# GANtastic3/MaskCycleGAN-VC

Measured on AMD Instinct MI355X. Metric: train iters/s (full G+D step), 80x64 mel bs=1, higher is better.
Workload: dtype f32

## Files before the change

### include/mcvc.h

```cpp
#ifndef MCVC_H
#define MCVC_H

#ifdef __cplusplus
extern "C" {
#endif

#define MCVC_ABI_VERSION 3
#define MCVC_GEN_NPARAMS 110
#define MCVC_DISC_NPARAMS 20
#define MCVC_N_MEL 80

int mcvc_version(void);

int mcvc_set_deterministic(int on);
int mcvc_get_deterministic(void);
int mcvc_set_precise(int on);
int mcvc_get_precise(void);
int mcvc_set_trunk_persistent(int on);

int mcvc_twin_begin(void);
int mcvc_twin_switch(void);
int mcvc_twin_end(void);
int mcvc_twin_launches(void);

// ... 19 lines not shown
                     float* out, float* stash, float* scratch, long long scratch_floats, int B, int T, void* stream);
int mcvc_gen_backward(const float* const* params, const float* packed, float* const* grads, const float* mask,
                      const float* dout, float* dx, int accumulate_dx, const float* stash,
                      float* scratch, long long scratch_floats, int B, int T, void* stream, void* aux_stream);
int mcvc_gen_backward_overlap(const float* const* params, const float* packed, float* const* grads, const float* mask,
                              const float* dout, float* dx, int accumulate_dx, const float* stash,
                              float* scratch, long long scratch_floats, int B, int T, void* stream, void* aux_stream,
                              void* const* milestones);

int mcvc_gen_trunk_fault(float* scratch, int B, int T, int reset, void* stream);
int mcvc_debug_trunk_fault_inject(int on);

#define MCVC_BWD_NO_JOIN 1
#define MCVC_BWD_FINE_MILESTONES 2
#define MCVC_BWD_STORE_GRADS 4
int mcvc_grad_store_mask(int net, int T, unsigned char* covered);
int mcvc_gen_backward_flags(const float* const* params, const float* packed, float* const* grads, const float* mask,
                            const float* dout, float* dx, int accumulate_dx, const float* stash,
                            float* scratch, long long scratch_floats, int B, int T, void* stream, void* aux_stream,
                            void* const* milestones, int flags);
int mcvc_gen_backward_prefix(const float* const* params, const float* packed, float* const* grads, const float* mask,
                             const float* dout, float* dx, int accumulate_dx, const float* stash, int stash_B,
                             float* scratch, long long scratch_floats, int B, int T, void* stream, void* aux_stream,
                             void* const* milestones, int flags);
int mcvc_gen_backward_window(const float* const* params, const float* packed, float* const* grads, const float* mask,
                             const float* dout, float* dx, int accumulate_dx, const float* stash, int stash_B, int stash_b0,
                             float* scratch, long long scratch_floats, int B, int T, void* stream, void* aux_stream,
                             void* const* milestones, int flags);
int mcvc_set_trunk_passes_in_flight(int n);
int mcvc_gen_trunk_persistent(int B, int T);

long long mcvc_gen_bf16_packed_bytes(void);
long long mcvc_gen_bf16_workspace_bytes(int B, int T);
int mcvc_gen_bf16_pack(const float* const* params, void* packed, void* stream);
int mcvc_gen_infer_bf16(const float* const* params, const void* packed, const float* x, const float* mask, float* out, void* workspace,
                        long long workspace_bytes, int B, int T, void* stream);

long long mcvc_bf16_conv2d_pack_bytes(int Cout, int Cin, int KH, int KW);
int mcvc_bf16_conv2d(const void* x, const float* w, const float* bias, void* y, void* wpack, int N, int H, int W, int Cin, int Cout,
                     int KH, int KW, int stride, int pad_h, int pad_w, void* stream);
long long mcvc_bf16_conv1_glu_pack_bytes(void);
int mcvc_bf16_conv1_glu(const float* x, const float* mask, const float* w, const float* b, const float* wg, const float* bg, void* y, void* wpack,
                        int B, int T, void* stream);
long long mcvc_bf16_last_conv_pack_bytes(void);
int mcvc_bf16_last_conv(const void* x, const float* w, const float* b, float* out, void* wpack, int B, int T, void* stream);
long long mcvc_bf16_c2d1d_pack_bytes(void);
int mcvc_bf16_c2d1d_norm(const void* x, const float* w, const float* gamma, const float* beta, void* y, void* wpack, int B, int W, void* stream);
long long mcvc_bf16_trunk_layer_pack_bytes(int Cin, int C, int gated);
int mcvc_bf16_trunk_layer(const void* x, const float* w, const float* w_gate, const float* gamma, const float* beta, const float* gamma_gate,
                          const float* beta_gate, const void* residual, void* y, void* wpack, int B, int W, int Cin, int C, void* stream);
int mcvc_bf16_instnorm_act(const void* x, const float* gamma, const float* beta, const float* gamma_gate, const float* beta_gate,
                           const void* residual, void* y, float* scratch, int N, int H, int W, int Cx, int act, int pixel_shuffle, void* stream);

int mcvc_disc_forward(const float* const* params, const float* packed, const float* x, float* out,
                      float* stash, float* scratch, long long scratch_floats, int B, int T, void* stream);
int mcvc_disc_backward(const float* const* params, const float* packed, float* const* grads,
                       const float* dout, int dout_is_logit_grad, float* dx, int accumulate_dx,
                       const float* stash, float* scratch, long long scratch_floats, int B, int T, void* stream,
                       void* aux_stream);
int mcvc_disc_backward_flags(const float* const* params, const float* packed, float* const* grads,
                             const float* dout, int dout_is_logit_grad, float* dx, int accumulate_dx,
                             const float* stash, float* scratch, long long scratch_floats, int B, int T, void* stream,
                             void* aux_stream, int flags);

int mcvc_l1_loss(const float* a, const float* b, long long n, float weight, float* loss_slot, float* term_slot,
                 float* grad_a, int accumulate_grad, void* stream);
int mcvc_lsgan_loss(const float* d, long long n, float target, float weight, float* loss_slot, float* term_slot,
                    float* grad_logit, void* stream);

int mcvc_loss_combine(const float* pairs, int n, const int* loss_dst, const int* term_dst, float* slots, void* stream);

int mcvc_adam_step(float* p, const float* g, float* exp_avg, float* exp_avg_sq, long long n, float lr,
                   float beta1, float beta2, float eps, int step, float grad_scale, void* stream);
int mcvc_adam_step2(float* p, float* g, float* g2, int zero_grads, float* exp_avg, float* exp_avg_sq, long long n, float lr,
                    float beta1, float beta2, float eps, int step, float grad_scale, void* stream);
int mcvc_gen_update_ranges(const float* const* params, const long long* numel, float* packed, int max_batch, int T, int range_mask,
                           const float* flat, float* grad, float* grad2, float* exp_avg, float* exp_avg_sq, float lr, float beta1,
                           float beta2, float eps, int step, float grad_scale, int zero_grads, void* stream);
int mcvc_disc_update_batch(const float* const* params, const long long* numel, float* packed, int max_batch, int T,
                           const float* flat, float* grad, float* grad2, float* exp_avg, float* exp_avg_sq, float lr, float beta1,
                           float beta2, float eps, int step, float grad_scale, int zero_grads, void* stream);

int mcvc_pack_plan(int net, int max_batch, int T, int sets, int range_mask, int update, long long* rows, int cap, int* n_rows);
int mcvc_axpy(float* y, const float* x, float alpha, long long n, void* stream);

int mcvc_draw_batch(const float* bank_A, const int* offs_A, int n_A, long long frames_A, const float* bank_B, const int* offs_B, int n_B,
                    long long frames_B, int B, int T, int max_mask_len, unsigned long long seed, unsigned long long step,
                    float* real_A, float* mask_A, float* real_B, float* mask_B, int* draws, void* stream);

int mcvc_audio_frames(int n_samples);
long long mcvc_audio_basis_floats(void);
int mcvc_audio_basis_init(float* basis);
int mcvc_audio_plan(const int* sample_offs, int n_utts, int* frame_offs, int* tiles, int max_tiles, int* n_tiles);
int mcvc_audio_log_mel(const float* wave, long long n_samples, const int* tiles, int n_tiles, const float* basis, float* out,
                       long long total_frames, void* stream);

int mcvc_voc_out_samples(int T);
int mcvc_voc_launches(void);
long long mcvc_voc_packed_floats(void);
int mcvc_voc_pack(const float* const* host_table, float* packed_host);
long long mcvc_voc_workspace_floats(int B, int T);
int mcvc_voc_decode(const float* packed, const float* mel, float* out, float* workspace, long long workspace_floats, int B, int T, void* stream);
long long mcvc_voc_layer_packed_floats(int kind, int Cin, int Cout, int k, int r);
int mcvc_voc_layer_pack(int kind, const float* w0, const float* b0, const float* w1, const float* b1, float* packed_host, int Cin, int Cout, int k, int r);
int mcvc_voc_layer(int kind, const float* packed, const float* x0, const float* x1, float* y, int B, int Cin, int Cout, int L, int k, int dilation, int r,
                   int act_in, void* stream);

int mcvc_gl_out_samples(int T);
int mcvc_gl_launches(int n_iter);
long long mcvc_gl_tables_floats(void);
int mcvc_gl_tables_init(const float* host_pinv, float* host_out);
long long mcvc_gl_workspace_floats(int B, int T);
int mcvc_gl_decode(const float* in, int in_kind, const float* angles0, const float* tables, float* out, float* workspace,
                   long long workspace_floats, int B, int T, int n_iter, float momentum, void* stream);

int mcvc_melinv_max_iter(void);
long long mcvc_melinv_tables_floats(void);
int mcvc_melinv_tables_init(const float* host_basis, const float* host_pinv, double lambda, float* host_out);
int mcvc_melinv_solve(const float* logmel, const float* tables, float* mag_out, int B, int T, int n_iter, void* stream);

int mcvc_dtw_max_frames(void);
int mcvc_dtw_launches(int want_path);
int mcvc_cep_basis_init(int n_cep, float* basis_host);
int mcvc_cep_project(const float* mel, long long n_frames, const float* basis, int n_cep, float* out, void* stream);
int mcvc_dtw_plan(const int* x_offs, const int* y_offs, int n_pairs, int want_path, long long* table, long long* workspace_bytes, long long* path_rows);
int mcvc_dtw_run(const float* x, long long x_frames, const float* y, long long y_frames, int K, float scale, const int* x_offs, const int* y_offs,
                 const long long* table, int n_pairs, float* cost, int* length, int* path, void* workspace, long long workspace_bytes, void* stream);

int mcvc_f0_max_lag(void);
int mcvc_f0_launches(int want_cmnd);
int mcvc_f0_track(const float* wave, long long n_samples, const int* tiles, int n_tiles, int tau_min, int tau_max, float threshold, float* f0,
                  float* aperiodicity, float* cmnd, long long total_frames, void* stream);
int mcvc_f0_stats(const float* fx, long long x_frames, const float* fy, long long y_frames, const int* path, const long long* pairs, int n_pairs,
                  int* counts, float* sums, void* stream);

int mcvc_ms_max_fft(void);
int mcvc_ms_launches(void);
int mcvc_ms_table_init(int n_fft, float* table_host);
int mcvc_ms_power(const float* cep, long long n_frames, int K, const int* offs_dev, int n_utts, const int* offs_host, int n_fft, const float* table,
                  float* power, float* mean, float* var, void* stream);
int mcvc_ms_mean_log(const float* values, int n, long long R, float floor, float* out, void* stream);
int mcvc_ms_distance(const float* a, const float* b, int K, int n_bins, int n_used, float* per_dim, float* total, void* stream);

long long mcvc_conv2d_pack_floats(int Cout, int Cin, int KH, int KW);
int mcvc_conv2d_forward(const float* x, const float* w, const float* bias, float* y, float* wpack,
                        float* slabs, int max_slabs, int N, int Cin, int H, int W, int Cout, int KH, int KW,
                        int stride, int pad_h, int pad_w, int pixel_shuffle, void* stream);
int mcvc_conv2d_dgrad(const float* dy, const float* w, float* dx, float* wpack, float* slabs, int max_slabs,
                      int N, int Cin, int H, int W, int Cout, int KH, int KW, int stride, int pad_h, int pad_w,
                      void* stream);
long long mcvc_conv2d_wgrad_slab_floats(int N, int Cin, int H, int W, int Cout, int KH, int KW, int stride, int pad_h, int pad_w);
int mcvc_conv2d_wgrad(const float* x, const float* dy, float* dw, float* slabs, long long slab_floats, int N, int Cin, int H, int W,
                      int Cout, int KH, int KW, int stride, int pad_h, int pad_w, void* stream);
long long mcvc_layer_packed_floats(int Cin, int Cout, int branches, int KH, int KW, int stride, int pad_h, int pad_w);
long long mcvc_layer_scratch_floats(int N, int H, int W, int Cin, int Cout, int branches, int KH, int KW, int stride, int pad_h, int pad_w);
int mcvc_layer_pack(const float* w0, const float* b0, const float* w1, const float* b1, float* packed, int Cin, int Cout, int branches,
                    int KH, int KW, int stride, int pad_h, int pad_w, void* stream);
int mcvc_layer_forward(const float* x, const float* packed, const float* w0, const float* w1, float* y, float* scratch,
                       long long scratch_floats, int N, int H, int W, int Cin, int Cout, int branches, int KH, int KW, int stride,
                       int pad_h, int pad_w, int scheme, int pixel_shuffle, void* stream);
int mcvc_layer_dgrad(const float* dy, const float* packed, const float* w0, const float* w1, float* dx, float* scratch,
                     long long scratch_floats, int N, int H, int W, int Cin, int Cout, int branches, int KH, int KW, int stride,
                     int pad_h, int pad_w, int scheme, void* stream);
int mcvc_layer_wgrad(const float* x, const float* dy, float* dw0, float* dw1, float* scratch, long long scratch_floats, int N, int H,
                     int W, int Cin, int Cout, int branches, int KH, int KW, int stride, int pad_h, int pad_w, int scheme, void* stream);
int mcvc_layer_wgrad_flags(const float* x, const float* dy, float* dw0, float* dw1, float* scratch, long long scratch_floats, int N, int H,
// ... 39 lines not shown
```

### maskcyclegan-vc_amd/csrc/net.hip

```cpp
#include "mcvc_common.h"
#include "twin.h"
#include "pack.h"
#include "packforms.h"
#include "misc.h"
#include "trunk.h"
#include "wino.h"
#include "wino4.h"
#include "sgemm.h"
#include "sampler.h"
#include "audio.h"
#include "vocoder.h"
#include "griffinlim.h"
#include "melinv.h"
#include "dtw.h"
#include "ms.h"
#include "f0.h"
#include "../../include/mcvc.h"
#include <string.h>
#include <algorithm>
#include <array>
#include <tuple>
#include <map>
#include <mutex>
#include <vector>

static int g_deterministic = [] { const char* e = getenv("MCVC_DETERMINISTIC"); return (e && atoi(e) != 0) ? 1 : 0; }();
int mcvc_deterministic() { return g_deterministic; }

namespace {

constexpr float kInEps = 1e-5f;

struct View { float* p; long long sb, sc; int sh; };
struct CView { const float* p; long long sb, sc; int sh; };
static inline CView cv(const View& v) { return CView{v.p, v.sb, v.sc, v.sh}; }

constexpr int kMaxLayers = 20;
struct PackFresh { unsigned layer[kMaxLayers]; PackFresh() { for (unsigned& m : layer) m = kAllForms; } };

struct Exec {
    hipStream_t s;
    bool dry;
    int err;
    bool fine_ms = false;
    float* slabs;
    long long slab_cap;
    long long slab_need;
    int max_split;
    hipStream_t s2;
    float* wslabs;
    long long wslab_cap;
    long long wslab_need;
    float* wv; float* wm;
    long long wino_cap;
    float* wv2; float* wm2; float* wu;
    long long wu_cap;
    float* sg; long long sg_cap, sg_need;
    float* sgw; long long sgw_cap, sgw_need;
    const float* const* params;
    int br1_on_main = 0;
    int no_join = 0;
    int fuse_next = 0;
    const struct WinoFam* pend_fam = nullptr;
    WinoOutArgs pend;
    int y_xs_pw = 0; long long y_xs_plane = 0;
    int dx_pitch = 0;
    int wgrad_x_xs = 0;
    int store_grads = 0;
    int force_scheme = 0;
    PackFresh fresh;
    unsigned* sync;
    std::vector<std::pair<const void*, hipEvent_t>> readers;
    void fail(int e) { if (!err && e) err = e; }
};

static std::mutex g_pack_mu;
static std::map<const void*, PackFresh> g_pack_fresh;
static PackFresh get_fresh(const void* packed)
{
    std::lock_guard<std::mutex> lk(g_pack_mu);
    auto it = g_pack_fresh.find(packed);
    return it == g_pack_fresh.end() ? PackFresh() : it->second;
}

static hipEvent_t pool_event()
{
    static std::mutex mu;
    static std::vector<hipEvent_t> pool;
    static size_t next = 0;
    std::lock_guard<std::mutex> lk(mu);
    if (pool.empty()) {
        pool.resize(1024);
        for (hipEvent_t& e : pool) (void)hipEventCreateWithFlags(&e, hipEventDisableTiming);
    }
    next = (next + 1) % pool.size();
    return pool[next];
}

static bool is_fresh(const Exec& ex, const ConvSpec& c, PackForm f) { return (ex.fresh.layer[c.index] >> f & 1) != 0; }
static bool any_fresh(const Exec& ex, PackForm f) { for (unsigned m : ex.fresh.layer) if (m >> f & 1) return true; return false; }
static bool stale(Exec& ex, const ConvSpec& c, PackForm f)
{
    if (ex.dry || is_fresh(ex, c, f)) return false;
    ex.fail(MCVC_ERR_INVALID);
    return true;
}

static void wait_readers(Exec& ex, const void* buf)
{
    if (!ex.s2 || ex.dry) return;
    for (auto it = ex.readers.begin(); it != ex.readers.end();) {
        if (it->first == buf) { ex.fail(mcvc_stream_wait(ex.s, it->second)); it = ex.readers.erase(it); }
        else ++it;
    }
}

static void join_aux(Exec& ex)
{
    if (!ex.s2 || ex.dry) return;
    hipEvent_t e = pool_event();
    ex.fail(mcvc_event_record(e, ex.s2));
    ex.fail(mcvc_stream_wait(ex.s, e));
    ex.readers.clear();
}

static ConvSpec mk(int Cin, int Cout, int nbr, int KH, int KW, int stride, int ph, int pw, int w0, int b0, int w1, int b1, int bias_grad)
{
    ConvSpec c{};
    c.Cin = Cin; c.Cout = Cout; c.nbr = nbr; c.KH = KH; c.KW = KW; c.stride = stride; c.ph = ph; c.pw = pw;
    c.wi[0] = w0; c.bi[0] = b0; c.wi[1] = w1; c.bi[1] = b1; c.has_bias_grad = bias_grad;
    return c;
}

static inline int conv_out(int H, int K, int s, int p) { return (H + 2 * p - K) / s + 1; }

static void run_conv(Exec& ex, const ConvProblem& p, int NB, ConvIO io, long long y_total, const float* w, int w_rows, int w_cout,
                     const float* bias, int allow_split, int force_nsplit, int* nsplit_out)
{
    int ns = 1;
    if (force_nsplit > 0) ns = force_nsplit;
    else if (allow_split) ns = mcvc_conv_plan_nsplit(p, NB, 1);
    if (ns < 1) { ex.fail(MCVC_ERR_INVALID); ns = 1; }
    if (ex.max_split > 0 && ns > ex.max_split) ns = ex.max_split;
    if (io.accumulate && mcvc_deterministic()) ns = 1;
    if (!io.accumulate) {
        const long long need = (long long)(ns - 1) * y_total;
        if (need > ex.slab_need) ex.slab_need = need;
// ... 47 lines not shown
    return n < 32 ? 32 : n;
}
static int wino43_min_nb()
{
    static const int nb = mcvc_knob("MCVC_WINO43_NB", 4);
    return nb;
}
static bool wino4_applies(const Exec& ex, const ConvSpec& c, int NB, int H, int W, bool reads_set = true)
{
    if (ex.force_scheme == 1 || ex.force_scheme >= 3) return false;
    if (ex.force_scheme == 2) return c.wino && (H & 3) == 0 && (W & 3) == 0;
    return c.wino && wino4_min_nb() > 0 && NB >= wino4_min_nb() && (H & 3) == 0 && (W & 3) == 0 &&
           (reads_set ? is_fresh(ex, c, PF_W4F) : any_fresh(ex, PF_W4F));
}
static bool wino43_applies(const Exec& ex, const ConvSpec& c, int NB, int OH, int OW, bool reads_set = true)
{
    if (ex.force_scheme == 1 || ex.force_scheme >= 3) return false;
    if (ex.force_scheme == 2) return c.wino3 && (OH & 3) == 0 && (OW & 3) == 0;
    return c.wino3 && wino43_min_nb() > 0 && NB >= wino43_min_nb() && (OH & 3) == 0 && (OW & 3) == 0 &&
           (reads_set ? is_fresh(ex, c, PF_W43F) : any_fresh(ex, PF_W43F));
}
static int wino4_chunk(const Exec& ex, int NB, long long tiles_per_sample, int KM, int pts)
{
    const long long cap_tiles = (ex.wino_cap / ((long long)pts * KM)) & ~31LL;
    if (tiles_per_sample <= 0 || cap_tiles < tiles_per_sample) return 0;
    const long long nbmax = cap_tiles / tiles_per_sample;
    if (NB <= nbmax) return NB;
    const long long nch = (NB + nbmax - 1) / nbmax;
    return (int)((NB + nch - 1) / nch);
}

struct WinoFam {
    int pts;
    int nxi;
    int tile;
    int pad;
    int min_pitch;
    int norm_pts;
    int (*input)(const WinoXformArgs&, hipStream_t);
    int (*input_phase)(const WinoXformArgs&, int XH, int XW, hipStream_t);
    int (*output)(const WinoOutArgs&, hipStream_t);
    int (*input_t)(const WinoXformArgs&, hipStream_t);
    int (*input_phase_t)(const WinoXformArgs&, int XH, int XW, hipStream_t);
    int (*dy_t)(const WinoXformArgs&, hipStream_t);
    int (*dw)(const float* du, float* dw0, float* dw1, int Cout, int nbr, int Cin, int store, hipStream_t);
};
enum { kF23, kF25, kF43, kF45 };
static const WinoFam kWino[4] = {
    {16, 16, 2, 1, 32, 16, mcvc_wino3_input_launch, mcvc_wino3_input_phase_launch, mcvc_wino3_output_launch,
     nullptr, mcvc_wino3_input_phase_t_launch, mcvc_wino3_dy_t_launch, mcvc_wino3_dw_launch},
    {36, 0, 2, 2, 32, 36, mcvc_wino_input_launch, nullptr, mcvc_wino_output_launch,
     mcvc_wino_input_t_launch, nullptr, mcvc_wino_dy_t_launch,
     [](const float* du, float* dw0, float*, int Cout, int, int Cin, int store, hipStream_t s) { return mcvc_wino_dw_launch(du, dw0, Cout, Cin, store, s); }},
    {36, 36, 4, 1, 32, 43, mcvc_wino43_input_launch, mcvc_wino43_input_phase_launch, mcvc_wino43_output_launch,
     nullptr, mcvc_wino43_input_phase_t_launch, mcvc_wino43_dy_t_launch, mcvc_wino43_dw_launch},
    {64, 64, 4, 2, 64 , 64, mcvc_wino4_input_launch, nullptr, mcvc_wino4_output_launch,
     mcvc_wino4_input_t_launch, nullptr, mcvc_wino4_dy_t_launch,
     [](const float* du, float* dw0, float*, int Cout, int, int Cin, int store, hipStream_t s) { return mcvc_wino4_dw_launch(du, dw0, Cout, Cin, store, s); }},
};
static long long wino_tiles(const WinoFam& f, int H, int W) { return (long long)((H + f.tile - 1) / f.tile) * ((W + f.tile - 1) / f.tile); }

static int wino_nbc(const Exec& ex, const WinoFam& f, int NB, long long tiles, int KM, int min_tiles)
{
    if (f.tile == 4) {
        const int nbc = wino4_chunk(ex, NB, tiles, KM, f.pts);
        return (nbc && (nbc * tiles >= min_tiles || ex.force_scheme == 2)) ? nbc : 0;
    }
    const int nbc = wino_chunk(NB, tiles);
    const long long NTc = wino_chunk_tiles(NB, tiles);
    return (nbc && NTc >= min_tiles && f.pts * NTc * KM <= ex.wino_cap) ? nbc : 0;
}

struct WinoPass {
    const WinoFam* f;
    int K, M;
    int NB, nbc;
    int H, W;
    int XH, XW;
    const float* a; long long a_xi; int lda, a_rows;
    const float* bias;
    int shuffle, YH, YW, accumulate;
    bool may_defer;
};
static void wino_pass(Exec& ex, const WinoPass& p, CView x, View y)
{
    const WinoFam& f = *p.f;
    const int K = p.K, M = p.M, TH = (p.H + f.tile - 1) / f.tile, TW = (p.W + f.tile - 1) / f.tile;
    for (int b0 = 0; b0 < p.NB; b0 += p.nbc) {
        const int nb = p.NB - b0 < p.nbc ? p.NB - b0 : p.nbc;
        const long long NT = (long long)nb * TH * TW, NTp = std::max<long long>((NT + 31) & ~31LL, f.min_pitch);
        WinoXformArgs xi{};
        xi.x = x.p + (long long)b0 * x.sb; xi.x_sb = x.sb; xi.x_sc = x.sc; xi.x_sh = x.sh; xi.v = ex.wv;
        xi.N = nb; xi.C = K; xi.H = p.H; xi.W = p.W; xi.TH = TH; xi.TW = TW; xi.NT = (int)NT; xi.NTp = (int)NTp; xi.pad = f.pad;
        ex.fail(p.XH ? f.input_phase(xi, p.XH, p.XW, ex.s) : f.input(xi, ex.s));
        static const int own_gemm = mcvc_knob("MCVC_WINO_GEMM", 1);
        if (&f != &kWino[kF25] || (own_gemm && (M % 128) == 0 && (K % 16) == 0 && NTp >= 64)) {
            WinoGemmArgs ga{};
            ga.a = p.a; ga.a_xi = p.a_xi; ga.lda = p.lda;
            ga.b = ex.wv; ga.b_xi = (long long)K * NTp; ga.ldb = (int)NTp;
            ga.c = ex.wm; ga.c_xi = (long long)M * NTp; ga.ldc = (int)NTp;
            ga.M = M; ga.N = (int)NTp; ga.K = K; ga.nxi = f.nxi;
            ex.fail(mcvc_wino_gemm_launch(ga, ex.s));
        } else {
            ConvProblem cp{K, (int)(NTp / 32), 32, M, (int)(NTp / 32), 32, 1, 1, 1, 0, 0};
            ConvIO io{};
            io.x = ex.wv; io.x_sb = (long long)K * NTp; io.x_sc = NTp; io.x_sh = 32;
            io.y = ex.wm; io.y_sb = (long long)M * NTp; io.y_sc = NTp; io.y_sh = 32; io.y_sw = 1;
            io.nsplit = 1;
            io.w_nstride = p.a_xi;
            io.tile_cfg = wino_tile_cfg(M, NT);
            io.gemm_ok = 1;
            ex.fail(mcvc_conv_launch(cp, 36, io, p.a, p.a_rows, p.lda, nullptr, ex.s, nullptr));
        }
        WinoOutArgs oa{};
        oa.m = ex.wm; oa.bias = p.bias;
        oa.y = y.p + (long long)b0 * y.sb; oa.y_sb = y.sb; oa.y_sc = y.sc; oa.y_sh = y.sh;
        oa.N = nb; oa.Cout = M; oa.OH = p.H; oa.OW = p.W; oa.TH = TH; oa.TW = TW; oa.NT = (int)NT; oa.NTp = (int)NTp;
        oa.shuffle = p.shuffle; oa.YH = p.YH; oa.YW = p.YW; oa.accumulate = p.accumulate;
        if (p.may_defer && ex.fuse_next && p.nbc == p.NB) { ex.pend = oa; ex.pend_fam = &f; }
        else ex.fail(f.output(oa, ex.s));
    }
}

static void wino_wgrad_pass(Exec& ex, const WinoFam& f, const ConvSpec& c, float* const* grads, int NB, int nbc, int H, int W, CView x, CView dy,
                            int store, hipStream_t ws)
{
    const bool phase = c.stride == 2;
    const int IH = phase ? H / 2 : H, IW = phase ? W / 2 : W, N = phase ? 4 * c.Cin : c.Cin, M = c.cout_tot;
    const int TH = (IH + f.tile - 1) / f.tile, TW = (IW + f.tile - 1) / f.tile;
    for (int b0 = 0; b0 < NB; b0 += nbc) {
        const int nb = NB - b0 < nbc ? NB - b0 : nbc;
        const long long NT = (long long)nb * TH * TW, NTp = (NT + 31) & ~31LL;
        WinoXformArgs xi{};
        xi.x = x.p + (long long)b0 * x.sb; xi.x_sb = x.sb; xi.x_sc = x.sc; xi.x_sh = x.sh; xi.v = ex.wv2;
        xi.N = nb; xi.C = N; xi.H = IH; xi.W = IW; xi.TH = TH; xi.TW = TW; xi.NT = (int)NT; xi.NTp = (int)NTp; xi.pad = f.pad;
        ex.fail(phase ? f.input_phase_t(xi, H, W, ws) : f.input_t(xi, ws));
        WinoXformArgs di{};
        di.x = dy.p + (long long)b0 * dy.sb; di.x_sb = dy.sb; di.x_sc = dy.sc; di.x_sh = dy.sh; di.v = ex.wm2;
        di.N = nb; di.C = M; di.H = IH; di.W = IW; di.TH = TH; di.TW = TW; di.NT = (int)NT; di.NTp = (int)NTp; di.pad = 0;
        ex.fail(f.dy_t(di, ws));
        WinoGemmArgs ga{};
        ga.a = ex.wm2; ga.a_xi = NTp * M; ga.lda = M;
        ga.b = ex.wv2; ga.b_xi = NTp * N; ga.ldb = N;
        ga.c = ex.wu; ga.c_xi = (long long)M * N; ga.ldc = N;
        ga.M = M; ga.N = N; ga.K = (int)((NT + 15) & ~15LL); ga.nxi = f.nxi;
        ex.fail(mcvc_wino_gemm_launch(ga, ws));
        ex.fail(f.dw(ex.wu, grads[c.wi[0]], c.nbr == 2 ? grads[c.wi[1]] : nullptr, c.Cout, c.nbr, c.Cin, store && b0 == 0, ws));
    }
}

static bool conv_wino(Exec& ex, const ConvSpec& c, const float* packed, int dgrad, int NB, int H, int W, CView x, View y, int shuffle,
                      int accumulate)
{
    if (!c.wino || !wino_enabled() || !ex.wv) return false;
    const int K = dgrad ? c.cout_tot : c.Cin, M = dgrad ? c.Cin : c.cout_tot;
    const WinoFam* f = &kWino[kF45];
    int nbc = 0;
    if (wino4_applies(ex, c, NB, H, W) && (M % 128) == 0 && (K % 16) == 0) nbc = wino_nbc(ex, *f, NB, wino_tiles(*f, H, W), K > M ? K : M, wino4_min_tiles());
    if (!nbc) {
        if (stale(ex, c, wino_form(false, dgrad))) return true;
        f = &kWino[kF25];
        nbc = wino_nbc(ex, *f, NB, wino_tiles(*f, H, W), K > M ? K : M, 0);
    }
    if (!nbc) return false;
    if (ex.dry) return true;
    const bool four = f->tile == 4;
    WinoPass p{};
    p.f = f; p.K = K; p.M = M; p.NB = NB; p.nbc = nbc; p.H = H; p.W = W;
    const PackForm form = wino_form(four, dgrad);
    p.a = packed + c.off[form]; p.a_xi = form_xi(c, form); p.lda = kPackForms[form].ld(c); p.a_rows = dgrad ? c.dg_rows_co : c.cin_pad;
    p.bias = dgrad ? nullptr : packed + c.off[PF_BIAS];
    p.shuffle = shuffle; p.YH = 2 * H; p.YW = 2 * W; p.accumulate = accumulate;
    p.may_defer = !dgrad && shuffle;
    wino_pass(ex, p, x, y);
    return true;
}

static bool conv_wino3(Exec& ex, const ConvSpec& c, const float* packed, int dgrad, int NB, int H, int W, CView x, View y, int accumulate)
{
    if (!c.wino3 || !wino_enabled() || !ex.wv) return false;
    if (!dgrad && ((H & 1) != 0 || (W & 1) != 0 || (c.cout_tot % 128) != 0)) return false;
    static const int en[2] = {mcvc_knob("MCVC_WINO3_FWD", 1), mcvc_knob("MCVC_WINO3", 1)};
    if (!en[dgrad]) return false;
    const int OH = conv_out(H, c.KH, c.stride, c.ph), OW = conv_out(W, c.KW, c.stride, c.pw);
    const int K = dgrad ? c.cout_tot : 4 * c.Cin, M = dgrad ? 4 * c.Cin : c.cout_tot;
    const WinoFam* f = &kWino[kF43];
    int nbc = 0;
    if (wino43_applies(ex, c, NB, OH, OW) && 2 * OH == H && 2 * OW == W) nbc = wino_nbc(ex, *f, NB, wino_tiles(*f, OH, OW), K > M ? K : M, 64);
    if (!nbc) {
        f = &kWino[kF23];
        nbc = wino_nbc(ex, *f, NB, wino_tiles(*f, OH, OW), K > M ? K : M, 64);
    }
    if (!nbc) return false;
    if (ex.dry) return true;
    const bool four = f->tile == 4;
    WinoPass p{};
    p.f = f; p.K = K; p.M = M; p.NB = NB; p.nbc = nbc; p.H = OH; p.W = OW;
    const PackForm form = wino3_form(four, dgrad);
    p.a = packed + c.off[form]; p.a_xi = form_xi(c, form); p.lda = kPackForms[form].ld(c);
    if (dgrad) {
        p.shuffle = 1; p.YH = H; p.YW = W; p.accumulate = accumulate;
    } else {
        p.XH = H; p.XW = W;
        p.bias = packed + c.off[PF_BIAS];
        p.YH = OH; p.YW = OW;
        p.may_defer = true;
    }
    wino_pass(ex, p, x, y);
    return true;
}

struct SgKind { int kind, taps, OH, OW; };
static thread_local int t_no_sgemm = 0;
static thread_local int t_user_operands = 0;
static SgKind sgemm_kind(const ConvSpec& c, int NB, int H, int W)
{
    static const int min_cols = mcvc_knob("MCVC_SGEMM1D_COLS", 64);
    SgKind k{0, 0, 0, 0};
    if (t_no_sgemm || t_user_operands) return k;
    if (c.nbr > 2 || (c.cout_tot % 64) != 0 || (c.Cout % 32) != 0 || c.cin_pad != c.Cin) return k;
    if (c.KH == 1 && (c.KW == 1 || c.KW == 3) && c.stride == 1 && c.ph == 0 && c.pw == (c.KW - 1) / 2) {
        k.OH = H; k.OW = W; k.taps = c.KW;
        if (min_cols > 0 && (long long)NB * H * W >= min_cols && (c.Cin % 64) == 0 && (W & 3) == 0) k.kind = 2;
    }
    return k;
}
static int split_by_cost(long long tiles, int Kmin)
{
    static const int wgs = mcvc_knob("MCVC_SGEMM_WGS", 256);
    static const int maxsp = mcvc_knob("MCVC_SGEMM_MAXSPLIT", 8);
    int sp = 1;
    while (sp < maxsp && tiles * sp < wgs && (Kmin % (64 * sp)) == 0 && Kmin / (2 * sp) >= 64) sp *= 2;
    return sp;
}
static int sgemm_split(int M, long long N, int K)
{
    return split_by_cost((long long)(M / 64) * ((N + 63) / 64), K);
}

static bool igemm_enabled()
{
    static const int en = mcvc_knob("MCVC_IGEMM", 1);
    return en != 0;
}
static bool igemm_applies(const ConvSpec& c, int H, int W)
{
    return igemm_enabled() && c.igemm && (H & 1) == 0 && (W & 1) == 0 && ((W / 2) & 3) == 0 && H >= 2 && W >= 8;
}
static void xs_tap_offsets(int H, int W, long long boff[9])
{
    const int pw = mcvc_xs_pw(W);
    const long long plane = mcvc_xs_plane(H, W);
    for (int kh = 0; kh < 3; ++kh)
        for (int kw = 0; kw < 3; ++kw) {
            const int ph = (kh == 1) ? 0 : 1, di = (kh == 0) ? -1 : 0, pq = (kw == 1) ? 0 : 1, dj = (kw == 0) ? -1 : 0;
            boff[3 * kh + kw] = (long long)(2 * ph + pq) * plane + (long long)(1 + di) * pw + 4 + dj;
        }
}
static int igemm_split(long long tiles, int Kmin) { return split_by_cost(tiles, Kmin); }
static void conv_fwd_igemm(Exec& ex, const ConvSpec& c, const float* packed, int NB, int H, int W, const float* xs, View y, long long y_total,
                           int allow_split, int* nsplit)
{
    const int OH = H / 2, OW = W / 2, P = OH * OW, KT = 9 * c.Cin;
    const long long NT = (long long)NB * P;
    const int sp = (allow_split && nsplit) ? igemm_split((long long)(c.cout_tot / 64) * ((NT + 63) / 64), KT) : 1;
    const long long slab_need = (long long)(sp - 1) * y_total;
    if (slab_need > ex.slab_need) ex.slab_need = slab_need;
    if (nsplit) *nsplit = sp;
    if (ex.dry) return;
    if (slab_need > ex.slab_cap) { ex.fail(MCVC_ERR_WORKSPACE); return; }
    const int pw = mcvc_xs_pw(W);
    const long long plane = mcvc_xs_plane(H, W);
    IGemmArgs g{};
    g.ncls = 1;
    g.cls[0].a = packed + c.off[PF_IFWD]; g.cls[0].ntaps = 9; g.cls[0].coff = 0;
    xs_tap_offsets(H, W, g.cls[0].boff);
    for (int t = 0; t < 9; ++t) g.cls[0].aoff[t] = (long long)t * c.Cin * c.cout_pk;
    g.a_ks = c.cout_pk;
    g.b = xs; g.b_cs = 4 * plane; g.b_sn = (long long)c.Cin * 4 * plane; g.b_pitch = pw; g.Cb = c.Cin; g.OW = OW; g.P = P;
    g.c = y.p; g.ldc = y.sc; g.c_sn = y.sb; g.c_sh = y.sh; g.c_sw = 1;
    g.bias = packed + c.off[PF_BIAS];
    g.M = c.cout_tot; g.N = (int)NT; g.nsplit = sp; g.c_slab = ex.slabs; g.c_split = y_total;
    ex.fail(mcvc_igemm_launch(g, ex.s));
}
static void conv_dgrad_igemm(Exec& ex, const ConvSpec& c, const float* packed, int NB, int H, int W, const float* dyp, View dx, long long dx_total,
                             int accumulate, int allow_split, int* nsplit)
{
    const int OH = H / 2, OW = W / 2, P = OH * OW;
    const long long NT = (long long)NB * P;
    int sp = (allow_split && nsplit && !accumulate) ? igemm_split(4LL * (c.Cin / 64) * ((NT + 63) / 64), c.cout_tot) : 1;
    const long long slab_need = (long long)(sp - 1) * dx_total;
    if (slab_need > ex.slab_need) ex.slab_need = slab_need;
    if (nsplit) *nsplit = sp;
    if (ex.dry) return;
    if (slab_need > ex.slab_cap) { ex.fail(MCVC_ERR_WORKSPACE); return; }
    const int pitch = mcvc_dyp_pitch(OW);
    const long long plane = mcvc_dyp_plane(OH, OW);
    IGemmArgs g{};
    g.ncls = c.ncls;
    for (int k = 0; k < c.ncls; ++k) {
        const DgradClass& d = c.icls[k];
        IGemmClass& q = g.cls[k];
        q.a = packed + c.off[PF_IFWD]; q.ntaps = d.nth * d.ntw;
        q.coff = (long long)d.qh * dx.sh + d.qw;
        for (int u = 0; u < d.nth; ++u)
            for (int v = 0; v < d.ntw; ++v) {
                const int kh = d.khmax - 2 * u, kw = d.kwmax - 2 * v;
                q.boff[u * d.ntw + v] = (long long)((d.qh + 1 - kh) / 2) * pitch + (d.qw + 1 - kw) / 2;
                q.aoff[u * d.ntw + v] = (long long)(3 * kh + kw) * c.Cin * c.cout_pk;
            }
    }
    g.a_ks = c.cout_pk; g.arow = 1;
    g.b = dyp; g.b_cs = plane; g.b_sn = (long long)c.cout_tot * plane; g.b_pitch = pitch; g.Cb = c.cout_tot; g.OW = OW; g.P = P;
    g.c = dx.p; g.ldc = dx.sc; g.c_sn = dx.sb; g.c_sh = 2 * dx.sh; g.c_sw = 2; g.accumulate = accumulate;
    g.M = c.Cin; g.N = (int)NT; g.nsplit = sp; g.c_slab = ex.slabs; g.c_split = dx_total;
    ex.fail(mcvc_igemm_launch(g, ex.s));
}

static void conv_fwd(Exec& ex, const ConvSpec& c, const float* packed, int NB, int H, int W, CView x, View y, long long y_total,
                     int shuffle, int allow_split, int* nsplit)
{
    const SgKind sk = shuffle ? SgKind{0, 0, 0, 0} : sgemm_kind(c, NB, H, W);
    if (sk.kind) {
        const int P = sk.OH * sk.OW, KT = sk.taps * c.Cin;
        const long long NT = (long long)NB * P;
        const bool b_in_place = c.KW == 1;
        const int sp = (allow_split && nsplit) ? sgemm_split(c.cout_tot, NT, KT) : 1;
        const long long slab_need = (long long)(sp - 1) * y_total;
        if (ex.dry) { if (slab_need > ex.slab_need) ex.slab_need = slab_need; if (nsplit) *nsplit = sp; return; }
        if (stale(ex, c, PF_FWD)) return;
        if (!b_in_place && slab_need <= ex.slab_cap && y.sh == sk.OW && y.sc == P && (NB == 1 || y.sb == (long long)c.cout_tot * P)) {
            IGemmArgs g{};
            g.ncls = 1;
            IGemmClass& q = g.cls[0];
            q.a = packed + c.off[PF_FWD]; q.ntaps = c.KW; q.coff = 0;
            for (int kw = 0; kw < c.KW; ++kw) { q.boff[kw] = kw - c.pw; q.aoff[kw] = (long long)kw * c.cout_pk; q.zs[kw] = kw < c.pw ? 1 : (kw > c.pw ? 2 : 0); }
            g.a_ks = (long long)c.KW * c.cout_pk; g.zw = W;
            g.b = x.p; g.b_cs = x.sc; g.b_sn = x.sb; g.b_pitch = x.sh; g.Cb = c.Cin; g.OW = W; g.P = P;
            g.c = y.p; g.ldc = y.sc; g.c_sn = y.sb; g.c_sh = y.sh; g.c_sw = 1;
            g.bias = packed + c.off[PF_BIAS];
            g.M = c.cout_tot; g.N = (int)NT; g.nsplit = sp; g.c_slab = ex.slabs; g.c_split = y_total;
            ex.fail(mcvc_igemm_launch(g, ex.s));
            if (nsplit) *nsplit = sp;
            return;
        }
        if (b_in_place && x.sh == W && x.sc == P && slab_need <= ex.slab_cap && y.sh == sk.OW && y.sc == P &&
            (NB == 1 || y.sb == (long long)c.cout_tot * P)) {
            SGemmArgs g{};
            g.a = packed + c.off[PF_FWD]; g.lda = c.cout_pk;
            g.b = x.p; g.ldb = x.sc; g.bseg = P; g.b_sn = x.sb;
            g.c = y.p; g.ldc = y.sc; g.cseg = P; g.c_sn = y.sb;
            g.bias = packed + c.off[PF_BIAS];
            g.M = c.cout_tot; g.N = (int)NT; g.K = KT; g.nsplit = sp; g.c_slab = ex.slabs; g.c_split = y_total;
            ex.fail(mcvc_sgemm_launch(g, ex.s));
            if (nsplit) *nsplit = sp;
            return;
        }
    }
    if (conv_wino(ex, c, packed, 0, NB, H, W, x, y, shuffle, 0) || (!shuffle && conv_wino3(ex, c, packed, 0, NB, H, W, x, y, 0))) { if (nsplit) *nsplit = 1; return; }
    if (stale(ex, c, PF_FWD)) return;
    ConvProblem p{c.Cin, H, W, c.cout_tot, conv_out(H, c.KH, c.stride, c.ph), conv_out(W, c.KW, c.stride, c.pw),
                  c.KH, c.KW, c.stride, c.ph, c.pw};
    ConvIO io{};
    io.x = x.p; io.x_sb = x.sb; io.x_sc = x.sc; io.x_sh = x.sh;
    io.y = y.p; io.y_sb = y.sb; io.y_sc = y.sc; io.y_sh = y.sh; io.y_sw = 1;
    io.shuffle = shuffle;
    run_conv(ex, p, NB, io, y_total, packed + c.off[PF_FWD], c.w_rows, c.cout_pk, packed + c.off[PF_BIAS], allow_split, 0, nsplit);
}

static void conv_dgrad(Exec& ex, const ConvSpec& c, const float* packed, int NB, int H, int W, CView dy, View dx, long long dx_total,
                       int accumulate, int allow_split, int* nsplit)
{
    if (conv_wino(ex, c, packed, 1, NB, H, W, dy, dx, 0, accumulate)) { if (nsplit) *nsplit = 1; return; }
    const int OH = conv_out(H, c.KH, c.stride, c.ph), OW = conv_out(W, c.KW, c.stride, c.pw);
    const int st = c.stride;
    const SgKind sk = sgemm_kind(c, NB, H, W);
    if (sk.kind) {
        const int P = sk.OH * sk.OW;
        const long long NT = (long long)NB * P;
        int sp = (allow_split && nsplit) ? igemm_split((long long)(c.Cin / 64) * ((NT + 63) / 64), sk.taps * c.cout_tot) : 1;
        while (sp > 1 && ((long long)sk.taps * c.cout_tot) % (32LL * sp) != 0) sp /= 2;
        const bool slab_all = accumulate && sp > 1;
        const long long slab_need = (long long)(slab_all ? sp : sp - 1) * dx_total;
        if (slab_need > ex.slab_need) ex.slab_need = slab_need;
        if (nsplit) *nsplit = slab_all ? sp + 1 : sp;
        if (ex.dry) return;
        if (stale(ex, c, PF_FWD)) return;
        if (slab_need > ex.slab_cap) { ex.fail(MCVC_ERR_WORKSPACE); return; }
        IGemmArgs g{};
        g.ncls = 1;
        IGemmClass& q = g.cls[0];
        q.a = packed + c.off[PF_FWD]; q.ntaps = c.KW; q.coff = 0;
        for (int kw = 0; kw < c.KW; ++kw) {
            const int sh = c.pw - kw;
            q.boff[kw] = sh; q.aoff[kw] = (long long)kw * c.cout_pk; q.zs[kw] = sh < 0 ? 1 : (sh > 0 ? 2 : 0);
        }
        g.a_ks = (long long)c.KW * c.cout_pk; g.arow = 1; g.zw = W;
        g.b = dy.p; g.b_cs = dy.sc; g.b_sn = dy.sb; g.b_pitch = dy.sh; g.Cb = c.cout_tot; g.OW = W; g.P = P;
        g.ldc = dx.sc; g.c_sn = dx.sb; g.c_sh = dx.sh; g.c_sw = 1;
        g.M = c.Cin; g.N = (int)NT; g.nsplit = sp; g.c_split = dx_total;
        if (slab_all) { g.c = ex.slabs; g.c_slab = ex.slabs + dx_total; }
        else { g.c = dx.p; g.c_slab = ex.slabs; g.accumulate = accumulate; }
        ex.fail(mcvc_igemm_launch(g, ex.s));
        return;
    }
    if (conv_wino3(ex, c, packed, 1, NB, H, W, dy, dx, accumulate)) { if (nsplit) *nsplit = 1; return; }
    static const int ucls_nb = mcvc_knob("MCVC_DGRAD_CLASSES_NB", 8);
    const bool per_class = c.merged && c.off[PF_DCLS] >= 0 && NB >= ucls_nb;
    if (stale(ex, c, per_class ? PF_DCLS : PF_DGRAD)) return;
    if (c.merged && !per_class) {
        ConvProblem p{c.cout_tot, OH, OW, 4 * c.Cin, (H + 1) / 2, (W + 1) / 2, c.mg_kh, c.mg_kw, 1, c.mg_pad_h, c.mg_pad_w};
        ConvIO io{};
        io.x = dy.p; io.x_sb = dy.sb; io.x_sc = dy.sc; io.x_sh = dy.sh;
        io.y = dx.p; io.y_sb = dx.sb; io.y_sc = dx.sc; io.y_sh = dx.sh; io.y_sw = 1;
        io.accumulate = accumulate; io.shuffle = 1; io.YH = H; io.YW = W;
        run_conv(ex, p, NB, io, dx_total, packed + c.off[PF_DGRAD], c.dg_rows_co * c.mg_kh * c.mg_kw, c.mg_ld, nullptr, allow_split, 0, nsplit);
        return;
    }
    const DgradClass* klass = per_class ? c.ucls : c.cls;
    const long long kbase = c.off[per_class ? PF_DCLS : PF_DGRAD];
    ConvProblem ps[4];
    int force = 0;
    for (int k = 0; k < c.ncls; ++k) {
        const DgradClass& d = klass[k];
        ps[k] = ConvProblem{c.cout_tot, OH, OW, c.Cin, (H - d.qh + st - 1) / st, (W - d.qw + st - 1) / st,
                            d.nth, d.ntw, 1, d.pad_h, d.pad_w};
    }
    if (c.ncls > 1 && allow_split) {
        force = 1 << 30;
        for (int k = 0; k < c.ncls; ++k) { const int n = mcvc_conv_plan_nsplit(ps[k], NB, 1); if (n < force) force = n; }
        if (force < 1) force = 1;
        if (ex.max_split > 0 && force > ex.max_split) force = ex.max_split;
    }
    int ns_all = 1;
    for (int k = 0; k < c.ncls; ++k) {
        const DgradClass& d = klass[k];
        if (ps[k].OH <= 0 || ps[k].OW <= 0) continue;
        ConvIO io{};
        io.x = dy.p; io.x_sb = dy.sb; io.x_sc = dy.sc; io.x_sh = dy.sh;
        io.y = dx.p + (long long)d.qh * dx.sh + d.qw; io.y_sb = dx.sb; io.y_sc = dx.sc; io.y_sh = dx.sh * st; io.y_sw = st;
        io.accumulate = accumulate;
        int ns = 1;
        Exec sub = ex;
        if (!ex.dry) sub.slabs = ex.slabs + (long long)d.qh * dx.sh + d.qw;
        run_conv(sub, ps[k], NB, io, dx_total, packed + kbase + d.offset, c.dg_rows_co * d.nth * d.ntw, c.cin_pk, nullptr,
                 allow_split, force, &ns);
        ex.err = sub.err; ex.slab_need = sub.slab_need;
        if (ns > ns_all) ns_all = ns;
    }
    if (nsplit) *nsplit = ns_all;
// ... 323 lines not shown
    const float* x; const float* stats;
    const float* g0; const float* b0; const float* g1; const float* b1;
    float* out;
    float* dg0; float* db0; float* dg1; float* db1;
    int xB;
};

static bool trunk_dgrad(Exec& ex, const ConvSpec& c, const float* packed, const float* dy, float* dx, int accumulate, int B, int W4,
                        int* nsplit = nullptr, const TrunkPre* pre = nullptr)
{
    if (!trunk_enabled() || c.off[PF_TRUNK_T] < 0) return false;
    int ks = 1;
    if (!accumulate && mcvc_trunk_applies(c.cout_tot, c.KW, c.Cin, B, W4, TRUNK_PLAIN, 1)) ks = 1;
    else ks = trunk_pick_ksplit(c.cout_tot, c.KW, c.Cin, B, W4, 0);
    if (ks < 1) return false;
    if (!accumulate && ks > 1 && !nsplit) return false;
    const long long tot = (long long)c.Cin * B * W4;
    const bool slab_all = accumulate && ks > 1 && nsplit && mcvc_deterministic();
    if (ks > 1 && (!accumulate || nsplit)) {
        const long long need = (long long)(accumulate ? ks : ks - 1) * tot;
        if (need > ex.slab_need) ex.slab_need = need;
        if (!ex.dry && need > ex.slab_cap) { ex.fail(MCVC_ERR_WORKSPACE); return true; }
    }
    if (nsplit) *nsplit = slab_all ? ks + 1 : (accumulate ? 1 : ks);
    if (ex.dry) return true;
    TrunkArgs a{};
    a.a0 = packed + c.off[PF_TRUNK_T];
    a.x = dy; a.x_sc = (long long)B * W4; a.x_sb = W4;
    a.Cin = c.cout_tot; a.KW = c.KW; a.K = c.cout_tot * c.KW; a.M = c.Cin; a.Mtot = c.Cin; a.B = B; a.T4 = W4; a.N = B * W4;
    a.conv_out = dx; a.c_sc = (long long)B * W4; a.c_sb = W4; a.accumulate = accumulate; a.mode = TRUNK_PLAIN;
    a.slabs = ex.slabs; a.slab_stride = tot; a.slab_all = slab_all ? 1 : 0;
    if (pre) {
        a.pre = pre->kind; a.pre_C = (pre->kind == 2) ? c.cout_tot / 2 : c.cout_tot;
        a.pre_x = pre->x; a.pre_xB = pre->xB; a.pre_stats = pre->stats; a.pre_gamma0 = pre->g0; a.pre_beta0 = pre->b0; a.pre_gamma1 = pre->g1; a.pre_beta1 = pre->b1;
        a.pre_out = pre->out; a.pre_dgamma0 = pre->dg0; a.pre_dbeta0 = pre->db0; a.pre_dgamma1 = pre->dg1; a.pre_dbeta1 = pre->db1;
        wait_readers(ex, pre->out);
    }
    ex.fail(mcvc_trunk_launch(a, ks, ex.s));
    return true;
}

static bool trunk_fwd_ksplit(Exec& ex, const ConvSpec& c, const float* const* P, const float* x, float* conv_out, int B, int W4, int* nsplit)
{
    if (!trunk_enabled() || c.KH != 1 || c.nbr != 1) return false;
    const int ks = trunk_pick_ksplit(c.Cin, c.KW, c.Cout, B, W4, 1);
    if (ks < 1) return false;
    const long long tot = (long long)c.Cout * B * W4;
    const long long need = (long long)(ks - 1) * tot;
    if (need > ex.slab_need) ex.slab_need = need;
    if (!ex.dry && need > ex.slab_cap) { ex.fail(MCVC_ERR_WORKSPACE); return true; }
    *nsplit = ks;
    if (ex.dry) return true;
    TrunkArgs a{};
    a.a0 = P[c.wi[0]]; a.bias0 = P[c.bi[0]];
    a.x = x; a.x_sc = (long long)B * W4; a.x_sb = W4;
    a.Cin = c.Cin; a.KW = c.KW; a.K = c.Cin * c.KW; a.M = c.Cout; a.Mtot = c.Cout; a.B = B; a.T4 = W4; a.N = B * W4;
    a.conv_out = conv_out; a.c_sc = (long long)B * W4; a.c_sb = W4; a.accumulate = 0; a.mode = TRUNK_PLAIN;
    a.slabs = ex.slabs; a.slab_stride = tot;
    ex.fail(mcvc_trunk_launch(a, ks, ex.s));
    return true;
}

struct NormP { const float* g[2]; const float* b[2]; float* dg[2]; float* db[2]; };

static NormP normp(const float* const* params, float* const* grads, int g0, int b0, int g1 = -1, int b1 = -1)
{
    NormP n{};
    if (!params) return n;
    n.g[0] = params[g0]; n.b[0] = params[b0];
    if (g1 >= 0) { n.g[1] = params[g1]; n.b[1] = params[b1]; }
    if (grads) {
        n.dg[0] = grads[g0]; n.db[0] = grads[b0];
        if (g1 >= 0) { n.dg[1] = grads[g1]; n.db[1] = grads[b1]; }
    }
    return n;
}

static int fuse_wino_norm()
{
    static const int en = mcvc_knob("MCVC_FUSE_WINO_NORM", 1);
    return en;
}

static void norm_fwd(Exec& ex, float* x, long long x_sn, long long x_sc, long long x_total, int nslab, const NormP& np, float* stats,
                     float* y, long long y_sn, long long y_sc, int y_sh, const float* res, int N, int C, int H, int W, int act)
{
    if (ex.dry) { ex.y_xs_pw = 0; return; }
    NormArgs a{};
    a.x = x; a.x_slabs = ex.slabs; a.x_sn = x_sn; a.x_sc = x_sc; a.slab_stride = x_total; a.nslab = nslab;
    a.gamma[0] = np.g[0]; a.gamma[1] = np.g[1]; a.beta[0] = np.b[0]; a.beta[1] = np.b[1];
    a.stats = stats; a.y = y; a.res = res; a.y_sn = y_sn; a.y_sc = y_sc; a.y_sh = y_sh;
    a.N = N; a.C = C; a.H = H; a.W = W; a.act = act; a.eps = kInEps;
    if (ex.y_xs_pw) { a.y_xs = 1; a.xs_pw = ex.y_xs_pw; a.xs_plane = ex.y_xs_plane; ex.y_xs_pw = 0; }
    if (ex.pend_fam) {
        const WinoFam& f = *ex.pend_fam;
        ex.pend_fam = nullptr;
        if (mcvc_norm_fwd_wino_applies(a, ex.pend, f.norm_pts)) { ex.fail(mcvc_norm_fwd_wino_launch(a, ex.pend, f.norm_pts, ex.s)); return; }
        ex.fail(f.output(ex.pend, ex.s));
    }
    ex.fail(mcvc_norm_fwd_launch(a, ex.s));
}

static void norm_bwd(Exec& ex, const float* x, long long x_sn, long long x_sc, const NormP& np, const float* stats,
                     float* dy, long long y_sn, long long y_sc, int y_sh, long long dy_total, int nslab,
                     float* dx, long long dx_sn, long long dx_sc, int dx_sh, int unshuffle, int N, int C, int H, int W, int act)
{
    if (ex.dry) { ex.dx_pitch = 0; return; }
    wait_readers(ex, dx);
    NormBwdArgs a{};
    a.x = x; a.x_sn = x_sn; a.x_sc = x_sc;
    a.gamma[0] = np.g[0]; a.gamma[1] = np.g[1]; a.beta[0] = np.b[0]; a.beta[1] = np.b[1];
    a.stats = stats; a.dy = dy; a.dy_slabs = ex.slabs; a.y_sn = y_sn; a.y_sc = y_sc; a.y_sh = y_sh; a.slab_stride = dy_total; a.nslab = nslab;
    a.dx = dx; a.dx_sn = dx_sn; a.dx_sc = dx_sc; a.dx_sh = dx_sh; a.unshuffle = unshuffle;
    a.dgamma[0] = np.dg[0]; a.dgamma[1] = np.dg[1]; a.dbeta[0] = np.db[0]; a.dbeta[1] = np.db[1];
    a.N = N; a.C = C; a.H = H; a.W = W; a.act = act;
    a.dx_pitch = ex.dx_pitch; ex.dx_pitch = 0;
    ex.fail(mcvc_norm_bwd_launch(a, ex.s));
}

static void act_fwd(Exec& ex, float* x, long long x_total, int nslab, float* y, int N, int C, int P, int act)
{
    if (ex.dry) return;
    ActArgs a{}; a.x = x; a.x_slabs = ex.slabs; a.slab_stride = x_total; a.nslab = nslab; a.y = y; a.N = N; a.C = C; a.P = P; a.act = act;
    ex.fail(mcvc_act_fwd_launch(a, ex.s));
}

static void act_bwd(Exec& ex, const float* x, float* dy, long long dy_total, int nslab, float* dx, int N, int C, int P, int act)
{
    if (ex.dry) return;
    wait_readers(ex, dx);
    ActBwdArgs a{}; a.x = x; a.dy = dy; a.dy_slabs = ex.slabs; a.slab_stride = dy_total; a.nslab = nslab; a.dx = dx; a.N = N; a.C = C; a.P = P; a.act = act;
    ex.fail(mcvc_act_bwd_launch(a, ex.s));
}

struct GenNet {
    ConvSpec conv1, ds1, ds2, c2d1d, res_vg[6], res_out[6], c1d2d, up1, up2, last;
    long long packed_floats;
};

static void gen_layers(const GenNet& g, const ConvSpec** l)
{
    const ConvSpec* head[] = {&g.conv1, &g.ds1, &g.ds2, &g.c2d1d, &g.c1d2d, &g.up1, &g.up2, &g.last};
    for (int i = 0; i < 8; ++i) l[i] = head[i];
    for (int i = 0; i < 6; ++i) { l[8 + 2 * i] = &g.res_vg[i]; l[9 + 2 * i] = &g.res_out[i]; }
}
static GenNet build_gen()
{
    GenNet g{};
    long long cur = 0;
    g.conv1 = mk(2, 128, 2, 5, 15, 1, 2, 7, 0, 1, 2, 3, 1);
    g.ds1 = mk(128, 256, 2, 5, 5, 2, 2, 2, 4, 5, 8, 9, 0);
    g.ds2 = mk(256, 256, 2, 5, 5, 2, 2, 2, 12, 13, 16, 17, 0);
    g.c2d1d = mk(5120, 256, 1, 1, 1, 1, 0, 0, 20, 21, -1, -1, 0);
    for (int i = 0; i < 6; ++i) {
        const int b = 24 + 12 * i;
        g.res_vg[i] = mk(256, 512, 2, 1, 3, 1, 0, 1, b + 0, b + 1, b + 4, b + 5, 0);
        g.res_out[i] = mk(512, 256, 1, 1, 3, 1, 0, 1, b + 8, b + 9, -1, -1, 0);
    }
    g.c1d2d = mk(256, 5120, 1, 1, 1, 1, 0, 0, 96, 97, -1, -1, 0);
    g.up1 = mk(256, 1024, 1, 5, 5, 1, 2, 2, 104, 105, -1, -1, 1);
    g.up2 = mk(256, 512, 1, 5, 5, 1, 2, 2, 100, 101, -1, -1, 1);
    g.last = mk(128, 1, 1, 5, 15, 1, 2, 7, 108, 109, -1, -1, 1);
    const ConvSpec* l[kMaxLayers];
    gen_layers(g, l);
    for (int i = 0; i < kMaxLayers; ++i) { ConvSpec& c = const_cast<ConvSpec&>(*l[i]); c.index = i; spec_finalize(c, cur); }
    g.packed_floats = cur;
    return g;
}
static const GenNet& gen_net() { static const GenNet g = build_gen(); return g; }
static const ConvSpec* const* gen_specs()
{
    static const ConvSpec* l[kMaxLayers];
    static const bool once = (gen_layers(gen_net(), l), true);
    (void)once;
    return l;
}

struct GenDims {
    int B, T, W2, W4, Wu1, Wu2;
    long long big;
};
static GenDims gen_dims(int B, int T)
{
    GenDims d{};
    d.B = B; d.T = T;
    d.W2 = conv_out(T, 5, 2, 2);
    d.W4 = conv_out(d.W2, 5, 2, 2);
    d.Wu1 = 2 * d.W4; d.Wu2 = 4 * d.W4;
    const int wmax = d.T > d.Wu2 ? d.T : d.Wu2;
    d.big = (long long)B * 256 * 80 * wmax;
    return d;
}

struct GenStash {
    long long xin, c1, y1, c2, s2, y2, c3, s3, y3, c4, s4, y4;
    struct { long long ca, sa, ya, cb, sb, y; } r[6];
    long long c6, s6, y6, c7, s7, y7, c8, s8, y8, total;
};
static GenStash gen_stash(const GenDims& d)
{
    GenStash s{};
    long long cur = 0;
    auto take = [&](long long n) { const long long o = cur; cur += (n + 3) & ~3LL; return o; };
    const long long B = d.B;
    s.xin = take(B * 2 * 80 * d.T);
    s.c1 = take(B * 256 * 80 * d.T);   s.y1 = take(B * 128 * 80 * d.T);
    s.c2 = take(B * 512 * 40 * d.W2);  s.s2 = take(B * 512 * 2);  s.y2 = take(B * 256 * 40 * d.W2);
    s.c3 = take(B * 512 * 20 * d.W4);  s.s3 = take(B * 512 * 2);  s.y3 = take(B * 5120 * d.W4);
    s.c4 = take(B * 256 * d.W4);       s.s4 = take(B * 256 * 2);  s.y4 = take(B * 256 * d.W4);
    for (int i = 0; i < 6; ++i) {
        s.r[i].ca = take(B * 1024 * d.W4); s.r[i].sa = take(B * 1024 * 2); s.r[i].ya = take(B * 512 * d.W4);
        s.r[i].cb = take(B * 256 * d.W4);  s.r[i].sb = take(B * 256 * 2);  s.r[i].y = take(B * 256 * d.W4);
    }
    s.c6 = take(B * 5120 * d.W4);      s.s6 = take(B * 5120 * 2); s.y6 = take(B * 5120 * d.W4);
    s.c7 = take(B * 256 * 40 * d.Wu1); s.s7 = take(B * 256 * 2);  s.y7 = take(B * 256 * 40 * d.Wu1);
    s.c8 = take(B * 128 * 80 * d.Wu2); s.s8 = take(B * 128 * 2);  s.y8 = take(B * 128 * 80 * d.Wu2);
    s.total = cur;
    return s;
}

struct GenScratch { long long ga, gb, gb2, dh, dt1, dt1b, dt2, dt3, dt3b, dtx1, dtx3, wv, wm, wino_floats, wv2, wm2, wu, wu_floats, sync, slabs; };
static GenScratch gen_scratch(const GenDims& d)
{
    GenScratch s{};
    long long cur = 0;
    auto take = [&](long long n) { const long long o = cur; cur += (n + 3) & ~3LL; return o; };
    s.sync = take(2 * MCVC_TRUNK_SYNC_WORDS);
    s.ga = take(d.big); s.gb = take(d.big); s.gb2 = take(d.big);
    s.dh = take((long long)256 * d.B * d.W4); s.dt1 = take((long long)1024 * d.B * d.W4); s.dt1b = take((long long)1024 * d.B * d.W4);
    s.dt2 = take((long long)512 * d.B * d.W4); s.dt3 = take((long long)256 * d.B * d.W4); s.dt3b = take((long long)256 * d.B * d.W4);
    s.dtx1 = take(mcvc_wgrad_smallk_batch_applies(d.B, d.W4) ? 6LL * 1024 * d.B * d.W4 : 0);
    s.dtx3 = take(mcvc_wgrad_smallk_batch_applies(d.B, d.W4) ? 6LL * 256 * d.B * d.W4 : 0);
    {
        const long long nt1 = wino_chunk_tiles(d.B, 10LL * ((d.W4 + 1) / 2)), nt2 = wino_chunk_tiles(d.B, 20LL * ((d.Wu1 + 1) / 2));
        const long long a1 = 36LL * 1024 * nt1, a2 = 36LL * 512 * nt2;
        s.wino_floats = wino_enabled() ? (a1 > a2 ? a1 : a2) : 0;
        s.wv = take(s.wino_floats); s.wm = take(s.wino_floats);
        s.wv2 = take(s.wino_floats); s.wm2 = take(s.wino_floats);
        s.wu_floats = wino_enabled() ? 36LL * 1024 * 1024 : 0;
        s.wu = take(s.wu_floats);
    }
    s.slabs = cur;
    return s;
}

static void gen_forward_impl(Exec& ex, const float* const* P, const float* packed, const float* x, const float* mask, float* out,
                             float* st, const GenDims& d)
{
    ex.params = P;
    const GenNet& g = gen_net();
    const GenStash o = gen_stash(d);
    const int B = d.B, T = d.T, W2 = d.W2, W4 = d.W4, Wu1 = d.Wu1, Wu2 = d.Wu2;
    const long long BT4 = (long long)B * W4;
    int ns = 1;
    if (!ex.dry) ex.fail(mcvc_prep_input_launch(x, mask, st + o.xin, B, 80 * T, ex.s));
    conv_fwd(ex, g.conv1, packed, B, 80, T, CView{st + o.xin, 2LL * 80 * T, 80LL * T, T}, View{st + o.c1, 256LL * 80 * T, 80LL * T, T},
             (long long)B * 256 * 80 * T, 0, 1, &ns);
    act_fwd(ex, st + o.c1, (long long)B * 256 * 80 * T, ns, st + o.y1, B, 128, 80 * T, ACT_GLU);
    ex.fuse_next = fuse_wino_norm();
    conv_fwd(ex, g.ds1, packed, B, 80, T, CView{st + o.y1, 128LL * 80 * T, 80LL * T, T}, View{st + o.c2, 512LL * 40 * W2, 40LL * W2, W2},
             (long long)B * 512 * 40 * W2, 0, 1, &ns);
    ex.fuse_next = 0;
    norm_fwd(ex, st + o.c2, 512LL * 40 * W2, 40LL * W2, (long long)B * 512 * 40 * W2, ns, normp(P, nullptr, 6, 7, 10, 11), st + o.s2,
             st + o.y2, 256LL * 40 * W2, 40LL * W2, W2, nullptr, B, 256, 40, W2, ACT_GLU);
    ex.fuse_next = fuse_wino_norm();
    conv_fwd(ex, g.ds2, packed, B, 40, W2, CView{st + o.y2, 256LL * 40 * W2, 40LL * W2, W2}, View{st + o.c3, 512LL * 20 * W4, 20LL * W4, W4},
             (long long)B * 512 * 20 * W4, 0, 1, &ns);
    ex.fuse_next = 0;
    norm_fwd(ex, st + o.c3, 512LL * 20 * W4, 20LL * W4, (long long)B * 512 * 20 * W4, ns, normp(P, nullptr, 14, 15, 18, 19), st + o.s3,
             st + o.y3, W4, 20LL * BT4, (int)BT4, nullptr, B, 256, 20, W4, ACT_GLU);
    if (trunk_fwd_ksplit(ex, g.c2d1d, P, st + o.y3, st + o.c4, B, W4, &ns)) {}
    else conv_fwd(ex, g.c2d1d, packed, 1, B, W4, CView{st + o.y3, 0, BT4, W4}, View{st + o.c4, 0, BT4, W4}, 256 * BT4, 0, 1, &ns);
    norm_fwd(ex, st + o.c4, W4, BT4, 256 * BT4, ns, normp(P, nullptr, 22, 23), st + o.s4, st + o.y4, W4, BT4, W4, nullptr, B, 256, 1, W4, ACT_NONE);
    const float* h = st + o.y4;
    if (trunk_net_enabled() && trunk_enabled() && ex.sync && mcvc_trunk_net_applies(B, W4)) {
        if (!ex.dry) {
            TrunkFwdNetArgs na{};
            int l = 0;
            auto fill = [&](const ConvSpec& c, int g0, int be0, int g1, int be1, const float* x, float* cvo, float* stats, float* y,
                            long long y_sn, long long y_sc, const float* res, int rows) {
                TrunkLayerDesc& d = na.L[l++];
                d.a0 = P[c.wi[0]]; d.bias0 = P[c.bi[0]]; d.gamma0 = P[g0]; d.beta0 = P[be0];
                if (c.nbr == 2) { d.a1 = P[c.wi[1]]; d.bias1 = P[c.bi[1]]; d.gamma1 = P[g1]; d.beta1 = P[be1]; }
                d.x = x; d.conv_out = cvo; d.stats = stats; d.y = y; d.y_sn = y_sn; d.y_sc = y_sc; d.res = res;
                d.Cin = c.Cin; d.KW = c.KW; d.M = c.Cout; d.mode = (c.nbr == 2) ? TRUNK_IN_GLU : TRUNK_IN; d.rows = rows;
            };
            for (int i = 0; i < 6; ++i) {
                const int b = 24 + 12 * i;
                fill(g.res_vg[i], b + 2, b + 3, b + 6, b + 7, h, st + o.r[i].ca, st + o.r[i].sa, st + o.r[i].ya, W4, BT4, nullptr, 8);
                fill(g.res_out[i], b + 10, b + 11, -1, -1, st + o.r[i].ya, st + o.r[i].cb, st + o.r[i].sb, st + o.r[i].y, W4, BT4, h, 4);
                h = st + o.r[i].y;
            }
            na.nlayers = l; na.B = B; na.T4 = W4; na.eps = kInEps; na.sync = ex.sync;
            ex.fail(mcvc_trunk_fwd_net_launch(na, ex.s));
        } else {
            h = st + o.r[5].y;
        }
        if (!trunk_fwd(ex, g.c1d2d, P, 98, 99, -1, -1, h, st + o.c6, st + o.s6, st + o.y6, 5120LL * W4, W4, nullptr, B, W4)) ex.fail(MCVC_ERR_INVALID);
    } else {
    for (int i = 0; i < 6; ++i) {
        const int b = 24 + 12 * i;
        if (!trunk_fwd(ex, g.res_vg[i], P, b + 2, b + 3, b + 6, b + 7, h, st + o.r[i].ca, st + o.r[i].sa, st + o.r[i].ya, W4, BT4, nullptr, B, W4)) {
            conv_fwd(ex, g.res_vg[i], packed, 1, B, W4, CView{h, 0, BT4, W4}, View{st + o.r[i].ca, 0, BT4, W4}, 1024 * BT4, 0, 1, &ns);
            norm_fwd(ex, st + o.r[i].ca, W4, BT4, 1024 * BT4, ns, normp(P, nullptr, b + 2, b + 3, b + 6, b + 7), st + o.r[i].sa,
                     st + o.r[i].ya, W4, BT4, W4, nullptr, B, 512, 1, W4, ACT_GLU);
        }
        if (!trunk_fwd(ex, g.res_out[i], P, b + 10, b + 11, -1, -1, st + o.r[i].ya, st + o.r[i].cb, st + o.r[i].sb, st + o.r[i].y, W4, BT4, h, B, W4)) {
            conv_fwd(ex, g.res_out[i], packed, 1, B, W4, CView{st + o.r[i].ya, 0, BT4, W4}, View{st + o.r[i].cb, 0, BT4, W4}, 256 * BT4, 0, 1, &ns);
            norm_fwd(ex, st + o.r[i].cb, W4, BT4, 256 * BT4, ns, normp(P, nullptr, b + 10, b + 11), st + o.r[i].sb,
                     st + o.r[i].y, W4, BT4, W4, h, B, 256, 1, W4, ACT_NONE);
        }
        h = st + o.r[i].y;
    }
    if (!trunk_fwd(ex, g.c1d2d, P, 98, 99, -1, -1, h, st + o.c6, st + o.s6, st + o.y6, 5120LL * W4, W4, nullptr, B, W4)) {
        conv_fwd(ex, g.c1d2d, packed, 1, B, W4, CView{h, 0, BT4, W4}, View{st + o.c6, 0, BT4, W4}, 5120 * BT4, 0, 1, &ns);
        norm_fwd(ex, st + o.c6, W4, BT4, 5120 * BT4, ns, normp(P, nullptr, 98, 99), st + o.s6, st + o.y6, 5120LL * W4, W4, W4, nullptr,
                 B, 5120, 1, W4, ACT_NONE);
    }
    }
    ex.fuse_next = fuse_wino_norm();
    conv_fwd(ex, g.up1, packed, B, 20, W4, CView{st + o.y6, 256LL * 20 * W4, 20LL * W4, W4}, View{st + o.c7, 256LL * 40 * Wu1, 40LL * Wu1, Wu1},
             (long long)B * 256 * 40 * Wu1, 1, 1, &ns);
    ex.fuse_next = 0;
    norm_fwd(ex, st + o.c7, 256LL * 40 * Wu1, 40LL * Wu1, (long long)B * 256 * 40 * Wu1, ns, normp(P, nullptr, 106, 107), st + o.s7,
             st + o.y7, 256LL * 40 * Wu1, 40LL * Wu1, Wu1, nullptr, B, 256, 40, Wu1, ACT_SILU);
    ex.fuse_next = fuse_wino_norm();
    conv_fwd(ex, g.up2, packed, B, 40, Wu1, CView{st + o.y7, 256LL * 40 * Wu1, 40LL * Wu1, Wu1}, View{st + o.c8, 128LL * 80 * Wu2, 80LL * Wu2, Wu2},
             (long long)B * 128 * 80 * Wu2, 1, 1, &ns);
    ex.fuse_next = 0;
    norm_fwd(ex, st + o.c8, 128LL * 80 * Wu2, 80LL * Wu2, (long long)B * 128 * 80 * Wu2, ns, normp(P, nullptr, 102, 103), st + o.s8,
             st + o.y8, 128LL * 80 * Wu2, 80LL * Wu2, Wu2, nullptr, B, 128, 80, Wu2, ACT_SILU);
    conv_fwd(ex, g.last, packed, B, 80, Wu2, CView{st + o.y8, 128LL * 80 * Wu2, 80LL * Wu2, Wu2}, View{out, 80LL * Wu2, 80LL * Wu2, Wu2},
             (long long)B * 80 * Wu2, 0, 1, &ns);
    if (ns > 1) act_fwd(ex, out, (long long)B * 80 * Wu2, ns, nullptr, B, 1, 80 * Wu2, ACT_NONE);
}

static void record_milestone(Exec& ex, void* ev)
{
    if (!ev || ex.dry) return;
    hipStream_t on = ex.s;
    if (ex.s2) {
        hipEvent_t e = pool_event();
        ex.fail(mcvc_event_record(e, ex.s));
        ex.fail(mcvc_stream_wait(ex.s2, e));
        on = ex.s2;
    }
    ex.fail(mcvc_event_record((hipEvent_t)ev, on));
}

static void shift_stash(GenStash& s, const GenDims& d, int b0)
{
    if (b0 <= 0) return;
    const long long b = b0, T = d.T, W2 = d.W2, W4 = d.W4;
    s.xin += b * 2 * 80 * T; s.c1 += b * 256 * 80 * T; s.y1 += b * 128 * 80 * T;
    s.c2 += b * 512 * 40 * W2; s.s2 += b * 512 * 2; s.y2 += b * 256 * 40 * W2;
    s.c3 += b * 512 * 20 * W4; s.s3 += b * 512 * 2; s.y3 += b * W4;
    s.c4 += b * W4; s.s4 += b * 256 * 2; s.y4 += b * W4;
    for (int i = 0; i < 6; ++i) {
        s.r[i].ca += b * W4; s.r[i].sa += b * 1024 * 2; s.r[i].ya += b * W4;
        s.r[i].cb += b * W4; s.r[i].sb += b * 256 * 2; s.r[i].y += b * W4;
    }
    s.c6 += b * W4; s.s6 += b * 5120 * 2; s.y6 += b * 5120 * W4;
    s.c7 += b * 256 * 40 * d.Wu1; s.s7 += b * 256 * 2; s.y7 += b * 256 * 40 * d.Wu1;
    s.c8 += b * 128 * 80 * d.Wu2; s.s8 += b * 128 * 2; s.y8 += b * 128 * 80 * d.Wu2;
}

static void gen_backward_impl(Exec& ex, const float* const* P, const float* packed, float* const* G, const float* mask, const float* dout,
                              float* dx, int accumulate_dx, const float* stc, float* sc, const GenDims& d, void* const* milestones = nullptr,
                              int stash_B = 0, int stash_b0 = 0)
{
    ex.params = P;
    const GenNet& g = gen_net();
    if (stash_B < d.B) stash_B = d.B;
    GenStash o = gen_stash(gen_dims(stash_B, d.T));
    shift_stash(o, d, stash_b0);
    const GenScratch q = gen_scratch(d);
    float* st = const_cast<float*>(stc);
    const int B = d.B, T = d.T, W2 = d.W2, W4 = d.W4, Wu1 = d.Wu1, Wu2 = d.Wu2;
    const long long BT4 = (long long)B * W4;
    const long long SBT4 = (long long)stash_B * W4;
    const int pxB = stash_B > B ? stash_B : 0;
    if (stash_b0 > 0 && (((long long)stash_b0 * W4) & 3)) { ex.fail(MCVC_ERR_INVALID); return; }
    float* GA = sc + q.ga;
    float* GBs[2] = {sc + q.gb, sc + q.gb2};
    float* DT1s[2] = {sc + q.dt1, sc + q.dt1b};
    float* DT3s[2] = {sc + q.dt3, sc + q.dt3b};
    int gbi = 0;
    auto nextGB = [&]() { gbi ^= 1; return GBs[gbi]; };
    float* GB = GBs[0];
    float* DH = sc + q.dh; float* DT1 = DT1s[0]; float* DT2 = sc + q.dt2; float* DT3 = DT3s[0];
    int ns = 1;
    {
        CView dyv{dout, 80LL * Wu2, 80LL * Wu2, Wu2};
        CView xv{st + o.y8, 128LL * 80 * Wu2, 80LL * Wu2, Wu2};
        conv_wgrad(ex, g.last, G, B, 80, Wu2, xv, dyv);
        conv_bias_grad(ex, g.last, G, B, dyv, 80 * Wu2);
        conv_dgrad(ex, g.last, packed, B, 80, Wu2, dyv, View{GA, 128LL * 80 * Wu2, 80LL * Wu2, Wu2}, (long long)B * 128 * 80 * Wu2, 0, 1, &ns);
    }
    GB = nextGB();
    norm_bwd(ex, st + o.c8, 128LL * 80 * Wu2, 80LL * Wu2, normp(P, G, 102, 103), st + o.s8, GA, 128LL * 80 * Wu2, 80LL * Wu2, Wu2,
             (long long)B * 128 * 80 * Wu2, ns, GB, 512LL * 40 * Wu1, 40LL * Wu1, Wu1, 1, B, 128, 80, Wu2, ACT_SILU);
    {
        CView dyv{GB, 512LL * 40 * Wu1, 40LL * Wu1, Wu1};
        CView xv{st + o.y7, 256LL * 40 * Wu1, 40LL * Wu1, Wu1};
        conv_wgrad(ex, g.up2, G, B, 40, Wu1, xv, dyv);
        conv_bias_grad(ex, g.up2, G, B, dyv, 40 * Wu1);
        conv_dgrad(ex, g.up2, packed, B, 40, Wu1, dyv, View{GA, 256LL * 40 * Wu1, 40LL * Wu1, Wu1}, (long long)B * 256 * 40 * Wu1, 0, 1, &ns);
    }
    GB = nextGB();
    norm_bwd(ex, st + o.c7, 256LL * 40 * Wu1, 40LL * Wu1, normp(P, G, 106, 107), st + o.s7, GA, 256LL * 40 * Wu1, 40LL * Wu1, Wu1,
// ... 663 lines not shown
    if (!n_rows || (net != 0 && net != 1) || (update != 0 && update != 1) || max_batch < 1 || T < 1 || sets < 1 || sets > 3 || (update && sets != 3) ||
        cap < 0 || (cap > 0 && !rows)) return MCVC_ERR_INVALID;
    if (net == 0 ? !gen_range_mask_ok(range_mask) : range_mask != 7) return MCVC_ERR_INVALID;
    const ConvSpec* const* specs = net == 0 ? gen_specs() : disc_specs();
    const int nl = net == 0 ? kMaxLayers : 5, nparams = net == 0 ? MCVC_GEN_NPARAMS : MCVC_DISC_NPARAMS;
    long long cfg = 0;
    PackPlan k;
    if (net == 0) {
        const GenPackCfg q = gen_pack_cfg(max_batch, T);
        cfg = q.fused | q.wino_only << 1 | q.w4 << 2 | q.w43 << 3 | q.up1_w4 << 4 | q.up1_w2 << 5 | q.up2_w2 << 6;
        k = gen_pack_build(q, sets, range_mask, update);
    } else {
        cfg = disc_pack_kind(max_batch, T);
        k = disc_pack_build((int)cfg, update);
    }
    const PackTable t = build_table(k, specs);
    UpdPlan u;
    if (update) {
        long long numel[128] = {};
        net_numel(specs, nl, numel);
        std::vector<char> in_range(nparams, 1);
        if (net == 0) for (int p = 0; p < nparams; ++p) in_range[p] = gen_in_range(range_mask, p);
        if (int e = plan_upd(t, numel, nparams, in_range, covered_params(k, specs), u)) return e;
    }
    const std::vector<PackJob>& jobs = update ? u.jobs : t.jobs;
    PlanRows R{rows, cap};
    R.put({0, net, update, (long long)jobs.size(), (long long)u.owners.size(), (long long)t.dga.size(), update ? u.nblocks : t.nblocks,
           net == 0 ? gen_net().packed_floats : disc_net().packed_floats, dbits(t.bytes), dbits(t.wbytes), cfg, kPlanW});
    for (const PackJob& j : jobs) {
        int layer = -1, form = -1;
        for (int l = 0; l < nl && layer < 0; ++l)
            for (int f = 0; f < kNumForms; ++f) {
                const long long o = specs[l]->off[f];
                if (o >= 0 && kPackForms[f].kind == j.kind && j.dst >= o && j.dst < o + form_floats(*specs[l], (PackForm)f)) { layer = l; form = f; }
            }
        if (layer < 0) return MCVC_ERR_INVALID;
        const long long len = j.kind == PACK_COPY ? j.Cout : form_floats(*specs[layer], (PackForm)form);
        R.put({1, layer, form, j.kind, j.param, j.dst, len, j.block0, j.gx, j.Cout, j.Cin, j.K, j.ld, j.co_off, j.KW, j.taps, j.xi_stride, j.dg});
    }
    for (const UpdOwner& o : u.owners) R.put({2, o.param, o.block0, o.gx, o.Cout, o.Cin, o.taps, o.CB, o.IB, o.e0, o.ne, o.flat, o.vec4});
    std::sort(k.layers.begin(), k.layers.end());
    for (const auto& lf : k.layers) R.put({3, lf.first, sets, lf.second & side_forms(sets)});
    for (size_t i = 0; i < t.dga.size(); ++i) {
        const PackDgradArgs& a = t.dga[i];
        R.put({4, (long long)i, a.Cin, a.KH, a.KW, a.step, a.ld, a.co_off, a.merged, a.mg_kh, a.mg_kw, a.ncls, a.tapmajor, a.cout_rows});
        for (int c = 0; c < a.ncls; ++c) {
            const DgradClass& d = a.cls[c];
            R.put({5, (long long)i, c, d.nth, d.ntw, d.khmax, d.kwmax, d.pad_h, d.pad_w, d.qh, d.qw, d.su, d.sv, d.offset});
        }
    }
    *n_rows = R.n;
    return R.n > cap ? MCVC_ERR_WORKSPACE : 0;
}

int mcvc_grad_store_mask(int net, int T, unsigned char* covered)
{
    if ((net != 0 && net != 1) || T < 1 || !covered) return MCVC_ERR_INVALID;
    memset(covered, 0, 128);
    const ConvSpec* const* specs = net == 0 ? gen_specs() : disc_specs();
    const int nl = net == 0 ? kMaxLayers : 5;
    for (int l = 0; l < nl; ++l) {
        const ConvSpec& c = *specs[l];
        if (!grad_store_covered(c)) continue;
        for (int br = 0; br < c.nbr; ++br) covered[c.wi[br]] = 1;
    }
    return net == 0 ? MCVC_GEN_NPARAMS : MCVC_DISC_NPARAMS;
}

int mcvc_gen_forward(const float* const* params, const float* packed, const float* x, const float* mask, float* out, float* stash,
                     float* scratch, long long scratch_floats, int B, int T, void* stream)
{
    if (B < 1 || T < 1 || !params || !packed || !x || !out || !stash || !scratch) return MCVC_ERR_INVALID;
    const GenDims d = gen_dims(B, T);
    if (d.W4 < 2) return MCVC_ERR_INVALID;
    Exec ex = make_exec(stream, nullptr, scratch, scratch_floats, gen_scratch(d).slabs, gen_needs(B, T));
    if (ex.wslab_cap < 0) return MCVC_ERR_WORKSPACE;
    { const GenScratch q = gen_scratch(d); ex.wv = scratch + q.wv; ex.wm = scratch + q.wm; ex.wino_cap = q.wino_floats;
      ex.sync = reinterpret_cast<unsigned*>(scratch + q.sync); }
    ex.fresh = get_fresh(packed);
    gen_forward_impl(ex, params, packed, x, mask, out, stash, d);
    return ex.err;
}

int mcvc_gen_trunk_fault(float* scratch, int B, int T, int reset, void* stream)
{
    if (!scratch || B < 1 || T < 1) return -MCVC_ERR_INVALID;
    unsigned* w = reinterpret_cast<unsigned*>(scratch + gen_scratch(gen_dims(B, T)).sync) + MCVC_TRUNK_SYNC_WORDS - 1;
    unsigned v = 0;
    hipStream_t s = (hipStream_t)stream;
    if (hipMemcpyAsync(&v, w, sizeof(v), hipMemcpyDeviceToHost, s) != hipSuccess) return -MCVC_ERR_INVALID;
    if (reset && hipMemsetAsync(w, 0, sizeof(v), s) != hipSuccess) return -MCVC_ERR_INVALID;
    if (hipStreamSynchronize(s) != hipSuccess) return -MCVC_ERR_INVALID;
    return (int)(v & 0x7fffffffu);
}
int mcvc_debug_trunk_fault_inject(int on) { return mcvc_trunk_set_fault_inject(on); }
int mcvc_set_trunk_passes_in_flight(int n) { return mcvc_trunk_set_passes_in_flight(n); }

int mcvc_gen_backward_overlap(const float* const* params, const float* packed, float* const* grads, const float* mask, const float* dout,
                              float* dx, int accumulate_dx, const float* stash, float* scratch, long long scratch_floats, int B, int T,
                              void* stream, void* aux_stream, void* const* milestones)
{
    return mcvc_gen_backward_flags(params, packed, grads, mask, dout, dx, accumulate_dx, stash, scratch, scratch_floats, B, T, stream, aux_stream,
                                   milestones, 0);
}

int mcvc_gen_backward_flags(const float* const* params, const float* packed, float* const* grads, const float* mask, const float* dout,
                            float* dx, int accumulate_dx, const float* stash, float* scratch, long long scratch_floats, int B, int T,
                            void* stream, void* aux_stream, void* const* milestones, int flags)
{
    return mcvc_gen_backward_window(params, packed, grads, mask, dout, dx, accumulate_dx, stash, B, 0, scratch, scratch_floats, B, T, stream, aux_stream,
                                    milestones, flags);
}

int mcvc_gen_backward_prefix(const float* const* params, const float* packed, float* const* grads, const float* mask, const float* dout,
                             float* dx, int accumulate_dx, const float* stash, int stash_B, float* scratch, long long scratch_floats, int B, int T,
                             void* stream, void* aux_stream, void* const* milestones, int flags)
{
    return mcvc_gen_backward_window(params, packed, grads, mask, dout, dx, accumulate_dx, stash, stash_B, 0, scratch, scratch_floats, B, T, stream,
                                    aux_stream, milestones, flags);
}

int mcvc_gen_backward_window(const float* const* params, const float* packed, float* const* grads, const float* mask, const float* dout,
                             float* dx, int accumulate_dx, const float* stash, int stash_B, int stash_b0, float* scratch, long long scratch_floats,
                             int B, int T, void* stream, void* aux_stream, void* const* milestones, int flags)
{
    if (B < 1 || T < 1 || stash_b0 < 0 || stash_B < stash_b0 + B || !params || !packed || !dout || !stash || !scratch) return MCVC_ERR_INVALID;
    const GenDims d = gen_dims(B, T);
    if (d.W4 < 2) return MCVC_ERR_INVALID;
    Exec ex = make_exec(stream, aux_stream, scratch, scratch_floats, gen_scratch(d).slabs, gen_needs(B, T));
    if (ex.wslab_cap < 0) return MCVC_ERR_WORKSPACE;
    { const GenScratch q = gen_scratch(d); ex.wv = scratch + q.wv; ex.wm = scratch + q.wm; ex.wino_cap = q.wino_floats;
      ex.wv2 = scratch + q.wv2; ex.wm2 = scratch + q.wm2; ex.wu = scratch + q.wu; ex.wu_cap = q.wu_floats;
      ex.sync = reinterpret_cast<unsigned*>(scratch + q.sync); }
    ex.fresh = get_fresh(packed);
    for (int l = 0; l < kMaxLayers; ++l)
        if (!(ex.fresh.layer[l] & spec_forms(*gen_specs()[l]) & side_forms(PACK_SIDE_BWD))) return MCVC_ERR_INVALID;
    ex.no_join = (flags & 1) && aux_stream;
    ex.fine_ms = (flags & 2) != 0;
    ex.store_grads = (flags & MCVC_BWD_STORE_GRADS) ? 1 : 0;
    gen_backward_impl(ex, params, packed, grads, mask, dout, dx, accumulate_dx, stash, scratch, d, milestones, stash_B, stash_b0);
    return ex.err;
}

int mcvc_gen_backward(const float* const* params, const float* packed, float* const* grads, const float* mask, const float* dout,
                      float* dx, int accumulate_dx, const float* stash, float* scratch, long long scratch_floats, int B, int T, void* stream,
                      void* aux_stream)
{
    return mcvc_gen_backward_overlap(params, packed, grads, mask, dout, dx, accumulate_dx, stash, scratch, scratch_floats, B, T, stream,
                                     aux_stream, nullptr);
}

int mcvc_disc_forward(const float* const* params, const float* packed, const float* x, float* out, float* stash, float* scratch,
                      long long scratch_floats, int B, int T, void* stream)
{
    if (B < 1 || T < 1 || !params || !packed || !x || !out || !stash || !scratch) return MCVC_ERR_INVALID;
    const DiscDims d = disc_dims(B, T);
    Exec ex = make_exec(stream, nullptr, scratch, scratch_floats, disc_scratch(d).slabs, disc_needs(B, T));
    if (ex.wslab_cap < 0) return MCVC_ERR_WORKSPACE;
    ex.fresh = get_fresh(packed);
    ex.fail(mcvc_copy_launch(x, stash + disc_stash(d).total, B * 80 * T, ex.s));
    disc_forward_impl(ex, params, packed, x, out, stash, d);
    return ex.err;
}

int mcvc_disc_backward(const float* const* params, const float* packed, float* const* grads, const float* dout, int dout_is_logit_grad,
                       float* dx, int accumulate_dx, const float* stash, float* scratch, long long scratch_floats, int B, int T, void* stream,
// ... 632 lines not shown
```

### maskcyclegan-vc_amd/csrc/norm_kernels.hip

```cpp
#include "mcvc_common.h"
#include "trace.h"
#include "launch.h"
#include "wino.h"

namespace {

__device__ __forceinline__ float sigmoidf_(float v) { return 1.0f / (1.0f + expf(-v)); }

template <int G>
__device__ __forceinline__ float gsum(float v, float* red)
{
    if constexpr (G <= 64) {
#pragma unroll
        for (int o = G / 2; o > 0; o >>= 1) v += __shfl_xor(v, o, 64);
        return v;
    } else {
#pragma unroll
        for (int o = 32; o > 0; o >>= 1) v += __shfl_xor(v, o, 64);
        __syncthreads();
        if ((threadIdx.x & 63) == 0) red[threadIdx.x >> 6] = v;
        __syncthreads();
        return (red[0] + red[1]) + (red[2] + red[3]);
    }
}

template <int G>
__device__ __forceinline__ void xs_zero_borders(float* y0, int H, int pw, long long plane, int l)
{
    const int per = pw + 4 * (H >> 1);
    for (int i = l; i < 4 * per; i += G) {
        const int pq = i / per, j = i - pq * per;
        float* p = y0 + pq * plane;
        if (j < pw) p[j] = 0.f;
        else { const int r = (j - pw) >> 2, cc = (j - pw) & 3; p[(long long)(r + 1) * pw + cc] = 0.f; }
    }
}
__device__ __forceinline__ long long xs_off(int h, int w, int pw, long long plane)
{
    return (long long)((h & 1) * 2 + (w & 1)) * plane + (long long)((h >> 1) + 1) * pw + (w >> 1) + 4;
}
template <int G>
__device__ __forceinline__ void dyp_zero_borders(float* d0, int H, int W, int pitch, int l)
{
    const int pc = pitch - W, per = H * pc + pitch;
    for (int i = l; i < per; i += G) {
        if (i < H * pc) { const int r = i / pc, cc = i - r * pc; d0[(long long)r * pitch + W + cc] = 0.f; }
        else d0[(long long)H * pitch + (i - H * pc)] = 0.f;
    }
}

template <int G>
__global__ void __launch_bounds__(256) norm_fwd_kernel(const Twin<NormArgs> tw)
{
    const NormArgs a = tw.v[blockIdx.z];
    __shared__ float red[4];
    constexpr int GPB = 256 / G;
    const int g = threadIdx.x / G, l = threadIdx.x % G;
    const long long plane_id = (long long)blockIdx.x * GPB + g;
    if (plane_id >= (long long)a.N * a.C) return;
    const int n = (int)(plane_id / a.C), c = (int)(plane_id - (long long)n * a.C);
    const int P = a.H * a.W;
    const float invP = 1.0f / (float)P;
    const int nbr = (a.act == ACT_GLU) ? 2 : 1;
    const int Cx = a.C * nbr;
    float mean[2] = {0.f, 0.f}, rstd[2] = {0.f, 0.f};
    float* xp[2];
    for (int br = 0; br < nbr; ++br) {
        const int cx = c + br * a.C;
        const long long poff = (long long)n * a.x_sn + (long long)cx * a.x_sc;
        float* x = a.x + poff;
        xp[br] = x;
        float s = 0.f;
        for (int i = l; i < P; i += G) {
            float v = x[i];
            if (a.nslab > 1) {
                for (int sl = 1; sl < a.nslab; ++sl) v += a.x_slabs[(long long)(sl - 1) * a.slab_stride + poff + i];
                x[i] = v;
            }
            s += v;
        }
        s = gsum<G>(s, red);
        const float m = s * invP;
        float q = 0.f;
        for (int i = l; i < P; i += G) { const float d = x[i] - m; q += d * d; }
        q = gsum<G>(q, red);
        const float r = 1.0f / sqrtf(q * invP + a.eps);
// ... 434 lines not shown
        float4 v[2];
        v[1] = make_float4(0.f, 0.f, 0.f, 0.f);
#pragma unroll
        for (int br = 0; br < 2; ++br) {
            if (br < nbr) {
                const long long xo = ((long long)(n * nbr * a.C + c + br * a.C)) * a.P + 4 * i4;
                float4 t = ld4(a.x + xo);
                if (a.nslab > 1) {
                    t = slab_sum4(t, a.x_slabs, a.slab_stride, xo, a.nslab);
                    st4(a.x + xo, t);
                }
                v[br] = t;
            }
        }
        float4 y;
        if (a.act == ACT_GLU) y = make_float4(v[0].x * sigmoidf_(v[1].x), v[0].y * sigmoidf_(v[1].y), v[0].z * sigmoidf_(v[1].z), v[0].w * sigmoidf_(v[1].w));
        else if (a.act == ACT_SILU) y = make_float4(v[0].x * sigmoidf_(v[0].x), v[0].y * sigmoidf_(v[0].y), v[0].z * sigmoidf_(v[0].z), v[0].w * sigmoidf_(v[0].w));
        else if (a.act == ACT_SIGMOID) y = make_float4(sigmoidf_(v[0].x), sigmoidf_(v[0].y), sigmoidf_(v[0].z), sigmoidf_(v[0].w));
        else y = v[0];
        if (a.y) st4(a.y + 4LL * q, y);
    }
}

__global__ void __launch_bounds__(256) act_bwd_vec_kernel(const Twin<ActBwdArgs> tw)
{
    const ActBwdArgs a = tw.v[blockIdx.z];
    const unsigned p4 = (unsigned)a.P >> 2;
    const unsigned total4 = (unsigned)a.N * (unsigned)a.C * p4;
    const int nbr = (a.act == ACT_GLU) ? 2 : 1;
    for (unsigned q = blockIdx.x * 256u + threadIdx.x; q < total4; q += gridDim.x * 256u) {
        const unsigned nc = q / p4, i4 = q - nc * p4;
        const unsigned n = nc / (unsigned)a.C, c = nc - n * (unsigned)a.C;
        float4 d = ld4(a.dy + 4LL * q);
        if (a.nslab > 1) {
            d = slab_sum4(d, a.dy_slabs, a.slab_stride, 4LL * q, a.nslab);
            st4(a.dy + 4LL * q, d);
        }
        const long long xo0 = ((long long)(n * nbr * a.C + c)) * a.P + 4 * i4;
        const float4 x0 = ld4(a.x + xo0);
        const float dv[4] = {d.x, d.y, d.z, d.w}, xv[4] = {x0.x, x0.y, x0.z, x0.w};
        float o0[4], o1[4];
        if (a.act == ACT_GLU) {
            const long long xo1 = xo0 + (long long)a.C * a.P;
            const float4 x1 = ld4(a.x + xo1);
            const float gv[4] = {x1.x, x1.y, x1.z, x1.w};
#pragma unroll
            for (int e = 0; e < 4; ++e) { const float sg = sigmoidf_(gv[e]); o0[e] = dv[e] * sg; o1[e] = dv[e] * xv[e] * sg * (1.0f - sg); }
            st4(a.dx + xo0, make_float4(o0[0], o0[1], o0[2], o0[3]));
            st4(a.dx + xo1, make_float4(o1[0], o1[1], o1[2], o1[3]));
        } else {
#pragma unroll
            for (int e = 0; e < 4; ++e) {
                if (a.act == ACT_SILU) { const float sg = sigmoidf_(xv[e]); o0[e] = dv[e] * (sg * (1.0f + xv[e] * (1.0f - sg))); }
                else if (a.act == ACT_SIGMOID) { const float sg = sigmoidf_(xv[e]); o0[e] = dv[e] * sg * (1.0f - sg); }
                else o0[e] = dv[e];
            }
            st4(a.dx + xo0, make_float4(o0[0], o0[1], o0[2], o0[3]));
        }
    }
}

template <int PTS> struct WinoOutT;
template <> struct WinoOutT<16> { static constexpr int R = 4, S = 2; static constexpr bool SHUF = false;
    static __device__ __forceinline__ void at(const float* m, float* o) { o[0] = m[0] + m[1] + m[2]; o[1] = m[1] - m[2] - m[3]; } };
template <> struct WinoOutT<36> { static constexpr int R = 6, S = 2; static constexpr bool SHUF = true;
    static __device__ __forceinline__ void at(const float* m, float* o) { o[0] = m[0] + m[1] + m[2] + m[3] + m[4]; o[1] = m[1] - m[2] + 2.f * (m[3] - m[4]) + m[5]; } };
template <> struct WinoOutT<43> { static constexpr int R = 6, S = 4; static constexpr bool SHUF = false;
    static __device__ __forceinline__ void at(const float* m, float* o)
    {
        const float s12 = m[1] + m[2], d12 = m[1] - m[2], s34 = m[3] + m[4], d34 = m[3] - m[4];
        o[0] = m[0] + s12 + s34; o[1] = d12 + 2.f * d34; o[2] = s12 + 4.f * s34; o[3] = d12 + 8.f * d34 + m[5];
    } };
template <> struct WinoOutT<64> { static constexpr int R = 8, S = 4; static constexpr bool SHUF = true;
    static __device__ __forceinline__ void at(const float* m, float* o)
    {
        const float s12 = m[1] + m[2], d12 = m[1] - m[2], s34 = m[3] + m[4], d34 = m[3] - m[4], s56 = m[5] + m[6], d56 = m[5] - m[6];
        o[0] = m[0] + s12 + s34 + s56;
        o[1] = d12 + 2.f * d34 + 0.5f * d56;
        o[2] = s12 + 4.f * s34 + 0.25f * s56;
        o[3] = d12 + 8.f * d34 + 0.125f * d56 + m[7];
    } };

struct NormFwdWinoKArgs { NormArgs a; WinoOutArgs w; };
template <int G, int TT, int PTS>
__global__ void __launch_bounds__(256) norm_fwd_wino_kernel(const Twin<NormFwdWinoKArgs> tw)
{
    const NormFwdWinoKArgs ka_ = tw.v[blockIdx.z];
    const NormArgs& a = ka_.a;
    const WinoOutArgs& w = ka_.w;
    __shared__ float red[4];
    using WT = WinoOutT<PTS>;
    constexpr bool SHUF = WT::SHUF;
    constexpr int R = WT::R, S = WT::S, E = S * S;
    constexpr int GPB = 256 / G;
    const int g = threadIdx.x / G, l = threadIdx.x % G;
    const long long plane_id = (long long)blockIdx.x * GPB + g;
    if (plane_id >= (long long)a.N * a.C) return;
    const int n = (int)(plane_id / a.C), c = (int)(plane_id - (long long)n * a.C);
    const int tiles = w.TH * w.TW;
    const int items = SHUF ? 4 * tiles : tiles;
    const int nbr = (!SHUF && a.act == ACT_GLU) ? 2 : 1;
    const int Cx = a.C * nbr;
    const long long xs = (long long)w.Cout * w.NTp;
    const float invP = 1.0f / (float)(a.H * a.W);
    float xv[2][TT][E];
    int pos[TT];
#pragma unroll
    for (int k = 0; k < TT; ++k) {
        const int item = l + k * G;
        const int sub = SHUF ? item / tiles : 0;
        const int t = item - sub * tiles;
        const int ty = t / w.TW, tx = t - ty * w.TW;
        pos[k] = item < items ? (SHUF ? (2 * S * ty + (sub >> 1)) * a.W + 2 * S * tx + (sub & 1) : S * ty * a.W + S * tx) : -1;
#pragma unroll
        for (int br = 0; br < 2; ++br) {
            if (br < nbr) {
                const int co = SHUF ? 4 * c + sub : c + br * a.C;
                float o[E];
#pragma unroll
                for (int e = 0; e < E; ++e) o[e] = 0.f;
                if (item < items) {
                    const float* src = w.m + (long long)co * w.NTp + (long long)n * tiles + t;
                    float u[S][R];
#pragma unroll
                    for (int b = 0; b < R; ++b) {
                        float m[R], q[S];
#pragma unroll
                        for (int aa = 0; aa < R; ++aa) m[aa] = src[(long long)(aa * R + b) * xs];
                        WT::at(m, q);
#pragma unroll
                        for (int i = 0; i < S; ++i) u[i][b] = q[i];
                    }
                    const float bias = w.bias ? w.bias[co] : 0.f;
#pragma unroll
                    for (int i = 0; i < S; ++i) {
                        float q[S];
                        WT::at(u[i], q);
#pragma unroll
                        for (int j = 0; j < S; ++j) o[i * S + j] = q[j] + bias;
                    }
                }
#pragma unroll
                for (int e = 0; e < E; ++e) xv[br][k][e] = o[e];
            }
        }
    }
    const float g0 = a.gamma[0][c], b0 = a.beta[0][c];
    float g1 = 0.f, b1 = 0.f;
    if (nbr == 2) { g1 = a.gamma[1][c]; b1 = a.beta[1][c]; }
    const int dh = (SHUF ? 2 : 1) * a.W, dw = SHUF ? 2 : 1;
    float mean[2] = {0.f, 0.f}, rstd[2] = {0.f, 0.f};
#pragma unroll
    for (int br = 0; br < 2; ++br) {
        if (br < nbr) {
            float s = 0.f;
#pragma unroll
            for (int k = 0; k < TT; ++k) {
                float sk = 0.f;
#pragma unroll
                for (int e = 0; e < E; e += 4) sk += (xv[br][k][e] + xv[br][k][e + 1]) + (xv[br][k][e + 2] + xv[br][k][e + 3]);
                s += sk;
            }
            s = gsum<G>(s, red);
            const float m = s * invP;
            float q = 0.f;
#pragma unroll
            for (int k = 0; k < TT; ++k) {
                if (pos[k] >= 0) {
#pragma unroll
                    for (int e = 0; e < E; ++e) { const float d = xv[br][k][e] - m; q += d * d; }
                }
            }
            q = gsum<G>(q, red);
            const float r = 1.0f / sqrtf(q * invP + a.eps);
            mean[br] = m; rstd[br] = r;
            if (l == 0) {
                float* st = a.stats + ((long long)n * Cx + c + br * a.C) * 2;
                st[0] = m; st[1] = r;
            }
            float* xp = a.x + (long long)n * a.x_sn + (long long)(c + br * a.C) * a.x_sc;
#pragma unroll
            for (int k = 0; k < TT; ++k) {
                if (pos[k] >= 0) {
#pragma unroll
                    for (int e = 0; e < E; ++e) xp[pos[k] + (e / S) * dh + (e % S) * dw] = xv[br][k][e];
                }
            }
        }
    }
    float* yp = a.y + (long long)n * a.y_sn + (long long)c * a.y_sc;
#pragma unroll
    for (int k = 0; k < TT; ++k) {
        if (pos[k] >= 0) {
            const int h0 = pos[k] / a.W, w0 = pos[k] - h0 * a.W;
#pragma unroll
            for (int e = 0; e < E; ++e) {
                const float z0 = (xv[0][k][e] - mean[0]) * rstd[0] * g0 + b0;
                float y;
                if (a.act == ACT_GLU) y = z0 * sigmoidf_((xv[1][k][e] - mean[1]) * rstd[1] * g1 + b1);
                else if (a.act == ACT_SILU) y = z0 * sigmoidf_(z0);
                else y = z0;
                yp[(long long)(h0 + (e / S) * (SHUF ? 2 : 1)) * a.y_sh + w0 + (e % S) * dw] = y;
            }
        }
    }
}

static int pick_group(int P) { return P <= 32 ? 16 : (P <= 640 ? 64 : 256); }

}

static int wino_norm_items(const NormArgs& a, const WinoOutArgs& w, int pts)
{
    if (a.nslab != 1 || a.res != nullptr || w.accumulate || w.N != a.N || (w.OH & 1) || (w.OW & 1) || w.NT != w.N * w.TH * w.TW) return 0;
    if ((pts == 43 || pts == 64) && ((w.OH & 3) || (w.OW & 3))) return 0;
    if (pts == 16 || pts == 43) {
        if (w.shuffle || a.H != w.OH || a.W != w.OW || w.Cout != a.C * (a.act == ACT_GLU ? 2 : 1) || a.x_sc != (long long)a.H * a.W) return 0;
        return w.TH * w.TW;
    }
    if (pts == 36 || pts == 64) {
        if (!w.shuffle || a.act == ACT_GLU || a.H != 2 * w.OH || a.W != 2 * w.OW || w.Cout != 4 * a.C || a.x_sc != (long long)a.H * a.W) return 0;
        return 4 * w.TH * w.TW;
    }
    return 0;
}
static int wino_norm_max_items(int pts) { return (pts == 43 || pts == 64) ? 320 : 1280; }

bool mcvc_norm_fwd_wino_applies(const NormArgs& a, const WinoOutArgs& w, int pts)
{
    const int items = wino_norm_items(a, w, pts);
    return items > 0 && items <= wino_norm_max_items(pts);
}

int mcvc_norm_fwd_wino_launch(const NormArgs& a, const WinoOutArgs& w, int pts, hipStream_t s)
{
    const int items = wino_norm_items(a, w, pts);
    if (items <= 0 || items > wino_norm_max_items(pts)) return MCVC_ERR_INVALID;
    const long long planes = (long long)a.N * a.C;
    const int nbr = ((pts == 16 || pts == 43) && a.act == ACT_GLU) ? 2 : 1;
    const double el = (double)planes * a.H * a.W * nbr;
    const double m_per_out = pts == 16 ? 4.0 : (pts == 36 ? 9.0 : (pts == 43 ? 2.25 : 4.0));
    TraceScope ts(K_NORM_FWD, s, 0.0, 4.0 * (el * m_per_out + el + (double)planes * a.H * a.W));
#define MCVC_FWD_WINO(GG, TT) { \
        if (pts == 16) mcvc_launch((norm_fwd_wino_kernel<GG, TT, 16>), dim3((unsigned)cdiv_ll(planes, 256 / GG)), dim3(256), 0, s, NormFwdWinoKArgs{a, w}); \
        else if (pts == 36) mcvc_launch((norm_fwd_wino_kernel<GG, TT, 36>), dim3((unsigned)cdiv_ll(planes, 256 / GG)), dim3(256), 0, s, NormFwdWinoKArgs{a, w}); \
        else if (pts == 43) mcvc_launch((norm_fwd_wino_kernel<GG, TT, 43>), dim3((unsigned)cdiv_ll(planes, 256 / GG)), dim3(256), 0, s, NormFwdWinoKArgs{a, w}); \
        else mcvc_launch((norm_fwd_wino_kernel<GG, TT, 64>), dim3((unsigned)cdiv_ll(planes, 256 / GG)), dim3(256), 0, s, NormFwdWinoKArgs{a, w}); \
        return (int)hipGetLastError(); }
    if (pts == 43 || pts == 64) {
        if (items <= 64) MCVC_FWD_WINO(64, 1)
        if (items <= 128) MCVC_FWD_WINO(64, 2)
        if (items <= 256 && planes < 2048) MCVC_FWD_WINO(256, 1)
        if (items <= 512) MCVC_FWD_WINO(256, 2)
        MCVC_FWD_WINO(64, 5)
    }
    if (items <= 128) MCVC_FWD_WINO(64, 2)
    if (items <= 512 && planes < 2048) MCVC_FWD_WINO(256, 2)
    if (items <= 320) MCVC_FWD_WINO(64, 5)
    MCVC_FWD_WINO(256, 5)
#undef MCVC_FWD_WINO
}

int mcvc_norm_fwd_launch(const NormArgs& a, hipStream_t s)
{
    const int P = a.H * a.W;
    const long long planes = (long long)a.N * a.C;
    const int G = pick_group(P);
    const unsigned blocks = (unsigned)cdiv_ll(planes, 256 / G);
    const double el = (double)planes * P * (a.act == ACT_GLU ? 2 : 1);
    TraceScope ts(K_NORM_FWD, s, 0.0, 4.0 * (el * (a.nslab + 1) + (double)planes * P));
#define MCVC_FWD_REG(GG, EE) { mcvc_launch((norm_fwd_reg_kernel<GG, EE>), dim3((unsigned)cdiv_ll(planes, 256 / GG)), dim3(256), 0, s, a); return (int)hipGetLastError(); }
    if (P <= 16) MCVC_FWD_REG(16, 1)
    if (P <= 64) MCVC_FWD_REG(16, 4)
    if (P <= 128) MCVC_FWD_REG(64, 2)
    if (P <= 320) MCVC_FWD_REG(64, 5)
    if (P <= 1280) MCVC_FWD_REG(256, 5)
    if (P <= 5120) MCVC_FWD_REG(256, 20)
#undef MCVC_FWD_REG
    if (G == 16) mcvc_launch(norm_fwd_kernel<16>, dim3(blocks), dim3(256), 0, s, a);
    else if (G == 64) mcvc_launch(norm_fwd_kernel<64>, dim3(blocks), dim3(256), 0, s, a);
    else mcvc_launch(norm_fwd_kernel<256>, dim3(blocks), dim3(256), 0, s, a);
    return (int)hipGetLastError();
}

int mcvc_norm_bwd_launch(const NormBwdArgs& a, hipStream_t s)
{
    const int P = a.H * a.W;
    const int G = pick_group(P);
    const unsigned blocks = (unsigned)cdiv_i(a.C, 256 / G);
    const double el = (double)a.N * a.C * P;
    TraceScope ts(K_NORM_BWD, s, 0.0, 4.0 * el * ((a.act == ACT_GLU ? 4 : 2) + a.nslab));
    auto chunks = [&](int cblocks) {
        int nc = 1;
        if (!mcvc_deterministic())
            while (2 * nc <= a.N && nc < 32 && cblocks * nc < 768) nc *= 2;
        return nc;
    };
#define MCVC_BWD_REG(GG, EE) { const int cb = cdiv_i(a.C, 256 / GG); mcvc_launch((norm_bwd_reg_kernel<GG, EE>), dim3((unsigned)cb, (unsigned)chunks(cb)), dim3(256), 0, s, a); return (int)hipGetLastError(); }
    if (P <= 16) MCVC_BWD_REG(16, 1)
    if (P <= 64) MCVC_BWD_REG(16, 4)
    if (P <= 128) MCVC_BWD_REG(64, 2)
    if (P <= 320) MCVC_BWD_REG(64, 5)
    if (P <= 1280) MCVC_BWD_REG(256, 5)
    if (P <= 5120) MCVC_BWD_REG(256, 20)
#undef MCVC_BWD_REG
    if (G == 16) mcvc_launch(norm_bwd_kernel<16>, dim3(blocks), dim3(256), 0, s, a);
    else if (G == 64) mcvc_launch(norm_bwd_kernel<64>, dim3(blocks), dim3(256), 0, s, a);
    else mcvc_launch(norm_bwd_kernel<256>, dim3(blocks), dim3(256), 0, s, a);
    return (int)hipGetLastError();
}

static unsigned ew_blocks(long long total)
{
    long long b = cdiv_ll(total, 256);
    if (b > 4096) b = 4096;
    if (b < 1) b = 1;
    return (unsigned)b;
}

int mcvc_act_fwd_launch(const ActArgs& a, hipStream_t s)
{
    TraceScope ts(K_ACT_FWD, s, 0.0, 4.0 * (double)a.N * a.C * a.P * ((a.act == ACT_GLU ? 2 : 1) * a.nslab + 1));
    const long long total = (long long)a.N * a.C * a.P;
    const bool al = ((((uintptr_t)a.x | (uintptr_t)a.x_slabs | (uintptr_t)a.y) & 15) == 0) && (a.slab_stride & 3) == 0;
    if ((a.P & 3) == 0 && al && total < (1LL << 33)) mcvc_launch(act_fwd_vec_kernel, dim3(ew_blocks(total >> 2)), dim3(256), 0, s, a);
    else mcvc_launch(act_fwd_kernel, dim3(ew_blocks(total)), dim3(256), 0, s, a);
    return (int)hipGetLastError();
}

int mcvc_act_bwd_launch(const ActBwdArgs& a, hipStream_t s)
{
    TraceScope ts(K_ACT_BWD, s, 0.0, 4.0 * (double)a.N * a.C * a.P * ((a.act == ACT_GLU ? 4 : 2) + a.nslab));
    const long long total = (long long)a.N * a.C * a.P;
    const bool al = ((((uintptr_t)a.x | (uintptr_t)a.dy | (uintptr_t)a.dy_slabs | (uintptr_t)a.dx) & 15) == 0) && (a.slab_stride & 3) == 0;
    if ((a.P & 3) == 0 && al && total < (1LL << 33)) mcvc_launch(act_bwd_vec_kernel, dim3(ew_blocks(total >> 2)), dim3(256), 0, s, a);
    else mcvc_launch(act_bwd_kernel, dim3(ew_blocks(total)), dim3(256), 0, s, a);
    return (int)hipGetLastError();
}
```

### maskcyclegan-vc_amd/csrc/wino.h

```cpp
#pragma once
#include <hip/hip_runtime.h>

struct WinoXformArgs {
    const float* x; long long x_sb, x_sc; int x_sh;
    float* v;
    int N, C, H, W;
    int TH, TW, NT;
    int NTp;
    int pad;
};

struct WinoOutArgs {
    const float* m;
    const float* bias;
    float* y; long long y_sb, y_sc; int y_sh;
    int N, Cout, OH, OW, TH, TW, NT, NTp;
    int shuffle, YH, YW;
    int accumulate;
};

int mcvc_wino_input_launch(const WinoXformArgs& a, hipStream_t s);
struct NormArgs;
bool mcvc_norm_fwd_wino_applies(const NormArgs& a, const WinoOutArgs& w, int pts);
int mcvc_norm_fwd_wino_launch(const NormArgs& a, const WinoOutArgs& w, int pts, hipStream_t s);
int mcvc_wino3_input_launch(const WinoXformArgs& a, hipStream_t s);
int mcvc_wino3_output_launch(const WinoOutArgs& a, hipStream_t s);
int mcvc_wino3_input_phase_launch(const WinoXformArgs& a, int XH, int XW, hipStream_t s);
int mcvc_wino3_input_phase_t_launch(const WinoXformArgs& a, int XH, int XW, hipStream_t s);
int mcvc_wino3_dy_t_launch(const WinoXformArgs& a, hipStream_t s);
int mcvc_wino3_dw_launch(const float* du, float* dw0, float* dw1, int Cout, int nbr, int Cin, int store, hipStream_t s);
int mcvc_wino_input_t_launch(const WinoXformArgs& a, hipStream_t s);
int mcvc_wino_dy_t_launch(const WinoXformArgs& a, hipStream_t s);
int mcvc_wino_dw_launch(const float* du, float* dw, int Cout, int Cin, int store, hipStream_t s);
int mcvc_wino_output_launch(const WinoOutArgs& a, hipStream_t s);
static __device__ __forceinline__ void wino_weight_core(const float* g, float* dst, int co, int ci, int ld, long long xi_stride, int co_off, int dgrad)
{
    float gg[5][5];
#pragma unroll
    for (int k = 0; k < 5; ++k)
#pragma unroll
        for (int l = 0; l < 5; ++l) gg[k][l] = dgrad ? g[(4 - k) * 5 + (4 - l)] : g[k * 5 + l];
    auto grow = [](const float v[5], float o[6]) {
        const float s_even = v[0] + v[2] + v[4], s_odd = v[1] + v[3];
        o[0] = 0.25f * v[0];
        o[1] = -(s_even + s_odd) * (1.0f / 6.0f);
        o[2] = -(s_even - s_odd) * (1.0f / 6.0f);
        const float e2 = v[0] * (1.0f / 24.0f) + v[2] * (1.0f / 6.0f) + v[4] * (2.0f / 3.0f);
        const float o2 = v[1] * (1.0f / 12.0f) + v[3] * (1.0f / 3.0f);
        o[3] = e2 + o2;
        o[4] = e2 - o2;
        o[5] = v[4];
    };
    float t[5][6];
#pragma unroll
    for (int k = 0; k < 5; ++k) grow(gg[k], t[k]);
    const long long row = dgrad ? (co_off + co) : ci;
    const long long col = dgrad ? ci : (co_off + co);
    float* d0 = dst + row * ld + col;
#pragma unroll
    for (int b = 0; b < 6; ++b) {
        float colv[5], o[6];
#pragma unroll
        for (int k = 0; k < 5; ++k) colv[k] = t[k][b];
        grow(colv, o);
#pragma unroll
        for (int aa = 0; aa < 6; ++aa) d0[(long long)(aa * 6 + b) * xi_stride] = o[aa];
    }
}
static __device__ __forceinline__ void wino_weight_tile(const float* w, float* dst, int Cout, int Cin, int ld, long long xi_stride, int co_off, int dgrad, int bx, int by)
{
    const int a_idx = bx * 256 + threadIdx.x;
    const int b_idx = by;
    const int co = dgrad ? b_idx : a_idx, ci = dgrad ? a_idx : b_idx;
    if (co >= Cout || ci >= Cin) return;
    wino_weight_core(w + ((long long)co * Cin + ci) * 25, dst, co, ci, ld, xi_stride, co_off, dgrad);
}


struct WinoGemmArgs {
    const float* a; long long a_xi; int lda;
    const float* b; long long b_xi; int ldb;
    float* c; long long c_xi; int ldc;
    int M, N, K;
    int nxi;
    int nt, mt;
    int mgroup;
};
int mcvc_wino_gemm_launch(const WinoGemmArgs& a, hipStream_t s);

template <int P>
static __device__ __forceinline__ void wino_g3(float v0, float v1, float v2, float* o)
{
    if constexpr (P == 4) { o[0] = v0; o[1] = 0.5f * (v0 + v1 + v2); o[2] = 0.5f * (v0 - v1 + v2); o[3] = v2; }
    else {
        const float e = v0 + v2, e2 = v0 * (1.0f / 24.0f) + v2 * (1.0f / 6.0f);
        o[0] = 0.25f * v0; o[1] = -(e + v1) * (1.0f / 6.0f); o[2] = -(e - v1) * (1.0f / 6.0f);
        o[3] = e2 + v1 * (1.0f / 12.0f); o[4] = e2 - v1 * (1.0f / 12.0f); o[5] = v2;
    }
}

template <int P>
static __device__ __forceinline__ void wino3_weight_core_p(const float* g, float* dst, int co, int ci, int ld, long long xi_stride, int co_off)
{
    float gg[5][5];
#pragma unroll
    for (int k = 0; k < 25; ++k) gg[k / 5][k % 5] = g[k];
#pragma unroll
// ... 82 lines not shown
```

### maskcyclegan-vc_amd/csrc/wino4.h

```cpp
#pragma once
#include <hip/hip_runtime.h>
#include "wino.h"

__device__ constexpr float kW4AT[4][8] = {
    {1.f, 1.f, 1.f, 1.f, 1.f, 1.f, 1.f, 0.f},
    {0.f, 1.f, -1.f, 2.f, -2.f, 0.5f, -0.5f, 0.f},
    {0.f, 1.f, 1.f, 4.f, 4.f, 0.25f, 0.25f, 0.f},
    {0.f, 1.f, -1.f, 8.f, -8.f, 0.125f, -0.125f, 1.f}};
__device__ constexpr float kW4G[8][5] = {
    {-1.f, 0.f, 0.f, 0.f, 0.f},
    {-2.f / 9.f, -2.f / 9.f, -2.f / 9.f, -2.f / 9.f, -2.f / 9.f},
    {-2.f / 9.f, 2.f / 9.f, -2.f / 9.f, 2.f / 9.f, -2.f / 9.f},
    {1.f / 90.f, 1.f / 45.f, 2.f / 45.f, 4.f / 45.f, 8.f / 45.f},
    {1.f / 90.f, -1.f / 45.f, 2.f / 45.f, -4.f / 45.f, 8.f / 45.f},
    {32.f / 45.f, 16.f / 45.f, 8.f / 45.f, 4.f / 45.f, 2.f / 45.f},
    {32.f / 45.f, -16.f / 45.f, 8.f / 45.f, -4.f / 45.f, 2.f / 45.f},
    {0.f, 0.f, 0.f, 0.f, 1.f}};
__device__ constexpr float kW4BT[8][8] = {
    {-1.f, 0.f, 5.25f, 0.f, -5.25f, 0.f, 1.f, 0.f},
    {0.f, 1.f, 1.f, -4.25f, -4.25f, 1.f, 1.f, 0.f},
    {0.f, -1.f, 1.f, 4.25f, -4.25f, -1.f, 1.f, 0.f},
    {0.f, 0.5f, 0.25f, -2.5f, -1.25f, 2.f, 1.f, 0.f},
    {0.f, -0.5f, 0.25f, 2.5f, -1.25f, -2.f, 1.f, 0.f},
    {0.f, 2.f, 4.f, -2.5f, -5.f, 0.5f, 1.f, 0.f},
    {0.f, -2.f, 4.f, 2.5f, -5.f, -0.5f, 1.f, 0.f},
    {0.f, -1.f, 0.f, 5.25f, 0.f, -5.25f, 0.f, 1.f}};

int mcvc_wino4_input_launch(const WinoXformArgs& a, hipStream_t s);
int mcvc_wino4_output_launch(const WinoOutArgs& a, hipStream_t s);
int mcvc_wino4_input_t_launch(const WinoXformArgs& a, hipStream_t s);
int mcvc_wino4_dy_t_launch(const WinoXformArgs& a, hipStream_t s);
int mcvc_wino4_dw_launch(const float* du, float* dw, int Cout, int Cin, int store, hipStream_t s);

static __device__ __forceinline__ void wino4_weight_core(const float* g, float* dst, int co, int ci, int ld, long long xi_stride, int co_off, int dgrad)
{
    float t[5][8];
#pragma unroll
    for (int k = 0; k < 5; ++k) {
        float gr[5];
#pragma unroll
        for (int l = 0; l < 5; ++l) gr[l] = dgrad ? g[(4 - k) * 5 + (4 - l)] : g[k * 5 + l];
#pragma unroll
        for (int b = 0; b < 8; ++b) {
            float acc = 0.f;
#pragma unroll
            for (int l = 0; l < 5; ++l) acc += gr[l] * kW4G[b][l];
            t[k][b] = acc;
        }
    }
    const long long row = dgrad ? (co_off + co) : ci;
    const long long col = dgrad ? ci : (co_off + co);
    float* d0 = dst + row * ld + col;
#pragma unroll
    for (int aa = 0; aa < 8; ++aa)
#pragma unroll
        for (int b = 0; b < 8; ++b) {
            float acc = 0.f;
#pragma unroll
            for (int k = 0; k < 5; ++k) acc += kW4G[aa][k] * t[k][b];
            d0[(long long)(aa * 8 + b) * xi_stride] = acc;
        }
}
static __device__ __forceinline__ void wino4_weight_tile(const float* w, float* dst, int Cout, int Cin, int ld, long long xi_stride, int co_off, int dgrad, int bx, int by)
{
    const int a_idx = bx * 256 + threadIdx.x, b_idx = by;
    const int co = dgrad ? b_idx : a_idx, ci = dgrad ? a_idx : b_idx;
    if (co >= Cout || ci >= Cin) return;
    wino4_weight_core(w + ((long long)co * Cin + ci) * 25, dst, co, ci, ld, xi_stride, co_off, dgrad);
}
```

### maskcyclegan-vc_amd/csrc/wino4_kernels.hip

```cpp
#include "mcvc_common.h"
#include "trace.h"
#include "launch.h"
#include "wino4.h"

namespace {

__device__ __forceinline__ void w4_bt(const float d[8], float o[8])
{
    const float e1 = d[2] - 4.25f * d[4] + d[6], o1 = d[1] - 4.25f * d[3] + d[5];
    const float e2 = 0.25f * d[2] - 1.25f * d[4] + d[6], o2 = 0.5f * d[1] - 2.5f * d[3] + 2.f * d[5];
    const float e3 = 4.f * d[2] - 5.f * d[4] + d[6], o3 = 2.f * d[1] - 2.5f * d[3] + 0.5f * d[5];
    o[0] = (d[6] - d[0]) + 5.25f * (d[2] - d[4]);
    o[1] = e1 + o1; o[2] = e1 - o1;
    o[3] = e2 + o2; o[4] = e2 - o2;
    o[5] = e3 + o3; o[6] = e3 - o3;
    o[7] = (d[7] - d[1]) + 5.25f * (d[3] - d[5]);
}
__device__ __forceinline__ void w4_at(const float m[8], float o[4])
{
    const float s12 = m[1] + m[2], d12 = m[1] - m[2], s34 = m[3] + m[4], d34 = m[3] - m[4], s56 = m[5] + m[6], d56 = m[5] - m[6];
    o[0] = m[0] + s12 + s34 + s56;
    o[1] = d12 + 2.f * d34 + 0.5f * d56;
    o[2] = s12 + 4.f * s34 + 0.25f * s56;
    o[3] = d12 + 8.f * d34 + 0.125f * d56 + m[7];
}
__device__ __forceinline__ void w4_a(const float d[4], float o[8])
{
    const float e = d[0] + d[2], f = d[1] + d[3];
    const float e4 = d[0] + 4.f * d[2], f4 = 2.f * d[1] + 8.f * d[3];
    const float eh = d[0] + 0.25f * d[2], fh = 0.5f * d[1] + 0.125f * d[3];
    o[0] = d[0]; o[1] = e + f; o[2] = e - f; o[3] = e4 + f4; o[4] = e4 - f4; o[5] = eh + fh; o[6] = eh - fh; o[7] = d[3];
}

__device__ __forceinline__ void w4_input(const float* src, int x_sh, int ih0, int iw0, int H, int W, float* o)
{
    float t[8][8];
    const float* rp = src + (long long)ih0 * x_sh + iw0;
    if (ih0 >= 0 && ih0 + 7 < H && iw0 >= 0 && iw0 + 7 < W) {
#pragma unroll
        for (int i = 0; i < 8; ++i) {
            float d[8];
#pragma unroll
            for (int j = 0; j < 8; ++j) d[j] = rp[j];
            rp += x_sh;
            w4_bt(d, t[i]);
        }
    } else {
#pragma unroll
        for (int i = 0; i < 8; ++i) {
            float d[8];
            const int ih = ih0 + i;
            const bool rok = (ih >= 0) && (ih < H);
#pragma unroll
            for (int j = 0; j < 8; ++j) {
                const int iw = iw0 + j;
                d[j] = (rok && iw >= 0 && iw < W) ? rp[j] : 0.f;
            }
            rp += x_sh;
            w4_bt(d, t[i]);
        }
    }
#pragma unroll
    for (int b = 0; b < 8; ++b) {
        float col[8], q[8];
#pragma unroll
        for (int i = 0; i < 8; ++i) col[i] = t[i][b];
        w4_bt(col, q);
#pragma unroll
        for (int aa = 0; aa < 8; ++aa) o[aa * 8 + b] = q[aa];
    }
}

__device__ __forceinline__ void w4_dy(const float* src, int x_sh, int oh0, int ow0, int H, int W, float* o)
{
    float t[8][4];
    float dy[4][4];
#pragma unroll
    for (int i = 0; i < 4; ++i)
#pragma unroll
        for (int j = 0; j < 4; ++j) dy[i][j] = (oh0 + i < H && ow0 + j < W) ? src[(long long)(oh0 + i) * x_sh + ow0 + j] : 0.f;
#pragma unroll
    for (int j = 0; j < 4; ++j) {
        const float col[4] = {dy[0][j], dy[1][j], dy[2][j], dy[3][j]};
        float q[8];
        w4_a(col, q);
#pragma unroll
        for (int aa = 0; aa < 8; ++aa) t[aa][j] = q[aa];
    }
#pragma unroll
    for (int aa = 0; aa < 8; ++aa) w4_a(t[aa], o + aa * 8);
}

__global__ void __launch_bounds__(256) wino4_input_kernel(const Twin<WinoXformArgs> tw)
{
    const WinoXformArgs a = tw.v[blockIdx.z];
    const int tile = blockIdx.x * 256 + threadIdx.x;
    const int c = blockIdx.y;
    if (tile >= a.NT) return;
    const int per = a.TH * a.TW;
    const int n = tile / per, r = tile - n * per;
    const int ty = r / a.TW, tx = r - ty * a.TW;
    float o[64];
    w4_input(a.x + (long long)n * a.x_sb + (long long)c * a.x_sc, a.x_sh, 4 * ty - a.pad, 4 * tx - a.pad, a.H, a.W, o);
    float* dst = a.v + (long long)c * a.NTp + tile;
    const long long xs = (long long)a.C * a.NTp;
#pragma unroll
    for (int q = 0; q < 64; ++q) dst[(long long)q * xs] = o[q];
}

__global__ void __launch_bounds__(256) wino4_output_kernel(const Twin<WinoOutArgs> tw)
{
    const WinoOutArgs a = tw.v[blockIdx.z];
    const int tile = blockIdx.x * 256 + threadIdx.x;
    const int co = blockIdx.y;
    if (tile >= a.NT) return;
    const int per = a.TH * a.TW;
    const int n = tile / per, r = tile - n * per;
    const int ty = r / a.TW, tx = r - ty * a.TW;
    const float* src = a.m + (long long)co * a.NTp + tile;
    const long long xs = (long long)a.Cout * a.NTp;
    float u[4][8];
#pragma unroll
    for (int b = 0; b < 8; ++b) {
        float col[8];
#pragma unroll
        for (int aa = 0; aa < 8; ++aa) col[aa] = src[(long long)(aa * 8 + b) * xs];
        float q[4];
        w4_at(col, q);
#pragma unroll
        for (int i = 0; i < 4; ++i) u[i][b] = q[i];
    }
    const float bias = a.bias ? a.bias[co] : 0.f;
    float* yn = a.y + (long long)n * a.y_sb;
#pragma unroll
    for (int i = 0; i < 4; ++i) {
        float row[4];
        w4_at(u[i], row);
#pragma unroll
        for (int j = 0; j < 4; ++j) {
            const float acc = row[j] + bias;
            const int oh = 4 * ty + i, ow = 4 * tx + j;
            if (oh >= a.OH || ow >= a.OW) continue;
            long long off;
            if (a.shuffle) {
                const int yh = 2 * oh + ((co >> 1) & 1), yw = 2 * ow + (co & 1);
                if (yh >= a.YH || yw >= a.YW) continue;
                off = (long long)(co >> 2) * a.y_sc + (long long)yh * a.y_sh + yw;
            } else {
                off = (long long)co * a.y_sc + (long long)oh * a.y_sh + ow;
            }
            if (a.accumulate) yn[off] += acc; else yn[off] = acc;
        }
    }
// ... 129 lines not shown
```

### maskcyclegan-vc_amd/csrc/wino_kernels.hip

```cpp
#include "mcvc_common.h"
#include "trace.h"
#include "launch.h"
#include "wino.h"

namespace {

__device__ __forceinline__ void bt6(const float d[6], float o[6])
{
    o[0] = 4.f * d[0] - 5.f * d[2] + d[4];
    o[1] = -4.f * (d[1] + d[2]) + d[3] + d[4];
    o[2] = 4.f * (d[1] - d[2]) - d[3] + d[4];
    o[3] = -2.f * d[1] - d[2] + 2.f * d[3] + d[4];
    o[4] = 2.f * d[1] - d[2] - 2.f * d[3] + d[4];
    o[5] = 4.f * d[1] - 5.f * d[3] + d[5];
}

__global__ void __launch_bounds__(256) wino_input_kernel(const Twin<WinoXformArgs> tw)
{
    const WinoXformArgs a = tw.v[blockIdx.z];
    const int tile = blockIdx.x * 256 + threadIdx.x;
    const int c = blockIdx.y;
    if (tile >= a.NT) return;
    const int per = a.TH * a.TW;
    const int n = tile / per, r = tile - n * per;
    const int ty = r / a.TW, tx = r - ty * a.TW;
    const int ih0 = 2 * ty - a.pad, iw0 = 2 * tx - a.pad;
    const float* src = a.x + (long long)n * a.x_sb + (long long)c * a.x_sc;
    float t[6][6];
#pragma unroll
    for (int i = 0; i < 6; ++i) {
        float d[6];
        const int ih = ih0 + i;
        const bool rok = (ih >= 0) && (ih < a.H);
#pragma unroll
        for (int j = 0; j < 6; ++j) {
            const int iw = iw0 + j;
            d[j] = (rok && iw >= 0 && iw < a.W) ? src[(long long)ih * a.x_sh + iw] : 0.f;
        }
        bt6(d, t[i]);
    }
    float* dst = a.v + (long long)c * a.NTp + tile;
    const long long xs = (long long)a.C * a.NTp;
#pragma unroll
    for (int b = 0; b < 6; ++b) {
        float col[6], o[6];
#pragma unroll
        for (int i = 0; i < 6; ++i) col[i] = t[i][b];
        bt6(col, o);
#pragma unroll
        for (int aa = 0; aa < 6; ++aa) dst[(long long)(aa * 6 + b) * xs] = o[aa];
    }
}

__device__ __forceinline__ void bt4(const float d[4], float o[4])
{
    o[0] = d[0] - d[2]; o[1] = d[1] + d[2]; o[2] = d[2] - d[1]; o[3] = d[1] - d[3];
}

__global__ void __launch_bounds__(256) wino3_input_kernel(const Twin<WinoXformArgs> tw)
{
    const WinoXformArgs a = tw.v[blockIdx.z];
    const int tile = blockIdx.x * 256 + threadIdx.x;
    const int c = blockIdx.y;
    if (tile >= a.NT) return;
    const int per = a.TH * a.TW;
    const int n = tile / per, r = tile - n * per;
    const int ty = r / a.TW, tx = r - ty * a.TW;
    const int ih0 = 2 * ty - a.pad, iw0 = 2 * tx - a.pad;
    const float* src = a.x + (long long)n * a.x_sb + (long long)c * a.x_sc;
    float t[4][4];
#pragma unroll
    for (int i = 0; i < 4; ++i) {
        float d[4];
        const int ih = ih0 + i;
        const bool rok = (ih >= 0) && (ih < a.H);
#pragma unroll
        for (int j = 0; j < 4; ++j) {
            const int iw = iw0 + j;
            d[j] = (rok && iw >= 0 && iw < a.W) ? src[(long long)ih * a.x_sh + iw] : 0.f;
        }
        bt4(d, t[i]);
    }
    float* dst = a.v + (long long)c * a.NTp + tile;
    const long long xs = (long long)a.C * a.NTp;
#pragma unroll
    for (int b = 0; b < 4; ++b) {
        float col[4], o[4];
#pragma unroll
        for (int i = 0; i < 4; ++i) col[i] = t[i][b];
        bt4(col, o);
#pragma unroll
        for (int aa = 0; aa < 4; ++aa) dst[(long long)(aa * 4 + b) * xs] = o[aa];
    }
}

struct Wino3InputPhaseKArgs { WinoXformArgs a; int XH; int XW; };
__global__ void __launch_bounds__(256) wino3_input_phase_kernel(const Twin<Wino3InputPhaseKArgs> tw)
{
    const Wino3InputPhaseKArgs ka_ = tw.v[blockIdx.z];
    const WinoXformArgs& a = ka_.a;
    int XH = ka_.XH;
    int XW = ka_.XW;
    const int tile = blockIdx.x * 256 + threadIdx.x;
    const int k = blockIdx.y;
    if (tile >= a.NT) return;
    const int ci = k >> 2, p = (k >> 1) & 1, q = k & 1;
    const int per = a.TH * a.TW;
    const int n = tile / per, r = tile - n * per;
    const int ty = r / a.TW, tx = r - ty * a.TW;
    const int i0 = 2 * ty - 1, j0 = 2 * tx - 1;
    const float* src = a.x + (long long)n * a.x_sb + (long long)ci * a.x_sc;
    float t[4][4];
#pragma unroll
    for (int i = 0; i < 4; ++i) {
        float d[4];
        const int ih = 2 * (i0 + i) + p;
        const bool rok = (i0 + i >= 0) && (ih < XH);
#pragma unroll
        for (int j = 0; j < 4; ++j) {
            const int iw = 2 * (j0 + j) + q;
            d[j] = (rok && j0 + j >= 0 && iw < XW) ? src[(long long)ih * a.x_sh + iw] : 0.f;
        }
        bt4(d, t[i]);
    }
    float* dst = a.v + (long long)k * a.NTp + tile;
    const long long xs = (long long)a.C * a.NTp;
#pragma unroll
    for (int b = 0; b < 4; ++b) {
        float col[4], o[4];
#pragma unroll
        for (int i = 0; i < 4; ++i) col[i] = t[i][b];
        bt4(col, o);
#pragma unroll
        for (int aa = 0; aa < 4; ++aa) dst[(long long)(aa * 4 + b) * xs] = o[aa];
    }
}


__device__ __forceinline__ void a42(float d0, float d1, float o[4]) { o[0] = d0; o[1] = d0 + d1; o[2] = d0 - d1; o[3] = -d1; }


struct Wino3DwKArgs { const float* du; float* dw0; float* dw1; int Cout; int nbr; int Cin; };
template <bool STORE>
__global__ void __launch_bounds__(256) wino3_dw_kernel(const Twin<Wino3DwKArgs> tw)
{
    const Wino3DwKArgs ka_ = tw.v[blockIdx.z];
    const float* __restrict__ du = ka_.du;
    float* __restrict__ dw0 = ka_.dw0;
    float* __restrict__ dw1 = ka_.dw1;
    int Cout = ka_.Cout;
    int nbr = ka_.nbr;
    int Cin = ka_.Cin;
    const int k = blockIdx.x * 256 + threadIdx.x, co = blockIdx.y;
    const int K = 4 * Cin;
    if (k >= K) return;
    const long long xs = (long long)Cout * nbr * K;
    const float* src = du + (long long)co * K + k;
    auto gt3 = [](const float v[4], float o[3]) {
        o[0] = v[0] + 0.5f * (v[1] + v[2]); o[1] = 0.5f * (v[1] - v[2]); o[2] = 0.5f * (v[1] + v[2]) + v[3];
    };
    float t[3][4];
#pragma unroll
    for (int b = 0; b < 4; ++b) {
        float col[4], o[3];
#pragma unroll
        for (int aa = 0; aa < 4; ++aa) col[aa] = src[(long long)(aa * 4 + b) * xs];
        gt3(col, o);
#pragma unroll
        for (int u = 0; u < 3; ++u) t[u][b] = o[u];
    }
    const int ci = k >> 2, p = (k >> 1) & 1, q = k & 1;
    float* dw = (co < Cout) ? dw0 : dw1;
    const int col = (co < Cout) ? co : co - Cout;
    if (!dw) return;
    float* dst = dw + ((long long)col * Cin + ci) * 25;
    float r[3][3], old[3][3];
#pragma unroll
    for (int u = 0; u < 3; ++u) gt3(t[u], r[u]);
#pragma unroll
    for (int u = 0; u < 3; ++u)
#pragma unroll
        for (int v = 0; v < 3; ++v) {
            const int kh = 2 * u + p, kw = 2 * v + q;
            old[u][v] = (!STORE && kh <= 4 && kw <= 4) ? dst[kh * 5 + kw] : 0.f;
        }
#pragma unroll
    for (int u = 0; u < 3; ++u)
#pragma unroll
        for (int v = 0; v < 3; ++v) {
            const int kh = 2 * u + p, kw = 2 * v + q;
            if (kh <= 4 && kw <= 4) dst[kh * 5 + kw] = STORE ? r[u][v] : old[u][v] + r[u][v];
        }
}

__global__ void __launch_bounds__(256) wino3_output_kernel(const Twin<WinoOutArgs> tw)
{
    const WinoOutArgs a = tw.v[blockIdx.z];
    const int tile = blockIdx.x * 256 + threadIdx.x;
    const int co = blockIdx.y;
    if (tile >= a.NT) return;
    const int per = a.TH * a.TW;
    const int n = tile / per, r = tile - n * per;
    const int ty = r / a.TW, tx = r - ty * a.TW;
    const float* src = a.m + (long long)co * a.NTp + tile;
    const long long xs = (long long)a.Cout * a.NTp;
    float u[2][4];
#pragma unroll
    for (int b = 0; b < 4; ++b) {
        float m[4];
#pragma unroll
        for (int aa = 0; aa < 4; ++aa) m[aa] = src[(long long)(aa * 4 + b) * xs];
        u[0][b] = m[0] + m[1] + m[2];
        u[1][b] = m[1] - m[2] - m[3];
    }
    const float bias = a.bias ? a.bias[co] : 0.f;
    float* yn = a.y + (long long)n * a.y_sb;
#pragma unroll
    for (int i = 0; i < 2; ++i) {
// ... 670 lines not shown
```

### maskcyclegan-vc_amd/mask_cyclegan_vc/_hip.py

```python
from __future__ import annotations

import ctypes
import os
from ctypes import c_double, c_float, c_int, c_longlong, c_void_p

import torch

_HERE = os.path.dirname(os.path.abspath(__file__))
LIB_PATH = os.environ.get("MCVC_LIB") or os.path.join(os.path.dirname(_HERE), "lib", "libmcvc_hip.so")

ABI_VERSION = 3
GEN_NPARAMS = 110
DISC_NPARAMS = 20
N_MEL = 80

_lib = None

_PP = ctypes.POINTER(c_void_p)

_SIGS = {
    "mcvc_version": (c_int, []),
    "mcvc_set_deterministic": (c_int, [c_int]),
    "mcvc_get_deterministic": (c_int, []),
    "mcvc_set_precise": (c_int, [c_int]),
    "mcvc_get_precise": (c_int, []),
    "mcvc_set_trunk_persistent": (c_int, [c_int]),
    "mcvc_twin_begin": (c_int, []),
    "mcvc_twin_switch": (c_int, []),
    "mcvc_twin_end": (c_int, []),
    "mcvc_twin_launches": (c_int, []),
    "mcvc_gen_packed_floats": (c_longlong, []),
    "mcvc_disc_packed_floats": (c_longlong, []),
    "mcvc_gen_stash_floats": (c_longlong, [c_int, c_int]),
    "mcvc_gen_scratch_floats": (c_longlong, [c_int, c_int]),
    "mcvc_disc_stash_floats": (c_longlong, [c_int, c_int]),
    "mcvc_disc_scratch_floats": (c_longlong, [c_int, c_int]),
    "mcvc_gen_out_frames": (c_int, [c_int]),
    "mcvc_disc_out_frames": (c_int, [c_int]),
    "mcvc_gen_pack": (c_int, [_PP, c_void_p, c_void_p]),
    "mcvc_gen_trunk_fused": (c_int, [c_int, c_int]),
    "mcvc_gen_pack_small_batch": (c_int, [_PP, c_void_p, c_int, c_int, c_void_p]),
    "mcvc_gen_pack_sets": (c_int, [_PP, c_void_p, c_int, c_int, c_int, c_void_p]),
    "mcvc_gen_pack_ranges": (c_int, [_PP, c_void_p, c_int, c_int, c_int, c_int, c_void_p]),
    "mcvc_disc_pack": (c_int, [_PP, c_void_p, c_void_p]),
    "mcvc_disc_pack_small": (c_int, [_PP, c_void_p, c_int, c_void_p]),
    "mcvc_disc_pack_batch": (c_int, [_PP, c_void_p, c_int, c_int, c_void_p]),
    "mcvc_gen_forward": (c_int, [_PP, c_void_p, c_void_p, c_void_p, c_void_p, c_void_p, c_void_p, c_longlong, c_int, c_int, c_void_p]),
    "mcvc_gen_backward": (c_int, [_PP, c_void_p, _PP, c_void_p, c_void_p, c_void_p, c_int, c_void_p, c_void_p, c_longlong, c_int, c_int, c_void_p, c_void_p]),
    "mcvc_gen_backward_overlap": (c_int, [_PP, c_void_p, _PP, c_void_p, c_void_p, c_void_p, c_int, c_void_p, c_void_p, c_longlong, c_int, c_int,
                                          c_void_p, c_void_p, _PP]),
    "mcvc_gen_backward_flags": (c_int, [_PP, c_void_p, _PP, c_void_p, c_void_p, c_void_p, c_int, c_void_p, c_void_p, c_longlong, c_int, c_int,
                                        c_void_p, c_void_p, _PP, c_int]),
    "mcvc_gen_backward_prefix": (c_int, [_PP, c_void_p, _PP, c_void_p, c_void_p, c_void_p, c_int, c_void_p, c_int, c_void_p, c_longlong, c_int, c_int,
                                         c_void_p, c_void_p, _PP, c_int]),
    "mcvc_gen_backward_window": (c_int, [_PP, c_void_p, _PP, c_void_p, c_void_p, c_void_p, c_int, c_void_p, c_int, c_int, c_void_p, c_longlong, c_int, c_int,
                                         c_void_p, c_void_p, _PP, c_int]),
    "mcvc_set_trunk_passes_in_flight": (c_int, [c_int]),
    "mcvc_gen_trunk_persistent": (c_int, [c_int, c_int]),
    "mcvc_gen_trunk_fault": (c_int, [c_void_p, c_int, c_int, c_int, c_void_p]),
    "mcvc_debug_trunk_fault_inject": (c_int, [c_int]),
    "mcvc_gen_bf16_packed_bytes": (c_longlong, []),
    "mcvc_gen_bf16_workspace_bytes": (c_longlong, [c_int, c_int]),
    "mcvc_gen_bf16_pack": (c_int, [_PP, c_void_p, c_void_p]),
    "mcvc_gen_infer_bf16": (c_int, [_PP, c_void_p, c_void_p, c_void_p, c_void_p, c_void_p, c_longlong, c_int, c_int, c_void_p]),
    "mcvc_bf16_conv2d_pack_bytes": (c_longlong, [c_int, c_int, c_int, c_int]),
    "mcvc_bf16_conv2d": (c_int, [c_void_p] * 5 + [c_int] * 10 + [c_void_p]),
    "mcvc_bf16_instnorm_act": (c_int, [c_void_p] * 8 + [c_int] * 6 + [c_void_p]),
    "mcvc_bf16_c2d1d_pack_bytes": (c_longlong, []),
    "mcvc_bf16_c2d1d_norm": (c_int, [c_void_p] * 6 + [c_int] * 2 + [c_void_p]),
    "mcvc_bf16_trunk_layer_pack_bytes": (c_longlong, [c_int] * 3),
    "mcvc_bf16_trunk_layer": (c_int, [c_void_p] * 10 + [c_int] * 4 + [c_void_p]),
    "mcvc_bf16_last_conv_pack_bytes": (c_longlong, []),
    "mcvc_bf16_last_conv": (c_int, [c_void_p] * 5 + [c_int] * 2 + [c_void_p]),
    "mcvc_bf16_conv1_glu_pack_bytes": (c_longlong, []),
    "mcvc_bf16_conv1_glu": (c_int, [c_void_p] * 8 + [c_int] * 2 + [c_void_p]),
    "mcvc_disc_forward": (c_int, [_PP, c_void_p, c_void_p, c_void_p, c_void_p, c_void_p, c_longlong, c_int, c_int, c_void_p]),
    "mcvc_disc_backward": (c_int, [_PP, c_void_p, _PP, c_void_p, c_int, c_void_p, c_int, c_void_p, c_void_p, c_longlong, c_int, c_int, c_void_p, c_void_p]),
    "mcvc_disc_backward_flags": (c_int, [_PP, c_void_p, _PP, c_void_p, c_int, c_void_p, c_int, c_void_p, c_void_p, c_longlong, c_int, c_int, c_void_p, c_void_p,
                                         c_int]),
    "mcvc_grad_store_mask": (c_int, [c_int, c_int, c_void_p]),
    "mcvc_l1_loss": (c_int, [c_void_p, c_void_p, c_longlong, c_float, c_void_p, c_void_p, c_void_p, c_int, c_void_p]),
    "mcvc_lsgan_loss": (c_int, [c_void_p, c_longlong, c_float, c_float, c_void_p, c_void_p, c_void_p, c_void_p]),
    "mcvc_loss_combine": (c_int, [c_void_p, c_int, c_void_p, c_void_p, c_void_p, c_void_p]),
    "mcvc_adam_step": (c_int, [c_void_p, c_void_p, c_void_p, c_void_p, c_longlong, c_float, c_float, c_float, c_float, c_int, c_float, c_void_p]),
    "mcvc_adam_step2": (c_int, [c_void_p, c_void_p, c_void_p, c_int, c_void_p, c_void_p, c_longlong, c_float, c_float, c_float, c_float, c_int, c_float, c_void_p]),
    "mcvc_gen_update_ranges": (c_int, [_PP, c_void_p, c_void_p, c_int, c_int, c_int, c_void_p, c_void_p, c_void_p, c_void_p, c_void_p,
                                       c_float, c_float, c_float, c_float, c_int, c_float, c_int, c_void_p]),
    "mcvc_disc_update_batch": (c_int, [_PP, c_void_p, c_void_p, c_int, c_int, c_void_p, c_void_p, c_void_p, c_void_p, c_void_p,
                                       c_float, c_float, c_float, c_float, c_int, c_float, c_int, c_void_p]),
    "mcvc_pack_plan": (c_int, [c_int, c_int, c_int, c_int, c_int, c_int, c_void_p, c_int, c_void_p]),
    "mcvc_draw_batch": (c_int, [c_void_p, c_void_p, c_int, c_longlong, c_void_p, c_void_p, c_int, c_longlong, c_int, c_int, c_int,
                                ctypes.c_ulonglong, ctypes.c_ulonglong, c_void_p, c_void_p, c_void_p, c_void_p, c_void_p, c_void_p]),
    "mcvc_audio_frames": (c_int, [c_int]),
    "mcvc_audio_basis_floats": (c_longlong, []),
    "mcvc_audio_basis_init": (c_int, [c_void_p]),
    "mcvc_audio_plan": (c_int, [c_void_p, c_int, c_void_p, c_void_p, c_int, ctypes.POINTER(c_int)]),
    "mcvc_audio_log_mel": (c_int, [c_void_p, c_longlong, c_void_p, c_int, c_void_p, c_void_p, c_longlong, c_void_p]),
    "mcvc_voc_out_samples": (c_int, [c_int]),
    "mcvc_voc_launches": (c_int, []),
    "mcvc_voc_packed_floats": (c_longlong, []),
    "mcvc_voc_pack": (c_int, [_PP, c_void_p]),
    "mcvc_voc_workspace_floats": (c_longlong, [c_int, c_int]),
    "mcvc_voc_decode": (c_int, [c_void_p, c_void_p, c_void_p, c_void_p, c_longlong, c_int, c_int, c_void_p]),
    "mcvc_voc_layer_packed_floats": (c_longlong, [c_int] * 5),
    "mcvc_voc_layer_pack": (c_int, [c_int] + [c_void_p] * 5 + [c_int] * 4),
    "mcvc_voc_layer": (c_int, [c_int] + [c_void_p] * 4 + [c_int] * 8 + [c_void_p]),
    "mcvc_gl_out_samples": (c_int, [c_int]),
    "mcvc_gl_launches": (c_int, [c_int]),
    "mcvc_gl_tables_floats": (c_longlong, []),
    "mcvc_gl_tables_init": (c_int, [c_void_p, c_void_p]),
    "mcvc_gl_workspace_floats": (c_longlong, [c_int, c_int]),
    "mcvc_gl_decode": (c_int, [c_void_p, c_int, c_void_p, c_void_p, c_void_p, c_void_p, c_longlong, c_int, c_int, c_int, c_float, c_void_p]),
    "mcvc_melinv_max_iter": (c_int, []),
    "mcvc_melinv_tables_floats": (c_longlong, []),
    "mcvc_melinv_tables_init": (c_int, [c_void_p, c_void_p, c_double, c_void_p]),
    "mcvc_melinv_solve": (c_int, [c_void_p, c_void_p, c_void_p, c_int, c_int, c_int, c_void_p]),
    "mcvc_dtw_max_frames": (c_int, []),
    "mcvc_dtw_launches": (c_int, [c_int]),
    "mcvc_cep_basis_init": (c_int, [c_int, c_void_p]),
    "mcvc_cep_project": (c_int, [c_void_p, c_longlong, c_void_p, c_int, c_void_p, c_void_p]),
    "mcvc_dtw_plan": (c_int, [c_void_p, c_void_p, c_int, c_int, c_void_p, ctypes.POINTER(c_longlong), ctypes.POINTER(c_longlong)]),
    "mcvc_dtw_run": (c_int, [c_void_p, c_longlong, c_void_p, c_longlong, c_int, c_float, c_void_p, c_void_p, c_void_p, c_int, c_void_p, c_void_p,
                             c_void_p, c_void_p, c_longlong, c_void_p]),
    "mcvc_f0_max_lag": (c_int, []),
    "mcvc_f0_launches": (c_int, [c_int]),
    "mcvc_f0_track": (c_int, [c_void_p, c_longlong, c_void_p, c_int, c_int, c_int, c_float, c_void_p, c_void_p, c_void_p, c_longlong, c_void_p]),
    "mcvc_f0_stats": (c_int, [c_void_p, c_longlong, c_void_p, c_longlong, c_void_p, c_void_p, c_int, c_void_p, c_void_p, c_void_p]),
    "mcvc_ms_max_fft": (c_int, []),
    "mcvc_ms_launches": (c_int, []),
    "mcvc_ms_table_init": (c_int, [c_int, c_void_p]),
    "mcvc_ms_power": (c_int, [c_void_p, c_longlong, c_int, c_void_p, c_int, c_void_p, c_int, c_void_p, c_void_p, c_void_p, c_void_p, c_void_p]),
    "mcvc_ms_mean_log": (c_int, [c_void_p, c_int, c_longlong, c_float, c_void_p, c_void_p]),
    "mcvc_ms_distance": (c_int, [c_void_p, c_void_p, c_int, c_int, c_int, c_void_p, c_void_p, c_void_p]),
    "mcvc_axpy": (c_int, [c_void_p, c_void_p, c_float, c_longlong, c_void_p]),
    "mcvc_conv2d_pack_floats": (c_longlong, [c_int, c_int, c_int, c_int]),
    "mcvc_conv2d_forward": (c_int, [c_void_p] * 6 + [c_int] * 12 + [c_void_p]),
    "mcvc_conv2d_dgrad": (c_int, [c_void_p] * 5 + [c_int] * 11 + [c_void_p]),
    "mcvc_conv2d_wgrad_slab_floats": (c_longlong, [c_int] * 10),
    "mcvc_conv2d_wgrad": (c_int, [c_void_p] * 4 + [c_longlong] + [c_int] * 10 + [c_void_p]),
    "mcvc_layer_packed_floats": (c_longlong, [c_int] * 8),
    "mcvc_layer_scratch_floats": (c_longlong, [c_int] * 11),
    "mcvc_layer_pack": (c_int, [c_void_p] * 5 + [c_int] * 8 + [c_void_p]),
    "mcvc_layer_forward": (c_int, [c_void_p] * 6 + [c_longlong] + [c_int] * 13 + [c_void_p]),
    "mcvc_layer_dgrad": (c_int, [c_void_p] * 6 + [c_longlong] + [c_int] * 12 + [c_void_p]),
    "mcvc_layer_wgrad": (c_int, [c_void_p] * 5 + [c_longlong] + [c_int] * 12 + [c_void_p]),
    "mcvc_layer_wgrad_flags": (c_int, [c_void_p] * 5 + [c_longlong] + [c_int] * 13 + [c_void_p]),
    "mcvc_trunk_layer_backward": (c_int, [c_void_p] * 19 + [c_int] * 5 + [c_void_p]),
    "mcvc_instnorm_act_forward": (c_int, [c_void_p] * 8 + [c_int] * 5 + [c_void_p]),
    "mcvc_instnorm_act_backward": (c_int, [c_void_p] * 12 + [c_int] * 5 + [c_void_p]),
    "mcvc_trunk_layer_forward": (c_int, [c_void_p] * 13 + [c_int] * 5 + [c_void_p]),
    "mcvc_batched_gemm": (c_int, [c_void_p] * 3 + [c_int] * 7 + [c_longlong] * 3 + [c_void_p]),
    "mcvc_bias_grad": (c_int, [c_void_p, c_void_p, c_int, c_int, c_int, c_void_p]),
    "mcvc_act_forward": (c_int, [c_void_p, c_void_p, c_int, c_int, c_int, c_int, c_void_p]),
    "mcvc_act_backward": (c_int, [c_void_p, c_void_p, c_void_p, c_int, c_int, c_int, c_int, c_void_p]),
    "mcvc_fif_input": (c_int, [c_void_p, c_void_p, c_void_p, c_int, c_int, c_void_p]),
    "mcvc_fif_input_grad": (c_int, [c_void_p, c_void_p, c_void_p, c_int, c_int, c_int, c_void_p]),
    "mcvc_trace_enable": (c_int, [c_int]),
    "mcvc_trace_kinds": (c_int, []),
    "mcvc_trace_kind_name": (ctypes.c_char_p, [c_int]),
    "mcvc_trace_collect": (c_int, [ctypes.POINTER(ctypes.c_double)]),
    "mcvc_trace_collect_raw": (c_int, [ctypes.POINTER(ctypes.c_double), c_int]),
}

EXPORTED_SYMBOLS = tuple(_SIGS)


def lib():
    global _lib
    if _lib is None:
        if not os.path.exists(LIB_PATH):
            raise RuntimeError(
                "libmcvc_hip.so not found at %s -- build it with `python -c 'import __graft_entry__ as g; g.build()'` "
                "(hipcc --offload-arch=gfx950). There is no CPU fallback." % LIB_PATH)
# ... 86 lines not shown
```

Baseline: 181.7.

## Fuse next conv's Winograd input transform into norm/activation forward epilogue

Norm and activation forward kernels can now write the Winograd input transform (V) for the following convolution directly, and that conv's pass skips its separate input-transform launch when the cached arguments match. This removes one kernel launch and one read of the activation tensor per fused boundary in the generator forward. By default only one boundary class (bit F1) is enabled. It adds matching state to the executor, and a stale or mismatched V would give wrong results.

```diff
diff --git a/include/mcvc.h b/include/mcvc.h
--- a/include/mcvc.h
+++ b/include/mcvc.h
@@ -125,6 +125,9 @@
                            float beta2, float eps, int step, float grad_scale, int zero_grads, void* stream);
 
 int mcvc_pack_plan(int net, int max_batch, int T, int sets, int range_mask, int update, long long* rows, int cap, int* n_rows);
+#define MCVC_XFORM_BOUNDARIES 6
+int mcvc_set_fuse_wino_xform(int v);
+int mcvc_gen_xform_fusion_plan(int B, int T, int* fused, int* planned);
 int mcvc_axpy(float* y, const float* x, float alpha, long long n, void* stream);
 
 int mcvc_draw_batch(const float* bank_A, const int* offs_A, int n_A, long long frames_A, const float* bank_B, const int* offs_B, int n_B,
diff --git a/maskcyclegan-vc_amd/csrc/net.hip b/maskcyclegan-vc_amd/csrc/net.hip
--- a/maskcyclegan-vc_amd/csrc/net.hip
+++ b/maskcyclegan-vc_amd/csrc/net.hip
@@ -35,6 +35,8 @@
 struct CView { const float* p; long long sb, sc; int sh; };
 static inline CView cv(const View& v) { return CView{v.p, v.sb, v.sc, v.sh}; }
 
+struct NextConv { const ConvSpec* c; const float* packed; int NB, H, W; CView x; int shuffle; int bit; };
+
 constexpr int kMaxLayers = 20;
 struct PackFresh { unsigned layer[kMaxLayers]; PackFresh() { for (unsigned& m : layer) m = kAllForms; } };
 
@@ -63,6 +65,8 @@
     int fuse_next = 0;
     const struct WinoFam* pend_fam = nullptr;
     WinoOutArgs pend;
+    const NextConv* next_conv = nullptr;
+    struct { int valid; const struct WinoFam* f; WinoXformArgs xi; int XH, XW; } v_ready{};
     int y_xs_pw = 0; long long y_xs_plane = 0;
     int dx_pitch = 0;
     int wgrad_x_xs = 0;
@@ -276,6 +280,35 @@
     int shuffle, YH, YW, accumulate;
     bool may_defer;
 };
+static WinoXformArgs wino_xi(const Exec& ex, const WinoPass& p, CView x, int b0, int nb)
+{
+    const WinoFam& f = *p.f;
+    const int TH = (p.H + f.tile - 1) / f.tile, TW = (p.W + f.tile - 1) / f.tile;
+    const long long NT = (long long)nb * TH * TW, NTp = std::max<long long>((NT + 31) & ~31LL, f.min_pitch);
+    WinoXformArgs xi{};
+    xi.x = x.p + (long long)b0 * x.sb; xi.x_sb = x.sb; xi.x_sc = x.sc; xi.x_sh = x.sh; xi.v = ex.wv;
+    xi.N = nb; xi.C = p.K; xi.H = p.H; xi.W = p.W; xi.TH = TH; xi.TW = TW; xi.NT = (int)NT; xi.NTp = (int)NTp; xi.pad = f.pad;
+    return xi;
+}
+static bool same_xi(const WinoXformArgs& a, const WinoXformArgs& b)
+{
+    return a.x == b.x && a.x_sb == b.x_sb && a.x_sc == b.x_sc && a.x_sh == b.x_sh && a.v == b.v && a.N == b.N && a.C == b.C && a.H == b.H && a.W == b.W &&
+           a.TH == b.TH && a.TW == b.TW && a.NT == b.NT && a.NTp == b.NTp && a.pad == b.pad;
+}
+static bool wino_defers(const Exec& ex, const WinoPass& p) { return p.may_defer && ex.fuse_next && p.nbc == p.NB; }
+static WinoOutArgs wino_oa(const Exec& ex, const WinoPass& p, View y, int b0, int nb)
+{
+    const WinoFam& f = *p.f;
+    const int TH = (p.H + f.tile - 1) / f.tile, TW = (p.W + f.tile - 1) / f.tile;
+    const long long NT = (long long)nb * TH * TW, NTp = std::max<long long>((NT + 31) & ~31LL, f.min_pitch);
+    WinoOutArgs oa{};
+    oa.m = ex.wm; oa.bias = p.bias;
+    oa.y = y.p + (long long)b0 * y.sb; oa.y_sb = y.sb; oa.y_sc = y.sc; oa.y_sh = y.sh;
+    oa.N = nb; oa.Cout = p.M; oa.OH = p.H; oa.OW = p.W; oa.TH = TH; oa.TW = TW; oa.NT = (int)NT; oa.NTp = (int)NTp;
+    oa.shuffle = p.shuffle; oa.YH = p.YH; oa.YW = p.YW; oa.accumulate = p.accumulate;
+    return oa;
+}
+
 static void wino_pass(Exec& ex, const WinoPass& p, CView x, View y)
 {
     const WinoFam& f = *p.f;
@@ -283,10 +316,11 @@
     for (int b0 = 0; b0 < p.NB; b0 += p.nbc) {
         const int nb = p.NB - b0 < p.nbc ? p.NB - b0 : p.nbc;
         const long long NT = (long long)nb * TH * TW, NTp = std::max<long long>((NT + 31) & ~31LL, f.min_pitch);
-        WinoXformArgs xi{};
-        xi.x = x.p + (long long)b0 * x.sb; xi.x_sb = x.sb; xi.x_sc = x.sc; xi.x_sh = x.sh; xi.v = ex.wv;
-        xi.N = nb; xi.C = K; xi.H = p.H; xi.W = p.W; xi.TH = TH; xi.TW = TW; xi.NT = (int)NT; xi.NTp = (int)NTp; xi.pad = f.pad;
-        ex.fail(p.XH ? f.input_phase(xi, p.XH, p.XW, ex.s) : f.input(xi, ex.s));
+        const WinoXformArgs xi = wino_xi(ex, p, x, b0, nb);
+        const bool have_v = ex.v_ready.valid && ex.v_ready.f == &f && ex.v_ready.XH == p.XH && ex.v_ready.XW == p.XW && p.nbc == p.NB &&
+                            same_xi(ex.v_ready.xi, xi);
+        ex.v_ready.valid = 0;
+        if (!have_v) ex.fail(p.XH ? f.input_phase(xi, p.XH, p.XW, ex.s) : f.input(xi, ex.s));
         static const int own_gemm = mcvc_knob("MCVC_WINO_GEMM", 1);
         if (&f != &kWino[kF25] || (own_gemm && (M % 128) == 0 && (K % 16) == 0 && NTp >= 64)) {
             WinoGemmArgs ga{};
@@ -306,12 +340,8 @@
             io.gemm_ok = 1;
             ex.fail(mcvc_conv_launch(cp, 36, io, p.a, p.a_rows, p.lda, nullptr, ex.s, nullptr));
         }
-        WinoOutArgs oa{};
-        oa.m = ex.wm; oa.bias = p.bias;
-        oa.y = y.p + (long long)b0 * y.sb; oa.y_sb = y.sb; oa.y_sc = y.sc; oa.y_sh = y.sh;
-        oa.N = nb; oa.Cout = M; oa.OH = p.H; oa.OW = p.W; oa.TH = TH; oa.TW = TW; oa.NT = (int)NT; oa.NTp = (int)NTp;
-        oa.shuffle = p.shuffle; oa.YH = p.YH; oa.YW = p.YW; oa.accumulate = p.accumulate;
-        if (p.may_defer && ex.fuse_next && p.nbc == p.NB) { ex.pend = oa; ex.pend_fam = &f; }
+        const WinoOutArgs oa = wino_oa(ex, p, y, b0, nb);
+        if (wino_defers(ex, p)) { ex.pend = oa; ex.pend_fam = &f; }
         else ex.fail(f.output(oa, ex.s));
     }
 }
@@ -343,39 +373,47 @@
     }
 }
 
-static bool conv_wino(Exec& ex, const ConvSpec& c, const float* packed, int dgrad, int NB, int H, int W, CView x, View y, int shuffle,
-                      int accumulate)
-{
-    if (!c.wino || !wino_enabled() || !ex.wv) return false;
+enum { kPlanNo, kPlanDone, kPlanPass };
+static int plan_wino(Exec& ex, const ConvSpec& c, const float* packed, int dgrad, int NB, int H, int W, int shuffle, int accumulate, bool probe,
+                     WinoPass& p)
+{
+    if (!c.wino || !wino_enabled() || !ex.wv) return kPlanNo;
     const int K = dgrad ? c.cout_tot : c.Cin, M = dgrad ? c.Cin : c.cout_tot;
     const WinoFam* f = &kWino[kF45];
     int nbc = 0;
     if (wino4_applies(ex, c, NB, H, W) && (M % 128) == 0 && (K % 16) == 0) nbc = wino_nbc(ex, *f, NB, wino_tiles(*f, H, W), K > M ? K : M, wino4_min_tiles());
     if (!nbc) {
-        if (stale(ex, c, wino_form(false, dgrad))) return true;
+        if (probe ? !is_fresh(ex, c, wino_form(false, dgrad)) : stale(ex, c, wino_form(false, dgrad))) return probe ? kPlanNo : kPlanDone;
         f = &kWino[kF25];
         nbc = wino_nbc(ex, *f, NB, wino_tiles(*f, H, W), K > M ? K : M, 0);
     }
-    if (!nbc) return false;
-    if (ex.dry) return true;
+    if (!nbc) return kPlanNo;
+    if (ex.dry) return kPlanDone;
     const bool four = f->tile == 4;
-    WinoPass p{};
+    p = WinoPass{};
     p.f = f; p.K = K; p.M = M; p.NB = NB; p.nbc = nbc; p.H = H; p.W = W;
     const PackForm form = wino_form(four, dgrad);
     p.a = packed + c.off[form]; p.a_xi = form_xi(c, form); p.lda = kPackForms[form].ld(c); p.a_rows = dgrad ? c.dg_rows_co : c.cin_pad;
     p.bias = dgrad ? nullptr : packed + c.off[PF_BIAS];
     p.shuffle = shuffle; p.YH = 2 * H; p.YW = 2 * W; p.accumulate = accumulate;
     p.may_defer = !dgrad && shuffle;
-    wino_pass(ex, p, x, y);
-    return true;
-}
-
-static bool conv_wino3(Exec& ex, const ConvSpec& c, const float* packed, int dgrad, int NB, int H, int W, CView x, View y, int accumulate)
-{
-    if (!c.wino3 || !wino_enabled() || !ex.wv) return false;
-    if (!dgrad && ((H & 1) != 0 || (W & 1) != 0 || (c.cout_tot % 128) != 0)) return false;
+    return kPlanPass;
+}
+static bool conv_wino(Exec& ex, const ConvSpec& c, const float* packed, int dgrad, int NB, int H, int W, CView x, View y, int shuffle,
+                      int accumulate)
+{
+    WinoPass p{};
+    const int r = plan_wino(ex, c, packed, dgrad, NB, H, W, shuffle, accumulate, false, p);
+    if (r == kPlanPass) wino_pass(ex, p, x, y);
+    return r != kPlanNo;
+}
+
+static int plan_wino3(Exec& ex, const ConvSpec& c, const float* packed, int dgrad, int NB, int H, int W, int accumulate, WinoPass& p)
+{
+    if (!c.wino3 || !wino_enabled() || !ex.wv) return kPlanNo;
+    if (!dgrad && ((H & 1) != 0 || (W & 1) != 0 || (c.cout_tot % 128) != 0)) return kPlanNo;
     static const int en[2] = {mcvc_knob("MCVC_WINO3_FWD", 1), mcvc_knob("MCVC_WINO3", 1)};
-    if (!en[dgrad]) return false;
+    if (!en[dgrad]) return kPlanNo;
     const int OH = conv_out(H, c.KH, c.stride, c.ph), OW = conv_out(W, c.KW, c.stride, c.pw);
     const int K = dgrad ? c.cout_tot : 4 * c.Cin, M = dgrad ? 4 * c.Cin : c.cout_tot;
     const WinoFam* f = &kWino[kF43];
@@ -385,10 +423,10 @@
         f = &kWino[kF23];
         nbc = wino_nbc(ex, *f, NB, wino_tiles(*f, OH, OW), K > M ? K : M, 64);
     }
-    if (!nbc) return false;
-    if (ex.dry) return true;
+    if (!nbc) return kPlanNo;
+    if (ex.dry) return kPlanDone;
     const bool four = f->tile == 4;
-    WinoPass p{};
+    p = WinoPass{};
     p.f = f; p.K = K; p.M = M; p.NB = NB; p.nbc = nbc; p.H = OH; p.W = OW;
     const PackForm form = wino3_form(four, dgrad);
     p.a = packed + c.off[form]; p.a_xi = form_xi(c, form); p.lda = kPackForms[form].ld(c);
@@ -400,8 +438,20 @@
         p.YH = OH; p.YW = OW;
         p.may_defer = true;
     }
-    wino_pass(ex, p, x, y);
-    return true;
+    return kPlanPass;
+}
+static bool conv_wino3(Exec& ex, const ConvSpec& c, const float* packed, int dgrad, int NB, int H, int W, CView x, View y, int accumulate)
+{
+    WinoPass p{};
+    const int r = plan_wino3(ex, c, packed, dgrad, NB, H, W, accumulate, p);
+    if (r == kPlanPass) wino_pass(ex, p, x, y);
+    return r != kPlanNo;
+}
+static int plan_conv_fwd_wino(Exec& ex, const ConvSpec& c, const float* packed, int NB, int H, int W, int shuffle, bool probe, WinoPass& p)
+{
+    int r = plan_wino(ex, c, packed, 0, NB, H, W, shuffle, 0, probe, p);
+    if (r == kPlanNo && !shuffle) r = plan_wino3(ex, c, packed, 0, NB, H, W, 0, p);
+    return r;
 }
 
 struct SgKind { int kind, taps, OH, OW; };
@@ -511,8 +561,8 @@
     ex.fail(mcvc_igemm_launch(g, ex.s));
 }
 
-static void conv_fwd(Exec& ex, const ConvSpec& c, const float* packed, int NB, int H, int W, CView x, View y, long long y_total,
-                     int shuffle, int allow_split, int* nsplit)
+static void conv_fwd_run(Exec& ex, const ConvSpec& c, const float* packed, int NB, int H, int W, CView x, View y, long long y_total,
+                         int shuffle, int allow_split, int* nsplit)
 {
     const SgKind sk = shuffle ? SgKind{0, 0, 0, 0} : sgemm_kind(c, NB, H, W);
     if (sk.kind) {
@@ -551,7 +601,12 @@
             return;
         }
     }
-    if (conv_wino(ex, c, packed, 0, NB, H, W, x, y, shuffle, 0) || (!shuffle && conv_wino3(ex, c, packed, 0, NB, H, W, x, y, 0))) { if (nsplit) *nsplit = 1; return; }
+    {
+        WinoPass wp{};
+        const int r = plan_conv_fwd_wino(ex, c, packed, NB, H, W, shuffle, false, wp);
+        if (r == kPlanPass) wino_pass(ex, wp, x, y);
+        if (r != kPlanNo) { if (nsplit) *nsplit = 1; return; }
+    }
     if (stale(ex, c, PF_FWD)) return;
     ConvProblem p{c.Cin, H, W, c.cout_tot, conv_out(H, c.KH, c.stride, c.ph), conv_out(W, c.KW, c.stride, c.pw),
                   c.KH, c.KW, c.stride, c.ph, c.pw};
@@ -560,6 +615,13 @@
     io.y = y.p; io.y_sb = y.sb; io.y_sc = y.sc; io.y_sh = y.sh; io.y_sw = 1;
     io.shuffle = shuffle;
     run_conv(ex, p, NB, io, y_total, packed + c.off[PF_FWD], c.w_rows, c.cout_pk, packed + c.off[PF_BIAS], allow_split, 0, nsplit);
+}
+
+static void conv_fwd(Exec& ex, const ConvSpec& c, const float* packed, int NB, int H, int W, CView x, View y, long long y_total,
+                     int shuffle, int allow_split, int* nsplit)
+{
+    conv_fwd_run(ex, c, packed, NB, H, W, x, y, y_total, shuffle, allow_split, nsplit);
+    ex.v_ready.valid = 0;
 }
 
 static void conv_dgrad(Exec& ex, const ConvSpec& c, const float* packed, int NB, int H, int W, CView dy, View dx, long long dx_total,
@@ -1049,20 +1111,63 @@
     return en;
 }
 
-static void norm_fwd(Exec& ex, float* x, long long x_sn, long long x_sc, long long x_total, int nslab, const NormP& np, float* stats,
-                     float* y, long long y_sn, long long y_sc, int y_sh, const float* res, int N, int C, int H, int W, int act)
-{
-    if (ex.dry) { ex.y_xs_pw = 0; return; }
+enum { kXfF1 = 1, kXfF2 = 2, kXfF3 = 3 };
+constexpr int kXfDefaultMask = 1 << kXfF1;
+static int g_fuse_wino_xform = mcvc_knob("MCVC_FUSE_WINO_XFORM", 1);
+static bool fuse_wino_xform(int bit) { return ((g_fuse_wino_xform == 1 ? kXfDefaultMask : g_fuse_wino_xform & ~1) >> bit & 1) != 0; }
+
+static bool next_conv_emit(Exec& ex, const NextConv* h, WinoEmitArgs& e, const WinoFam** fam)
+{
+    if (!h || ex.dry || !fuse_wino_xform(h->bit)) return false;
+    if (!h->shuffle && sgemm_kind(*h->c, h->NB, h->H, h->W).kind) return false;
+    WinoPass p{};
+    if (plan_conv_fwd_wino(ex, *h->c, h->packed, h->NB, h->H, h->W, h->shuffle, true, p) != kPlanPass || p.nbc != p.NB) return false;
+    e = WinoEmitArgs{};
+    e.fam = (p.f == &kWino[kF23] && p.XH) ? 16 : ((p.f == &kWino[kF45] && !p.XH) ? 64 : 0);
+    if (!e.fam) return false;
+    e.xi = wino_xi(ex, p, h->x, 0, p.NB); e.XH = p.XH; e.XW = p.XW;
+    *fam = p.f;
+    return true;
+}
+static void set_v_ready(Exec& ex, const WinoEmitArgs& e, const WinoFam* fam)
+{
+    ex.v_ready.valid = 1; ex.v_ready.f = fam; ex.v_ready.xi = e.xi; ex.v_ready.XH = e.XH; ex.v_ready.XW = e.XW;
+}
+
+static NormArgs norm_fwd_args(const Exec& ex, float* x, long long x_sn, long long x_sc, long long x_total, int nslab, const NormP& np, float* stats,
+                              float* y, long long y_sn, long long y_sc, int y_sh, const float* res, int N, int C, int H, int W, int act)
+{
     NormArgs a{};
     a.x = x; a.x_slabs = ex.slabs; a.x_sn = x_sn; a.x_sc = x_sc; a.slab_stride = x_total; a.nslab = nslab;
     a.gamma[0] = np.g[0]; a.gamma[1] = np.g[1]; a.beta[0] = np.b[0]; a.beta[1] = np.b[1];
     a.stats = stats; a.y = y; a.res = res; a.y_sn = y_sn; a.y_sc = y_sc; a.y_sh = y_sh;
     a.N = N; a.C = C; a.H = H; a.W = W; a.act = act; a.eps = kInEps;
+    return a;
+}
+static bool norm_fwd_emits(Exec& ex, const NormArgs& a, const WinoOutArgs& pend, const WinoFam& f, const NextConv* h, WinoEmitArgs& e, const WinoFam** fam)
+{
+    return mcvc_norm_fwd_wino_applies(a, pend, f.norm_pts) && next_conv_emit(ex, h, e, fam) && mcvc_norm_fwd_wino_emit_applies(a, pend, f.norm_pts, e);
+}
+
+static void norm_fwd(Exec& ex, float* x, long long x_sn, long long x_sc, long long x_total, int nslab, const NormP& np, float* stats,
+                     float* y, long long y_sn, long long y_sc, int y_sh, const float* res, int N, int C, int H, int W, int act)
+{
+    const NextConv* const next = ex.next_conv;
+    ex.next_conv = nullptr;
+    if (ex.dry) { ex.y_xs_pw = 0; return; }
+    NormArgs a = norm_fwd_args(ex, x, x_sn, x_sc, x_total, nslab, np, stats, y, y_sn, y_sc, y_sh, res, N, C, H, W, act);
     if (ex.y_xs_pw) { a.y_xs = 1; a.xs_pw = ex.y_xs_pw; a.xs_plane = ex.y_xs_plane; ex.y_xs_pw = 0; }
     if (ex.pend_fam) {
         const WinoFam& f = *ex.pend_fam;
         ex.pend_fam = nullptr;
-        if (mcvc_norm_fwd_wino_applies(a, ex.pend, f.norm_pts)) { ex.fail(mcvc_norm_fwd_wino_launch(a, ex.pend, f.norm_pts, ex.s)); return; }
+        if (mcvc_norm_fwd_wino_applies(a, ex.pend, f.norm_pts)) {
+            WinoEmitArgs e{};
+            const WinoFam* efam = nullptr;
+            const bool emit = norm_fwd_emits(ex, a, ex.pend, f, next, e, &efam);
+            ex.fail(mcvc_norm_fwd_wino_launch(a, ex.pend, f.norm_pts, ex.s, emit ? &e : nullptr));
+            if (emit) set_v_ready(ex, e, efam);
+            return;
+        }
         ex.fail(f.output(ex.pend, ex.s));
     }
     ex.fail(mcvc_norm_fwd_launch(a, ex.s));
@@ -1085,10 +1190,25 @@
     ex.fail(mcvc_norm_bwd_launch(a, ex.s));
 }
 
+static ActArgs act_fwd_args(const Exec& ex, float* x, long long x_total, int nslab, float* y, int N, int C, int P, int act)
+{
+    ActArgs a{}; a.x = x; a.x_slabs = ex.slabs; a.slab_stride = x_total; a.nslab = nslab; a.y = y; a.N = N; a.C = C; a.P = P; a.act = act;
+    return a;
+}
+static bool act_fwd_emits(Exec& ex, const ActArgs& a, const NextConv* h, WinoEmitArgs& e, const WinoFam** fam)
+{
+    return next_conv_emit(ex, h, e, fam) && mcvc_act_fwd_emit_applies(a, e);
+}
 static void act_fwd(Exec& ex, float* x, long long x_total, int nslab, float* y, int N, int C, int P, int act)
 {
+    const NextConv* const next = ex.next_conv;
+    ex.next_conv = nullptr;
     if (ex.dry) return;
-    ActArgs a{}; a.x = x; a.x_slabs = ex.slabs; a.slab_stride = x_total; a.nslab = nslab; a.y = y; a.N = N; a.C = C; a.P = P; a.act = act;
+    const ActArgs a = act_fwd_args(ex, x, x_total, nslab, y, N, C, P, act);
+    WinoEmitArgs e{};
+    const WinoFam* efam = nullptr;
+    const bool emit = act_fwd_emits(ex, a, next, e, &efam);
+    if (emit) { ex.fail(mcvc_act_fwd_emit_launch(a, e, ex.s)); set_v_ready(ex, e, efam); return; }
     ex.fail(mcvc_act_fwd_launch(a, ex.s));
 }
 
@@ -1211,6 +1331,13 @@
     return s;
 }
 
+struct GenFwdViews { CView y1, y2, y7; };
+static GenFwdViews gen_fwd_views(const float* st, const GenStash& o, const GenDims& d)
+{
+    return GenFwdViews{CView{st + o.y1, 128LL * 80 * d.T, 80LL * d.T, d.T}, CView{st + o.y2, 256LL * 40 * d.W2, 40LL * d.W2, d.W2},
+                       CView{st + o.y7, 256LL * 40 * d.Wu1, 40LL * d.Wu1, d.Wu1}};
+}
+
 static void gen_forward_impl(Exec& ex, const float* const* P, const float* packed, const float* x, const float* mask, float* out,
                              float* st, const GenDims& d)
 {
@@ -1223,15 +1350,19 @@
     if (!ex.dry) ex.fail(mcvc_prep_input_launch(x, mask, st + o.xin, B, 80 * T, ex.s));
     conv_fwd(ex, g.conv1, packed, B, 80, T, CView{st + o.xin, 2LL * 80 * T, 80LL * T, T}, View{st + o.c1, 256LL * 80 * T, 80LL * T, T},
              (long long)B * 256 * 80 * T, 0, 1, &ns);
+    const GenFwdViews gv = gen_fwd_views(st, o, d);
+    const NextConv nc1{&g.ds1, packed, B, 80, T, gv.y1, 0, kXfF1}, nc2{&g.ds2, packed, B, 40, W2, gv.y2, 0, kXfF2}, nc3{&g.up2, packed, B, 40, Wu1, gv.y7, 1, kXfF3};
+    ex.next_conv = &nc1;
     act_fwd(ex, st + o.c1, (long long)B * 256 * 80 * T, ns, st + o.y1, B, 128, 80 * T, ACT_GLU);
     ex.fuse_next = fuse_wino_norm();
-    conv_fwd(ex, g.ds1, packed, B, 80, T, CView{st + o.y1, 128LL * 80 * T, 80LL * T, T}, View{st + o.c2, 512LL * 40 * W2, 40LL * W2, W2},
+    conv_fwd(ex, g.ds1, packed, B, 80, T, gv.y1, View{st + o.c2, 512LL * 40 * W2, 40LL * W2, W2},
              (long long)B * 512 * 40 * W2, 0, 1, &ns);
     ex.fuse_next = 0;
+    ex.next_conv = &nc2;
     norm_fwd(ex, st + o.c2, 512LL * 40 * W2, 40LL * W2, (long long)B * 512 * 40 * W2, ns, normp(P, nullptr, 6, 7, 10, 11), st + o.s2,
              st + o.y2, 256LL * 40 * W2, 40LL * W2, W2, nullptr, B, 256, 40, W2, ACT_GLU);
     ex.fuse_next = fuse_wino_norm();
-    conv_fwd(ex, g.ds2, packed, B, 40, W2, CView{st + o.y2, 256LL * 40 * W2, 40LL * W2, W2}, View{st + o.c3, 512LL * 20 * W4, 20LL * W4, W4},
+    conv_fwd(ex, g.ds2, packed, B, 40, W2, gv.y2, View{st + o.c3, 512LL * 20 * W4, 20LL * W4, W4},
              (long long)B * 512 * 20 * W4, 0, 1, &ns);
     ex.fuse_next = 0;
     norm_fwd(ex, st + o.c3, 512LL * 20 * W4, 20LL * W4, (long long)B * 512 * 20 * W4, ns, normp(P, nullptr, 14, 15, 18, 19), st + o.s3,
@@ -1289,10 +1420,11 @@
     conv_fwd(ex, g.up1, packed, B, 20, W4, CView{st + o.y6, 256LL * 20 * W4, 20LL * W4, W4}, View{st + o.c7, 256LL * 40 * Wu1, 40LL * Wu1, Wu1},
              (long long)B * 256 * 40 * Wu1, 1, 1, &ns);
     ex.fuse_next = 0;
+    ex.next_conv = &nc3;
     norm_fwd(ex, st + o.c7, 256LL * 40 * Wu1, 40LL * Wu1, (long long)B * 256 * 40 * Wu1, ns, normp(P, nullptr, 106, 107), st + o.s7,
              st + o.y7, 256LL * 40 * Wu1, 40LL * Wu1, Wu1, nullptr, B, 256, 40, Wu1, ACT_SILU);
     ex.fuse_next = fuse_wino_norm();
-    conv_fwd(ex, g.up2, packed, B, 40, Wu1, CView{st + o.y7, 256LL * 40 * Wu1, 40LL * Wu1, Wu1}, View{st + o.c8, 128LL * 80 * Wu2, 80LL * Wu2, Wu2},
+    conv_fwd(ex, g.up2, packed, B, 40, Wu1, gv.y7, View{st + o.c8, 128LL * 80 * Wu2, 80LL * Wu2, Wu2},
              (long long)B * 128 * 80 * Wu2, 1, 1, &ns);
     ex.fuse_next = 0;
     norm_fwd(ex, st + o.c8, 128LL * 80 * Wu2, 80LL * Wu2, (long long)B * 128 * 80 * Wu2, ns, normp(P, nullptr, 102, 103), st + o.s8,
@@ -2122,6 +2254,57 @@
     return ex.err;
 }
 
+int mcvc_set_fuse_wino_xform(int v)
+{
+    const int old = g_fuse_wino_xform;
+    if (v >= 0) g_fuse_wino_xform = v;
+    return old;
+}
+
+int mcvc_gen_xform_fusion_plan(int B, int T, int* fused, int* planned)
+{
+    if (B < 1 || T < 1 || !fused || !planned) return MCVC_ERR_INVALID;
+    const GenDims d = gen_dims(B, T);
+    if (d.W4 < 2) return MCVC_ERR_INVALID;
+    for (int i = 0; i < MCVC_XFORM_BOUNDARIES; ++i) fused[i] = planned[i] = 0;
+    const GenNet& g = gen_net();
+    const GenStash o = gen_stash(d);
+    const int W2 = d.W2, Wu1 = d.Wu1;
+    float* const st = reinterpret_cast<float*>(1 << 20);
+    const float* const packed = reinterpret_cast<const float*>(1 << 12);
+    Exec ex{};
+    ex.wv = ex.wm = reinterpret_cast<float*>(16);
+    ex.wino_cap = gen_scratch(d).wino_floats;
+    const GenFwdViews gv = gen_fwd_views(st, o, d);
+    const NextConv nc[3] = {{&g.ds1, packed, B, 80, T, gv.y1, 0, kXfF1}, {&g.ds2, packed, B, 40, W2, gv.y2, 0, kXfF2}, {&g.up2, packed, B, 40, Wu1, gv.y7, 1, kXfF3}};
+    for (int i = 0; i < 3; ++i) {
+        WinoPass p{};
+        if (plan_conv_fwd_wino(ex, *nc[i].c, packed, nc[i].NB, nc[i].H, nc[i].W, nc[i].shuffle, true, p) == kPlanPass) planned[i] = p.f->norm_pts;
+    }
+    WinoEmitArgs e{};
+    const WinoFam* ef = nullptr;
+    {
+        int ns = 1;
+        Exec dry{}; dry.dry = true;
+        conv_fwd(dry, g.conv1, nullptr, B, 80, T, CView{nullptr, 2LL * 80 * T, 80LL * T, T}, View{nullptr, 256LL * 80 * T, 80LL * T, T}, (long long)B * 256 * 80 * T, 0, 1, &ns);
+        if (act_fwd_emits(ex, act_fwd_args(ex, st + o.c1, (long long)B * 256 * 80 * T, ns, st + o.y1, B, 128, 80 * T, ACT_GLU), &nc[0], e, &ef)) fused[0] = ef->norm_pts;
+    }
+    struct { const ConvSpec* c; int H, W, shuffle; View cv; NormArgs a; } prod[2] = {
+        {&g.ds1, 80, T, 0, View{st + o.c2, 512LL * 40 * W2, 40LL * W2, W2},
+         norm_fwd_args(ex, st + o.c2, 512LL * 40 * W2, 40LL * W2, (long long)B * 512 * 40 * W2, 1, NormP{}, st + o.s2, st + o.y2, 256LL * 40 * W2, 40LL * W2, W2,
+                       nullptr, B, 256, 40, W2, ACT_GLU)},
+        {&g.up1, 20, d.W4, 1, View{st + o.c7, 256LL * 40 * Wu1, 40LL * Wu1, Wu1},
+         norm_fwd_args(ex, st + o.c7, 256LL * 40 * Wu1, 40LL * Wu1, (long long)B * 256 * 40 * Wu1, 1, NormP{}, st + o.s7, st + o.y7, 256LL * 40 * Wu1, 40LL * Wu1, Wu1,
+                       nullptr, B, 256, 40, Wu1, ACT_SILU)}};
+    ex.fuse_next = fuse_wino_norm();
+    for (int i = 0; i < 2; ++i) {
+        WinoPass p{};
+        if (plan_conv_fwd_wino(ex, *prod[i].c, packed, B, prod[i].H, prod[i].W, prod[i].shuffle, true, p) != kPlanPass || !wino_defers(ex, p)) continue;
+        if (norm_fwd_emits(ex, prod[i].a, wino_oa(ex, p, prod[i].cv, 0, B), *p.f, &nc[1 + i], e, &ef)) fused[1 + i] = ef->norm_pts;
+    }
+    return 0;
+}
+
 int mcvc_gen_trunk_fault(float* scratch, int B, int T, int reset, void* stream)
 {
     if (!scratch || B < 1 || T < 1) return -MCVC_ERR_INVALID;
diff --git a/maskcyclegan-vc_amd/csrc/norm_kernels.hip b/maskcyclegan-vc_amd/csrc/norm_kernels.hip
--- a/maskcyclegan-vc_amd/csrc/norm_kernels.hip
+++ b/maskcyclegan-vc_amd/csrc/norm_kernels.hip
@@ -2,6 +2,7 @@
 #include "trace.h"
 #include "launch.h"
 #include "wino.h"
+#include "wino4.h"
 
 namespace {
 
@@ -602,10 +603,14 @@
     } };
 
 struct NormFwdWinoKArgs { NormArgs a; WinoOutArgs w; };
-template <int G, int TT, int PTS>
-__global__ void __launch_bounds__(256) norm_fwd_wino_kernel(const Twin<NormFwdWinoKArgs> tw)
-{
-    const NormFwdWinoKArgs ka_ = tw.v[blockIdx.z];
+struct NormFwdWinoEmitKArgs { NormArgs a; WinoOutArgs w; WinoXformArgs e; int XH, XW; };
+template <int EMIT> struct NormFwdWinoKA { using type = NormFwdWinoEmitKArgs; };
+template <> struct NormFwdWinoKA<0> { using type = NormFwdWinoKArgs; };
+template <int G, int TT, int PTS, int EMIT>
+__global__ void __launch_bounds__(256) norm_fwd_wino_kernel(const Twin<typename NormFwdWinoKA<EMIT>::type> tw)
+{
+    const typename NormFwdWinoKA<EMIT>::type ka_ = tw.v[blockIdx.z];
+    extern __shared__ __attribute__((aligned(16))) float ybuf[];
     const NormArgs& a = ka_.a;
     const WinoOutArgs& w = ka_.w;
     __shared__ float red[4];
@@ -709,6 +714,7 @@
         }
     }
     float* yp = a.y + (long long)n * a.y_sn + (long long)c * a.y_sc;
+    float* yb = ybuf + (EMIT != 0 ? g * (a.H * a.W) : 0);
 #pragma unroll
     for (int k = 0; k < TT; ++k) {
         if (pos[k] >= 0) {
@@ -721,8 +727,79 @@
                 else if (a.act == ACT_SILU) y = z0 * sigmoidf_(z0);
                 else y = z0;
                 yp[(long long)(h0 + (e / S) * (SHUF ? 2 : 1)) * a.y_sh + w0 + (e % S) * dw] = y;
-            }
-        }
+                if constexpr (EMIT != 0) yb[(h0 + (e / S) * (SHUF ? 2 : 1)) * a.W + w0 + (e % S) * dw] = y;
+            }
+        }
+    }
+    if constexpr (EMIT != 0) {
+        __syncthreads();
+        const WinoXformArgs& ea = ka_.e;
+        const int per = ea.TH * ea.TW;
+        const long long exs = (long long)ea.C * ea.NTp;
+        if constexpr (EMIT == 16) {
+            for (int item = l; item < 4 * per; item += G) {
+                const int ph = item / per, t = item - ph * per;
+                const int ty = t / ea.TW, tx = t - ty * ea.TW;
+                float o[16];
+                wino3_phase_window(yb, a.W, ka_.XH, ka_.XW, ph >> 1, ph & 1, ty, tx, o);
+                float* dst = ea.v + (long long)(4 * c + ph) * ea.NTp + (long long)n * per + t;
+#pragma unroll
+                for (int pt = 0; pt < 16; ++pt) dst[(long long)pt * exs] = o[pt];
+            }
+        } else {
+            for (int t = l; t < per; t += G) {
+                const int ty = t / ea.TW, tx = t - ty * ea.TW;
+                float o[64];
+                w4_input(yb, a.W, 4 * ty - ea.pad, 4 * tx - ea.pad, ea.H, ea.W, o);
+                float* dst = ea.v + (long long)c * ea.NTp + (long long)n * per + t;
+#pragma unroll
+                for (int pt = 0; pt < 64; ++pt) dst[(long long)pt * exs] = o[pt];
+            }
+        }
+    }
+}
+
+struct ActFwdEmitKArgs { ActArgs a; WinoXformArgs e; int XH, XW, TB; };
+__global__ void __launch_bounds__(256) act_fwd_emit_kernel(const Twin<ActFwdEmitKArgs> tw)
+{
+    const ActFwdEmitKArgs ka_ = tw.v[blockIdx.z];
+    const ActArgs& a = ka_.a;
+    const WinoXformArgs& ea = ka_.e;
+    extern __shared__ __attribute__((aligned(16))) float ybuf[];
+    const int XH = ka_.XH, XW = ka_.XW;
+    const int plane_id = blockIdx.y;
+    const int n = plane_id / a.C, c = plane_id - n * a.C;
+    const int ty0 = blockIdx.x * ka_.TB, ty1 = min(ea.TH, ty0 + ka_.TB);
+    const int r0 = 4 * ty0 - 2;
+    const int rlo = max(r0, 0), rhi = min(XH, 4 * ty1 + 2);
+    const int own_lo = 4 * ty0, own_hi = min(XH, 4 * ty1);
+    const unsigned w4 = (unsigned)XW >> 2;
+    const float* xv = a.x + ((long long)n * 2 * a.C + c) * a.P;
+    const float* xg = xv + (long long)a.C * a.P;
+    float* yp = a.y + ((long long)n * a.C + c) * a.P;
+    for (unsigned q = threadIdx.x; q < (unsigned)(rhi - rlo) * w4; q += 256u) {
+        const unsigned rr = q / w4, i4 = q - rr * w4;
+        const int r = rlo + (int)rr;
+        const long long xo = (long long)r * XW + 4 * i4;
+        float4 v[2];
+        v[0] = ld4(xv + xo);
+        v[1] = ld4(xg + xo);
+        const float4 y = make_float4(v[0].x * sigmoidf_(v[1].x), v[0].y * sigmoidf_(v[1].y), v[0].z * sigmoidf_(v[1].z), v[0].w * sigmoidf_(v[1].w));
+        if (r >= own_lo && r < own_hi) st4(yp + xo, y);
+        st4(ybuf + (r - r0) * XW + 4 * i4, y);
+    }
+    __syncthreads();
+    const int per = ea.TH * ea.TW, band = (ty1 - ty0) * ea.TW;
+    const long long exs = (long long)ea.C * ea.NTp;
+    const float* src = ybuf - r0 * XW;
+    for (int item = threadIdx.x; item < 4 * band; item += 256) {
+        const int ph = item / band, t = item - ph * band;
+        const int ty = ty0 + t / ea.TW, tx = t % ea.TW;
+        float o[16];
+        wino3_phase_window(src, XW, XH, XW, ph >> 1, ph & 1, ty, tx, o);
+        float* dst = ea.v + (long long)(4 * c + ph) * ea.NTp + (long long)n * per + ty * ea.TW + tx;
+#pragma unroll
+        for (int pt = 0; pt < 16; ++pt) dst[(long long)pt * exs] = o[pt];
     }
 }
 
@@ -752,33 +829,99 @@
     return items > 0 && items <= wino_norm_max_items(pts);
 }
 
-int mcvc_norm_fwd_wino_launch(const NormArgs& a, const WinoOutArgs& w, int pts, hipStream_t s)
+static void wino_norm_cfg(int pts, int items, long long planes, int* G, int* TT)
+{
+    if (pts == 43 || pts == 64) {
+        if (items <= 64) { *G = 64; *TT = 1; }
+        else if (items <= 128) { *G = 64; *TT = 2; }
+        else if (items <= 256 && planes < 2048) { *G = 256; *TT = 1; }
+        else if (items <= 512) { *G = 256; *TT = 2; }
+        else { *G = 64; *TT = 5; }
+        return;
+    }
+    if (items <= 128) { *G = 64; *TT = 2; }
+    else if (items <= 512 && planes < 2048) { *G = 256; *TT = 2; }
+    else if (items <= 320) { *G = 64; *TT = 5; }
+    else { *G = 256; *TT = 5; }
+}
+
+bool mcvc_norm_fwd_wino_emit_applies(const NormArgs& a, const WinoOutArgs& w, int pts, const WinoEmitArgs& e)
+{
+    if (!mcvc_norm_fwd_wino_applies(a, w, pts) || a.y_xs) return false;
+    int G = 0, TT = 0;
+    wino_norm_cfg(pts, wino_norm_items(a, w, pts), (long long)a.N * a.C, &G, &TT);
+    if (G != 256 || (long long)a.H * a.W * 4 > 32768) return false;
+    const WinoXformArgs& x = e.xi;
+    if (x.x != a.y || x.x_sb != a.y_sn || x.x_sc != a.y_sc || x.x_sh != a.y_sh || a.y_sh != a.W || !x.v) return false;
+    if (x.N != a.N || x.NT != x.N * x.TH * x.TW || x.NTp < x.NT) return false;
+    if (e.fam == 16) {
+        if (pts != 16) return false;
+        return e.XH == a.H && e.XW == a.W && !(a.H & 1) && !(a.W & 1) && x.C == 4 * a.C && x.H == a.H / 2 && x.W == a.W / 2 &&
+               x.TH == (x.H + 1) / 2 && x.TW == (x.W + 1) / 2 && x.pad == 1;
+    }
+    if (e.fam == 64) {
+        if (pts != 36 && pts != 64) return false;
+        return e.XH == 0 && e.XW == 0 && x.C == a.C && x.H == a.H && x.W == a.W && x.TH == (x.H + 3) / 4 && x.TW == (x.W + 3) / 4 && x.pad == 2;
+    }
+    return false;
+}
+
+int mcvc_norm_fwd_wino_launch(const NormArgs& a, const WinoOutArgs& w, int pts, hipStream_t s, const WinoEmitArgs* emit)
 {
     const int items = wino_norm_items(a, w, pts);
     if (items <= 0 || items > wino_norm_max_items(pts)) return MCVC_ERR_INVALID;
+    if (emit && !mcvc_norm_fwd_wino_emit_applies(a, w, pts, *emit)) return MCVC_ERR_INVALID;
     const long long planes = (long long)a.N * a.C;
     const int nbr = ((pts == 16 || pts == 43) && a.act == ACT_GLU) ? 2 : 1;
     const double el = (double)planes * a.H * a.W * nbr;
     const double m_per_out = pts == 16 ? 4.0 : (pts == 36 ? 9.0 : (pts == 43 ? 2.25 : 4.0));
-    TraceScope ts(K_NORM_FWD, s, 0.0, 4.0 * (el * m_per_out + el + (double)planes * a.H * a.W));
-#define MCVC_FWD_WINO(GG, TT) { \
-        if (pts == 16) mcvc_launch((norm_fwd_wino_kernel<GG, TT, 16>), dim3((unsigned)cdiv_ll(planes, 256 / GG)), dim3(256), 0, s, NormFwdWinoKArgs{a, w}); \
-        else if (pts == 36) mcvc_launch((norm_fwd_wino_kernel<GG, TT, 36>), dim3((unsigned)cdiv_ll(planes, 256 / GG)), dim3(256), 0, s, NormFwdWinoKArgs{a, w}); \
-        else if (pts == 43) mcvc_launch((norm_fwd_wino_kernel<GG, TT, 43>), dim3((unsigned)cdiv_ll(planes, 256 / GG)), dim3(256), 0, s, NormFwdWinoKArgs{a, w}); \
-        else mcvc_launch((norm_fwd_wino_kernel<GG, TT, 64>), dim3((unsigned)cdiv_ll(planes, 256 / GG)), dim3(256), 0, s, NormFwdWinoKArgs{a, w}); \
+    const double v_bytes = emit ? 4.0 * emit->fam * emit->xi.C * emit->xi.NT : 0.0;
+    TraceScope ts(K_NORM_FWD, s, 0.0, 4.0 * (el * m_per_out + el + (double)planes * a.H * a.W) + v_bytes);
+    int G = 0, TT = 0;
+    wino_norm_cfg(pts, items, planes, &G, &TT);
+    const dim3 grid((unsigned)cdiv_ll(planes, 256 / G));
+#define MCVC_FWD_WINO(GG, T_, PP) \
+    if (G == GG && TT == T_ && pts == PP) { mcvc_launch((norm_fwd_wino_kernel<GG, T_, PP, 0>), grid, dim3(256), 0, s, NormFwdWinoKArgs{a, w}); return (int)hipGetLastError(); }
+#define MCVC_FWD_WINO_EMIT(T_, PP, EE) \
+    if (emit && G == 256 && TT == T_ && pts == PP && emit->fam == EE) { \
+        mcvc_launch((norm_fwd_wino_kernel<256, T_, PP, EE>), grid, dim3(256), (size_t)a.H * a.W * sizeof(float), s, \
+                    NormFwdWinoEmitKArgs{a, w, emit->xi, emit->XH, emit->XW}); \
         return (int)hipGetLastError(); }
-    if (pts == 43 || pts == 64) {
-        if (items <= 64) MCVC_FWD_WINO(64, 1)
-        if (items <= 128) MCVC_FWD_WINO(64, 2)
-        if (items <= 256 && planes < 2048) MCVC_FWD_WINO(256, 1)
-        if (items <= 512) MCVC_FWD_WINO(256, 2)
-        MCVC_FWD_WINO(64, 5)
-    }
-    if (items <= 128) MCVC_FWD_WINO(64, 2)
-    if (items <= 512 && planes < 2048) MCVC_FWD_WINO(256, 2)
-    if (items <= 320) MCVC_FWD_WINO(64, 5)
-    MCVC_FWD_WINO(256, 5)
+    MCVC_FWD_WINO_EMIT(2, 16, 16) MCVC_FWD_WINO_EMIT(5, 16, 16)
+    MCVC_FWD_WINO_EMIT(2, 36, 64) MCVC_FWD_WINO_EMIT(5, 36, 64)
+    MCVC_FWD_WINO_EMIT(1, 64, 64) MCVC_FWD_WINO_EMIT(2, 64, 64)
+    if (emit) return MCVC_ERR_INVALID;
+    MCVC_FWD_WINO(64, 2, 16) MCVC_FWD_WINO(256, 2, 16) MCVC_FWD_WINO(64, 5, 16) MCVC_FWD_WINO(256, 5, 16)
+    MCVC_FWD_WINO(64, 2, 36) MCVC_FWD_WINO(256, 2, 36) MCVC_FWD_WINO(64, 5, 36) MCVC_FWD_WINO(256, 5, 36)
+    MCVC_FWD_WINO(64, 1, 43) MCVC_FWD_WINO(64, 2, 43) MCVC_FWD_WINO(256, 1, 43) MCVC_FWD_WINO(256, 2, 43) MCVC_FWD_WINO(64, 5, 43)
+    MCVC_FWD_WINO(64, 1, 64) MCVC_FWD_WINO(64, 2, 64) MCVC_FWD_WINO(256, 1, 64) MCVC_FWD_WINO(256, 2, 64) MCVC_FWD_WINO(64, 5, 64)
 #undef MCVC_FWD_WINO
+#undef MCVC_FWD_WINO_EMIT
+    return MCVC_ERR_INVALID;
+}
+
+static int act_emit_band(const WinoEmitArgs& e) { const int tb = 256 / (4 * e.xi.TW); return tb < 1 ? 1 : (tb > e.xi.TH ? e.xi.TH : tb); }
+
+bool mcvc_act_fwd_emit_applies(const ActArgs& a, const WinoEmitArgs& e)
+{
+    const WinoXformArgs& x = e.xi;
+    if (a.act != ACT_GLU || a.nslab != 1 || !a.y || e.fam != 16 || !x.v) return false;
+    if (x.x != a.y || x.x_sb != (long long)a.C * a.P || x.x_sc != a.P || x.x_sh != e.XW) return false;
+    if (e.XH <= 0 || e.XW <= 0 || (e.XH & 1) || (e.XW & 3) || (long long)e.XH * e.XW != a.P) return false;
+    if (x.N != a.N || x.C != 4 * a.C || x.H != e.XH / 2 || x.W != e.XW / 2 || x.TH != (x.H + 1) / 2 || x.TW != (x.W + 1) / 2 || x.pad != 1) return false;
+    if (x.NT != x.N * x.TH * x.TW || x.NTp < x.NT) return false;
+    if ((((uintptr_t)a.x | (uintptr_t)a.y) & 15) != 0 || (long long)a.N * a.C > 65535) return false;
+    return (long long)(4 * act_emit_band(e) + 4) * e.XW * 4 <= 32768;
+}
+
+int mcvc_act_fwd_emit_launch(const ActArgs& a, const WinoEmitArgs& e, hipStream_t s)
+{
+    if (!mcvc_act_fwd_emit_applies(a, e)) return MCVC_ERR_INVALID;
+    const int tb = act_emit_band(e);
+    TraceScope ts(K_ACT_FWD, s, 0.0, 4.0 * (double)a.N * a.C * a.P * 3 + 4.0 * 16.0 * e.xi.C * e.xi.NT);
+    mcvc_launch(act_fwd_emit_kernel, dim3((unsigned)cdiv_i(e.xi.TH, tb), (unsigned)(a.N * a.C)), dim3(256), (size_t)(4 * tb + 4) * e.XW * sizeof(float), s,
+                ActFwdEmitKArgs{a, e.xi, e.XH, e.XW, tb});
+    return (int)hipGetLastError();
 }
 
 int mcvc_norm_fwd_launch(const NormArgs& a, hipStream_t s)
diff --git a/maskcyclegan-vc_amd/csrc/wino.h b/maskcyclegan-vc_amd/csrc/wino.h
--- a/maskcyclegan-vc_amd/csrc/wino.h
+++ b/maskcyclegan-vc_amd/csrc/wino.h
@@ -20,9 +20,45 @@
 };
 
 int mcvc_wino_input_launch(const WinoXformArgs& a, hipStream_t s);
+struct WinoEmitArgs { WinoXformArgs xi; int XH, XW; int fam; };
 struct NormArgs;
+struct ActArgs;
 bool mcvc_norm_fwd_wino_applies(const NormArgs& a, const WinoOutArgs& w, int pts);
-int mcvc_norm_fwd_wino_launch(const NormArgs& a, const WinoOutArgs& w, int pts, hipStream_t s);
+bool mcvc_norm_fwd_wino_emit_applies(const NormArgs& a, const WinoOutArgs& w, int pts, const WinoEmitArgs& e);
+int mcvc_norm_fwd_wino_launch(const NormArgs& a, const WinoOutArgs& w, int pts, hipStream_t s, const WinoEmitArgs* emit = nullptr);
+bool mcvc_act_fwd_emit_applies(const ActArgs& a, const WinoEmitArgs& e);
+int mcvc_act_fwd_emit_launch(const ActArgs& a, const WinoEmitArgs& e, hipStream_t s);
+
+static __device__ __forceinline__ void wino_bt4(const float d[4], float o[4])
+{
+    o[0] = d[0] - d[2]; o[1] = d[1] + d[2]; o[2] = d[2] - d[1]; o[3] = d[1] - d[3];
+}
+static __device__ __forceinline__ void wino3_phase_window(const float* src, int x_sh, int XH, int XW, int p, int q, int ty, int tx, float* o)
+{
+    const int i0 = 2 * ty - 1, j0 = 2 * tx - 1;
+    float t[4][4];
+#pragma unroll
+    for (int i = 0; i < 4; ++i) {
+        float d[4];
+        const int ih = 2 * (i0 + i) + p;
+        const bool rok = (i0 + i >= 0) && (ih < XH);
+#pragma unroll
+        for (int j = 0; j < 4; ++j) {
+            const int iw = 2 * (j0 + j) + q;
+            d[j] = (rok && j0 + j >= 0 && iw < XW) ? src[(long long)ih * x_sh + iw] : 0.f;
+        }
+        wino_bt4(d, t[i]);
+    }
+#pragma unroll
+    for (int b = 0; b < 4; ++b) {
+        float col[4], w[4];
+#pragma unroll
+        for (int i = 0; i < 4; ++i) col[i] = t[i][b];
+        wino_bt4(col, w);
+#pragma unroll
+        for (int aa = 0; aa < 4; ++aa) o[aa * 4 + b] = w[aa];
+    }
+}
 int mcvc_wino3_input_launch(const WinoXformArgs& a, hipStream_t s);
 int mcvc_wino3_output_launch(const WinoOutArgs& a, hipStream_t s);
 int mcvc_wino3_input_phase_launch(const WinoXformArgs& a, int XH, int XW, hipStream_t s);
diff --git a/maskcyclegan-vc_amd/csrc/wino4.h b/maskcyclegan-vc_amd/csrc/wino4.h
--- a/maskcyclegan-vc_amd/csrc/wino4.h
+++ b/maskcyclegan-vc_amd/csrc/wino4.h
@@ -25,6 +25,56 @@
     {0.f, 2.f, 4.f, -2.5f, -5.f, 0.5f, 1.f, 0.f},
     {0.f, -2.f, 4.f, 2.5f, -5.f, -0.5f, 1.f, 0.f},
     {0.f, -1.f, 0.f, 5.25f, 0.f, -5.25f, 0.f, 1.f}};
+
+static __device__ __forceinline__ void w4_bt(const float d[8], float o[8])
+{
+    const float e1 = d[2] - 4.25f * d[4] + d[6], o1 = d[1] - 4.25f * d[3] + d[5];
+    const float e2 = 0.25f * d[2] - 1.25f * d[4] + d[6], o2 = 0.5f * d[1] - 2.5f * d[3] + 2.f * d[5];
+    const float e3 = 4.f * d[2] - 5.f * d[4] + d[6], o3 = 2.f * d[1] - 2.5f * d[3] + 0.5f * d[5];
+    o[0] = (d[6] - d[0]) + 5.25f * (d[2] - d[4]);
+    o[1] = e1 + o1; o[2] = e1 - o1;
+    o[3] = e2 + o2; o[4] = e2 - o2;
+    o[5] = e3 + o3; o[6] = e3 - o3;
+    o[7] = (d[7] - d[1]) + 5.25f * (d[3] - d[5]);
+}
+static __device__ __forceinline__ void w4_input(const float* src, int x_sh, int ih0, int iw0, int H, int W, float* o)
+{
+    float t[8][8];
+    const float* rp = src + (long long)ih0 * x_sh + iw0;
+    if (ih0 >= 0 && ih0 + 7 < H && iw0 >= 0 && iw0 + 7 < W) {
+#pragma unroll
+        for (int i = 0; i < 8; ++i) {
+            float d[8];
+#pragma unroll
+            for (int j = 0; j < 8; ++j) d[j] = rp[j];
+            rp += x_sh;
+            w4_bt(d, t[i]);
+        }
+    } else {
+#pragma unroll
+        for (int i = 0; i < 8; ++i) {
+            float d[8];
+            const int ih = ih0 + i;
+            const bool rok = (ih >= 0) && (ih < H);
+#pragma unroll
+            for (int j = 0; j < 8; ++j) {
+                const int iw = iw0 + j;
+                d[j] = (rok && iw >= 0 && iw < W) ? rp[j] : 0.f;
+            }
+            rp += x_sh;
+            w4_bt(d, t[i]);
+        }
+    }
+#pragma unroll
+    for (int b = 0; b < 8; ++b) {
+        float col[8], q[8];
+#pragma unroll
+        for (int i = 0; i < 8; ++i) col[i] = t[i][b];
+        w4_bt(col, q);
+#pragma unroll
+        for (int aa = 0; aa < 8; ++aa) o[aa * 8 + b] = q[aa];
+    }
+}
 
 int mcvc_wino4_input_launch(const WinoXformArgs& a, hipStream_t s);
 int mcvc_wino4_output_launch(const WinoOutArgs& a, hipStream_t s);
diff --git a/maskcyclegan-vc_amd/csrc/wino4_kernels.hip b/maskcyclegan-vc_amd/csrc/wino4_kernels.hip
--- a/maskcyclegan-vc_amd/csrc/wino4_kernels.hip
+++ b/maskcyclegan-vc_amd/csrc/wino4_kernels.hip
@@ -5,17 +5,6 @@
 
 namespace {
 
-__device__ __forceinline__ void w4_bt(const float d[8], float o[8])
-{
-    const float e1 = d[2] - 4.25f * d[4] + d[6], o1 = d[1] - 4.25f * d[3] + d[5];
-    const float e2 = 0.25f * d[2] - 1.25f * d[4] + d[6], o2 = 0.5f * d[1] - 2.5f * d[3] + 2.f * d[5];
-    const float e3 = 4.f * d[2] - 5.f * d[4] + d[6], o3 = 2.f * d[1] - 2.5f * d[3] + 0.5f * d[5];
-    o[0] = (d[6] - d[0]) + 5.25f * (d[2] - d[4]);
-    o[1] = e1 + o1; o[2] = e1 - o1;
-    o[3] = e2 + o2; o[4] = e2 - o2;
-    o[5] = e3 + o3; o[6] = e3 - o3;
-    o[7] = (d[7] - d[1]) + 5.25f * (d[3] - d[5]);
-}
 __device__ __forceinline__ void w4_at(const float m[8], float o[4])
 {
     const float s12 = m[1] + m[2], d12 = m[1] - m[2], s34 = m[3] + m[4], d34 = m[3] - m[4], s56 = m[5] + m[6], d56 = m[5] - m[6];
@@ -30,45 +19,6 @@
     const float e4 = d[0] + 4.f * d[2], f4 = 2.f * d[1] + 8.f * d[3];
     const float eh = d[0] + 0.25f * d[2], fh = 0.5f * d[1] + 0.125f * d[3];
     o[0] = d[0]; o[1] = e + f; o[2] = e - f; o[3] = e4 + f4; o[4] = e4 - f4; o[5] = eh + fh; o[6] = eh - fh; o[7] = d[3];
-}
-
-__device__ __forceinline__ void w4_input(const float* src, int x_sh, int ih0, int iw0, int H, int W, float* o)
-{
-    float t[8][8];
-    const float* rp = src + (long long)ih0 * x_sh + iw0;
-    if (ih0 >= 0 && ih0 + 7 < H && iw0 >= 0 && iw0 + 7 < W) {
-#pragma unroll
-        for (int i = 0; i < 8; ++i) {
-            float d[8];
-#pragma unroll
-            for (int j = 0; j < 8; ++j) d[j] = rp[j];
-            rp += x_sh;
-            w4_bt(d, t[i]);
-        }
-    } else {
-#pragma unroll
-        for (int i = 0; i < 8; ++i) {
-            float d[8];
-            const int ih = ih0 + i;
-            const bool rok = (ih >= 0) && (ih < H);
-#pragma unroll
-            for (int j = 0; j < 8; ++j) {
-                const int iw = iw0 + j;
-                d[j] = (rok && iw >= 0 && iw < W) ? rp[j] : 0.f;
-            }
-            rp += x_sh;
-            w4_bt(d, t[i]);
-        }
-    }
-#pragma unroll
-    for (int b = 0; b < 8; ++b) {
-        float col[8], q[8];
-#pragma unroll
-        for (int i = 0; i < 8; ++i) col[i] = t[i][b];
-        w4_bt(col, q);
-#pragma unroll
-        for (int aa = 0; aa < 8; ++aa) o[aa * 8 + b] = q[aa];
-    }
 }
 
 __device__ __forceinline__ void w4_dy(const float* src, int x_sh, int oh0, int ow0, int H, int W, float* o)
diff --git a/maskcyclegan-vc_amd/csrc/wino_kernels.hip b/maskcyclegan-vc_amd/csrc/wino_kernels.hip
--- a/maskcyclegan-vc_amd/csrc/wino_kernels.hip
+++ b/maskcyclegan-vc_amd/csrc/wino_kernels.hip
@@ -52,10 +52,7 @@
     }
 }
 
-__device__ __forceinline__ void bt4(const float d[4], float o[4])
-{
-    o[0] = d[0] - d[2]; o[1] = d[1] + d[2]; o[2] = d[2] - d[1]; o[3] = d[1] - d[3];
-}
+__device__ __forceinline__ void bt4(const float d[4], float o[4]) { wino_bt4(d, o); }
 
 __global__ void __launch_bounds__(256) wino3_input_kernel(const Twin<WinoXformArgs> tw)
 {
@@ -108,32 +105,12 @@
     const int per = a.TH * a.TW;
     const int n = tile / per, r = tile - n * per;
     const int ty = r / a.TW, tx = r - ty * a.TW;
-    const int i0 = 2 * ty - 1, j0 = 2 * tx - 1;
-    const float* src = a.x + (long long)n * a.x_sb + (long long)ci * a.x_sc;
-    float t[4][4];
-#pragma unroll
-    for (int i = 0; i < 4; ++i) {
-        float d[4];
-        const int ih = 2 * (i0 + i) + p;
-        const bool rok = (i0 + i >= 0) && (ih < XH);
-#pragma unroll
-        for (int j = 0; j < 4; ++j) {
-            const int iw = 2 * (j0 + j) + q;
-            d[j] = (rok && j0 + j >= 0 && iw < XW) ? src[(long long)ih * a.x_sh + iw] : 0.f;
-        }
-        bt4(d, t[i]);
-    }
+    float o[16];
+    wino3_phase_window(a.x + (long long)n * a.x_sb + (long long)ci * a.x_sc, a.x_sh, XH, XW, p, q, ty, tx, o);
     float* dst = a.v + (long long)k * a.NTp + tile;
     const long long xs = (long long)a.C * a.NTp;
 #pragma unroll
-    for (int b = 0; b < 4; ++b) {
-        float col[4], o[4];
-#pragma unroll
-        for (int i = 0; i < 4; ++i) col[i] = t[i][b];
-        bt4(col, o);
-#pragma unroll
-        for (int aa = 0; aa < 4; ++aa) dst[(long long)(aa * 4 + b) * xs] = o[aa];
-    }
+    for (int pt = 0; pt < 16; ++pt) dst[(long long)pt * xs] = o[pt];
 }
 
 
diff --git a/maskcyclegan-vc_amd/mask_cyclegan_vc/_hip.py b/maskcyclegan-vc_amd/mask_cyclegan_vc/_hip.py
--- a/maskcyclegan-vc_amd/mask_cyclegan_vc/_hip.py
+++ b/maskcyclegan-vc_amd/mask_cyclegan_vc/_hip.py
@@ -89,6 +89,8 @@
     "mcvc_disc_update_batch": (c_int, [_PP, c_void_p, c_void_p, c_int, c_int, c_void_p, c_void_p, c_void_p, c_void_p, c_void_p,
                                        c_float, c_float, c_float, c_float, c_int, c_float, c_int, c_void_p]),
     "mcvc_pack_plan": (c_int, [c_int, c_int, c_int, c_int, c_int, c_int, c_void_p, c_int, c_void_p]),
+    "mcvc_set_fuse_wino_xform": (c_int, [c_int]),
+    "mcvc_gen_xform_fusion_plan": (c_int, [c_int, c_int, c_void_p, c_void_p]),
     "mcvc_draw_batch": (c_int, [c_void_p, c_void_p, c_int, c_longlong, c_void_p, c_void_p, c_int, c_longlong, c_int, c_int, c_int,
                                 ctypes.c_ulonglong, ctypes.c_ulonglong, c_void_p, c_void_p, c_void_p, c_void_p, c_void_p, c_void_p]),
     "mcvc_audio_frames": (c_int, [c_int]),
```

Result: no change. 183.0, median of 6 (+0.7%).
